# Muennighoff/sgpt

Measured on AMD Instinct MI355X. Metric: encoded sentences/sec (SGPT-125M, seq_len 128, encode + weighted-mean pool + cosine top-10 chunk loop), higher is better.
Workload: dtype f16

## Files before the change

include/sgpt_hip.h:

```cpp
#ifndef SGPT_HIP_H
#define SGPT_HIP_H

#include <stddef.h>
#include <stdint.h>

#ifdef __cplusplus
extern "C" {
#endif

#define SGPT_ABI_VERSION 18

typedef int sgpt_status;
#define SGPT_OK 0
#define SGPT_ERR_INVALID (-1)
#define SGPT_ERR_HIP (-2)
#define SGPT_ERR_MISSING (-3)
#define SGPT_ERR_OOM (-4)
#define SGPT_ERR_COMM (-6)
#define SGPT_ERR_RANGE (-5)

typedef struct sgpt_ctx sgpt_ctx;
typedef struct sgpt_model sgpt_model;

enum { SGPT_F32 = 0, SGPT_BF16 = 1, SGPT_FP8W = 2, SGPT_F16 = 3, SGPT_FP8M = 4 };
enum { SGPT_ARCH_GPTNEO = 0, SGPT_ARCH_GPTJ = 1, SGPT_ARCH_BLOOM = 2, SGPT_ARCH_BERT = 3, SGPT_ARCH_LLAMA = 4 };
enum { SGPT_POOL_WEIGHTEDMEAN = 0, SGPT_POOL_MEAN = 1, SGPT_POOL_LASTTOKEN = 2, SGPT_POOL_LEARNTMEAN = 3,
       SGPT_POOL_CLS = 4 };
enum { SGPT_COS = 0, SGPT_DOT = 1, SGPT_NEG_L2 = 2 };

typedef struct {
    int32_t arch;
    int32_t n_layers;
    int32_t d_model;
    int32_t n_heads;
    int32_t d_ffn;
    int32_t vocab;
    int32_t max_pos;
    int32_t window;
    float ln_eps;
    float attn_scale;
    int32_t compute_dtype;
    const uint8_t* layer_is_local;
    int32_t rotary_dim;
    int32_t qk_split;
    int32_t split_weights;
    int32_t n_kv_heads;
} sgpt_model_desc;

typedef struct {
    const char* name;
    const float* ptr;
    int64_t numel;
} sgpt_tensor_view;

int sgpt_abi_version(void);
sgpt_status sgpt_ctx_create(int hip_device, sgpt_ctx** out);
void sgpt_ctx_destroy(sgpt_ctx* ctx);
const char* sgpt_last_error(const sgpt_ctx* ctx);

sgpt_status sgpt_model_load(sgpt_ctx* ctx, const sgpt_model_desc* desc,
                            const sgpt_tensor_view* tensors, size_t n_tensors, sgpt_model** out);
void sgpt_model_free(sgpt_model* model);

sgpt_status sgpt_model_calibrate_begin(sgpt_model* model);
sgpt_status sgpt_model_calibrate_end(sgpt_model* model, float margin, float* scales_out);
sgpt_status sgpt_model_set_act_scales(sgpt_model* model, const float* scales, int32_t n_scales);

sgpt_status sgpt_encode(sgpt_model* model, const int32_t* ids, const int32_t* pos,
                        const int32_t* seq_off, const int32_t* seq_len, const int32_t* pad_left,
                        int32_t B, int32_t T_pad, int32_t max_alloc_len,
                        int32_t pool_mode, int32_t n_layers_run, int32_t apply_final_ln,
                        int32_t normalize, float* out, float* hidden_out, void* stream);

sgpt_status sgpt_encode_layers(sgpt_model* model, const int32_t* ids, const int32_t* pos,
                               const int32_t* seq_off, const int32_t* seq_len, const int32_t* pad_left,
                               int32_t B, int32_t T_pad, int32_t max_alloc_len, int32_t pool_mode,
                               int32_t normalize, float* out_layers, float* out_mean, void* stream);

sgpt_status sgpt_model_set_pool_weights(sgpt_model* model, const float* weights, int32_t n);

sgpt_status sgpt_lm_logprobs(sgpt_model* model, const float* hidden, const int32_t* row_idx, const int32_t* targets,
                             int32_t n, float* out_logprob, int32_t* out_greedy, void* stream);

sgpt_status sgpt_pool(sgpt_ctx* ctx, const void* hidden, int32_t hidden_dtype, const int32_t* mask,
                      int32_t B, int32_t S, int32_t d, int32_t pool_mode, float* out, void* stream);
sgpt_status sgpt_pool_learnt(sgpt_ctx* ctx, const void* hidden, int32_t hidden_dtype, const int32_t* mask,
                             int32_t B, int32_t S, int32_t d, const float* pos_weights, float* out, void* stream);

sgpt_status sgpt_l2_normalize(sgpt_ctx* ctx, const float* in, int64_t n, int32_t d,
                              void* out, int32_t out_dtype, void* stream);

sgpt_status sgpt_pairwise_scores(sgpt_ctx* ctx, const float* a, const float* b, int64_t n, int32_t d, int32_t cosine,
                                 float* out, void* stream);

sgpt_status sgpt_f32_to_16(sgpt_ctx* ctx, const float* in, int64_t numel, void* out, int32_t out_dtype, void* stream);
sgpt_status sgpt_f32_to_bf16(sgpt_ctx* ctx, const float* in, int64_t numel, void* out, void* stream);

sgpt_status sgpt_model_range_check(sgpt_model* model, int32_t* flagged, int32_t reset, void* stream);
sgpt_status sgpt_model_range_adapt(sgpt_model* model, int32_t* n_raised, void* stream);
sgpt_status sgpt_model_get_range_shifts(sgpt_model* model, int32_t* shifts, int32_t n);
sgpt_status sgpt_model_set_range_shifts(sgpt_model* model, const int32_t* shifts, int32_t n);
sgpt_status sgpt_range_check(sgpt_ctx* ctx, int32_t* flagged, int32_t reset, void* stream);

#define SGPT_PREC_CLASSES 5
enum { SGPT_PC_LN1 = 0, SGPT_PC_ATT = 1, SGPT_PC_CTX = 2, SGPT_PC_LN2 = 3, SGPT_PC_H = 4 };
sgpt_status sgpt_model_set_precision(sgpt_model* model, const int32_t* plan, int32_t n);
sgpt_status sgpt_model_get_precision(sgpt_model* model, int32_t* plan, int32_t n);
sgpt_status sgpt_model_release_split_weights(sgpt_model* model, int64_t* bytes_freed);
sgpt_status sgpt_model_precision_probe_begin(sgpt_model* model);
sgpt_status sgpt_model_precision_probe_end(sgpt_model* model, float* crest_out );
sgpt_status sgpt_row_crest(sgpt_ctx* ctx, const void* x, int32_t dtype, int64_t n, int32_t d, int64_t ld, float* crest_out,
                           void* stream);
sgpt_status sgpt_split16(sgpt_ctx* ctx, const float* in, int64_t n, int32_t d, int32_t layout, void* out, int32_t out_dtype,
                         void* stream);
sgpt_status sgpt_linear_split(sgpt_ctx* ctx, int32_t dtype, int32_t epi, const void* A, const void* W, const float* bias,
                              void* out, int64_t ldo, int64_t lo_delta, int64_t hi2_delta, int32_t M, int32_t N, int32_t K,
                              void* stream);

uint64_t sgpt_ctx_generation(const sgpt_ctx* ctx);
sgpt_status sgpt_ctx_reserve(sgpt_ctx* ctx, size_t encode_bytes, size_t score_bytes);

sgpt_status sgpt_fp8_quantize_rows(sgpt_ctx* ctx, const float* w, int64_t rows, int64_t cols,
                                   uint8_t* codes, float* scale, void* stream);
sgpt_status sgpt_fp8_dequantize_rows(sgpt_ctx* ctx, const uint8_t* codes, const float* scale, int64_t rows,
                                     int64_t cols, void* out, int32_t out_dtype, void* stream);

sgpt_status sgpt_scores(sgpt_ctx* ctx, const void* a, const void* b, int32_t dtype,
                        int64_t na, int64_t nb, int32_t d, float* out, int64_t ldo, void* stream);

sgpt_status sgpt_score_topk(sgpt_ctx* ctx, const void* q, const void* corpus, int32_t dtype,
                            int32_t nq, int64_t N, int32_t d, int32_t k, int64_t idx_base,
                            float* run_val, int64_t* run_idx, int32_t n_run, int32_t* n_out,
                            void* stream);

sgpt_status sgpt_score_topk_q8(sgpt_ctx* ctx, const void* q, const uint8_t* codes, const float* scale, int32_t nq, int64_t N, int32_t d,
                               int32_t k, int64_t idx_base, float* run_val, int64_t* run_idx, int32_t n_run, int32_t* n_out,
                               void* stream);

sgpt_status sgpt_score_topk_refined(sgpt_ctx* ctx, const float* q, const float* corpus32, const void* corpus16, int32_t dtype16,
                                    int32_t nq, int64_t N, int32_t d, int32_t k, int64_t idx_base, float margin,
                                    float* run_val, int64_t* run_idx, int32_t n_run, int32_t* n_out, int32_t* fallback_flag_out,
                                    void* stream);

sgpt_status sgpt_topk_merge(sgpt_ctx* ctx, const float* val, const int64_t* idx, int32_t nq,
                            int32_t m, int32_t k, const int64_t* exclude_idx,
                            float* out_val, int64_t* out_idx, void* stream);

#define SGPT_COMM_ID_BYTES 128
sgpt_status sgpt_comm_unique_id(uint8_t* id );
sgpt_status sgpt_comm_init(sgpt_ctx* ctx, const uint8_t* id, int32_t rank, int32_t world);
sgpt_status sgpt_comm_destroy(sgpt_ctx* ctx);
int32_t sgpt_comm_world(const sgpt_ctx* ctx);
int32_t sgpt_comm_rank(const sgpt_ctx* ctx);
sgpt_status sgpt_allgather_rows(sgpt_ctx* ctx, const void* local, const int64_t* counts, int64_t row_bytes, void* out,
                                void* stream);
sgpt_status sgpt_allgather_rows_padded(sgpt_ctx* ctx, const void* local, const int64_t* counts, int64_t row_bytes, void* out,
                                       void* stream);
sgpt_status sgpt_exchange_topk(sgpt_ctx* ctx, const float* val, const int64_t* idx, int32_t nq, int32_t k, int32_t k_out,
                               const int64_t* exclude_idx, float* out_val, int64_t* out_idx, void* stream);
sgpt_status sgpt_fold_gathered_topk(sgpt_ctx* ctx, const float* gathered_val, const int64_t* gathered_idx, int32_t world,
                                    int32_t nq, int32_t k, int32_t k_out, const int64_t* exclude_idx, float* out_val,
                                    int64_t* out_idx, void* stream);

sgpt_status sgpt_topk(sgpt_ctx* ctx, const float* scores, int32_t nq, int64_t n, int64_t ld,
                      int32_t k, int64_t idx_base, float* out_val, int64_t* out_idx, void* stream);

#define SGPT_EVAL_MAX_CUTS 16
sgpt_status sgpt_eval_ranked(sgpt_ctx* ctx, const int64_t* idx, const float* val, int32_t nq, int32_t K,
                             const int32_t* qrel_off, const int64_t* qrel_pos, const int32_t* qrel_rel,
                             const int32_t* ideal_rel, const int32_t* k_values, int32_t nk, int32_t check_order,
                             int32_t* out_hits, int32_t* out_first, float* out_dcg, float* out_idcg, float* out_sp,
                             int32_t* out_R, void* stream);

#define SGPT_EVAL_MAX_GROUP 1024
sgpt_status sgpt_eval_groups(sgpt_ctx* ctx, const float* emb, int32_t n_rows, int32_t d, int32_t mode, const float* scores_in,
                             int32_t G, const int32_t* grp_off, int32_t n_cand, int32_t max_group, const int32_t* q_row,
                             const int32_t* cand_row, const int32_t* cand_rel, const int32_t* R_extra,
                             const int32_t* ideal_off, const int32_t* ideal_rel, int32_t n_ideal, float* out_scores,
                             int32_t* out_order, int32_t* out_hits1, int32_t* out_hits5, int32_t* out_first, int32_t* out_R, float* out_sp,
                             float* out_dcg, float* out_idcg, void* stream);

#define SGPT_EVAL_MAX_PAIRS (1 << 24)
sgpt_status sgpt_eval_pairs(sgpt_ctx* ctx, const float* score, const int32_t* label, int32_t n, int32_t check_nan,
                            int32_t* out_rank2, int64_t* out_n_pos, int64_t* out_n_used, double* out_ap_num, void* stream);

sgpt_status sgpt_linear(sgpt_ctx* ctx, int32_t dtype, int32_t epi, int32_t out_dtype, const void* A, const void* W,
                        const float* bias, const float* resid, void* out, int32_t M, int32_t N, int32_t K, void* stream);

sgpt_status sgpt_linear_query(sgpt_ctx* ctx, int32_t dtype, int32_t epi, const void* A, const float* x, const float* ln_gamma,
                              const float* ln_beta, float ln_eps, const void* W, const float* bias, const float* resid, void* out,
                              void* out_vt, int32_t n_split, int32_t M, int32_t N, int32_t K, void* stream);

sgpt_status sgpt_linear_qkv(sgpt_ctx* ctx, int32_t dtype, const void* A, const void* W, void* out, void* out_vt, int32_t n_split,
                            int32_t M, int32_t N, int32_t K, void* stream);

sgpt_status sgpt_attention(sgpt_ctx* ctx, int32_t dtype, const void* q, const void* k, const void* v, int64_t ldq, int64_t ldvt,
                           void* out, int64_t ldo, const int32_t* seq_off, int32_t B, int32_t T, int32_t H, int32_t dh,
                           int32_t window, float scale, const float* alibi, int32_t max_alloc_len, int32_t out_fp8,
                           float out_scale, int32_t* range_flag, int32_t x3, int64_t qk_lo_delta, int64_t v_lo_delta,
                           int64_t ctx_lo_delta, int64_t ctx_hi2_delta, void* stream);

sgpt_status sgpt_attention_ex(sgpt_ctx* ctx, int32_t dtype, const void* q, const void* k, const void* v, int64_t ldq, int64_t ldvt,
                              void* out, int64_t ldo, const int32_t* seq_off, int32_t B, int32_t T, int32_t H, int32_t dh,
                              int32_t window, float scale, const float* alibi, int32_t max_alloc_len, int32_t out_fp8,
                              float out_scale, int32_t* range_flag, int32_t x3, int64_t qk_lo_delta, int64_t v_lo_delta,
                              int64_t ctx_lo_delta, int64_t ctx_hi2_delta, int32_t causal, const int32_t* seq_len, void* stream);

sgpt_status sgpt_attention_gqa(sgpt_ctx* ctx, int32_t dtype, const void* q, const void* k, const void* v, int64_t ldq, int64_t ldvt,
                               void* out, int64_t ldo, const int32_t* seq_off, int32_t B, int32_t T, int32_t H, int32_t n_kv_heads,
                               int32_t dh, int32_t window, float scale, const float* alibi, int32_t max_alloc_len, int32_t out_fp8,
                               float out_scale, int32_t* range_flag, int32_t x3, int64_t qk_lo_delta, int64_t v_lo_delta,
                               int64_t ctx_lo_delta, int64_t ctx_hi2_delta, void* stream);

sgpt_status sgpt_embed(sgpt_ctx* ctx, const int32_t* ids, const int32_t* pos, const float* wte, const float* wpe, int32_t T,
                       int32_t d, int32_t vocab, int32_t max_pos, float* out, void* stream);
sgpt_status sgpt_layernorm(sgpt_ctx* ctx, const float* x, const float* gamma, const float* beta, int32_t T, int32_t d, float eps,
                           void* out, int32_t out_dtype, float out_mul, int32_t split, void* stream);
sgpt_status sgpt_layernorm_writeback(sgpt_ctx* ctx, float* x, const float* gamma, const float* beta, int32_t T, int32_t d, float eps,
                                     void* out16, int32_t out_dtype, void* stream);
sgpt_status sgpt_rmsnorm(sgpt_ctx* ctx, const float* x, const float* gamma, int32_t T, int32_t d, float eps, void* out, int32_t out_dtype,
                         void* stream);
sgpt_status sgpt_swiglu(sgpt_ctx* ctx, const void* gu, int32_t dtype, int32_t T, int32_t ffn, void* out, void* stream);
sgpt_status sgpt_rope_half(sgpt_ctx* ctx, void* buf, int32_t dtype, int64_t ld, int64_t k_off, const int32_t* pos, const float* sin_t,
                           const float* cos_t, int32_t T, int32_t H, int32_t H_kv, int32_t head_dim, int32_t max_pos, void* stream);
sgpt_status sgpt_qknorm_rope_half(sgpt_ctx* ctx, void* buf, int32_t dtype, int64_t ld, int64_t k_off, const int32_t* pos,
                                  const float* sin_t, const float* cos_t, int32_t T, int32_t H, int32_t H_kv, int32_t head_dim,
                                  int32_t max_pos, const float* q_gamma, const float* k_gamma, float eps, void* stream);
sgpt_status sgpt_lnf_pool_ex(sgpt_ctx* ctx, const float* x, const float* gamma, const float* beta, const int32_t* seq_off,
                             const int32_t* seq_len, const int32_t* pad_left, int32_t B, int32_t d, float eps, int32_t apply_ln,
                             int32_t mode, int32_t normalize, const float* pos_weights, int32_t n_weights, float* out,
                             int32_t* nonfinite_flag, int32_t norm_kind, void* stream);
sgpt_status sgpt_lnf_pool(sgpt_ctx* ctx, const float* x, const float* gamma, const float* beta, const int32_t* seq_off,
                          const int32_t* seq_len, const int32_t* pad_left, int32_t B, int32_t d, float eps, int32_t apply_ln,
                          int32_t mode, int32_t normalize, const float* pos_weights, int32_t n_weights, float* out,
                          int32_t* nonfinite_flag, void* stream);
sgpt_status sgpt_rope(sgpt_ctx* ctx, void* buf, int32_t dtype, int64_t ld, int64_t k_off, const int32_t* pos, const float* sin,
                      const float* cos, int32_t T, int32_t H, int32_t head_dim, int32_t rotary_dim, int32_t max_pos, void* stream);
sgpt_status sgpt_logprob_rows(sgpt_ctx* ctx, const float* logits, int64_t ld, int32_t V, const int32_t* targets, int32_t n,
                              float* out_logprob, int32_t* out_greedy, void* stream);

sgpt_status sgpt_layernorm_fp8(sgpt_ctx* ctx, const float* x, const float* gamma, const float* beta, int32_t T, int32_t d,
                               float eps, uint8_t* codes, float* row_scale, void* stream);
sgpt_status sgpt_linear_fp8(sgpt_ctx* ctx, int32_t epi, int32_t out_dtype, const uint8_t* A, const float* a_scale,
                            float a_scalar, const uint8_t* W, const float* w_scale, const float* bias, const float* resid,
                            void* out, float out_scale, int32_t M, int32_t N, int32_t K, void* stream);

sgpt_status sgpt_prof_enable(sgpt_ctx* ctx, int32_t on);
sgpt_status sgpt_prof_read(sgpt_ctx* ctx, int64_t* launches, double* ms, double* flops, int32_t reset);

int32_t sgpt_ctx_set_gemm_cu_cap(sgpt_ctx* ctx, int32_t n);
int32_t sgpt_ctx_set_low_latency(sgpt_ctx* ctx, int32_t on);
int32_t sgpt_ctx_set_tile_policy(sgpt_ctx* ctx, int32_t policy);
int32_t sgpt_ctx_set_query_tile(sgpt_ctx* ctx, int32_t k);

sgpt_status sgpt_bench_gemm(sgpt_ctx* ctx, int32_t dtype, int32_t epi, int32_t out_dtype,
                            int32_t M, int32_t N, int32_t K, int32_t iters, float* ms_out);

#ifdef __cplusplus
}
#endif
#endif
```

sgpt_amd/_lib.py:

```python
import ctypes as C
import os

HERE = os.path.dirname(os.path.abspath(__file__))
LIB_PATH = os.environ.get("SGPT_HIP_LIB") or os.path.join(HERE, "lib", "libsgpt_hip.so")

SGPT_F32, SGPT_BF16, SGPT_FP8W, SGPT_F16, SGPT_FP8M = 0, 1, 2, 3, 4
SGPT_ABI_VERSION = 18
SGPT_PREC_CLASSES = 5
PC_LN1, PC_ATT, PC_CTX, PC_LN2, PC_H = 0, 1, 2, 3, 4
SGPT_ERR_RANGE = -5
SGPT_ERR_COMM = -6
SGPT_COMM_ID_BYTES = 128
SGPT_EVAL_MAX_CUTS = 16
SGPT_EVAL_MAX_GROUP = 1024
SGPT_EVAL_MAX_PAIRS = 1 << 24
SGPT_COS, SGPT_DOT, SGPT_NEG_L2 = 0, 1, 2
SGPT_ARCH_GPTNEO, SGPT_ARCH_GPTJ, SGPT_ARCH_BLOOM, SGPT_ARCH_BERT, SGPT_ARCH_LLAMA = 0, 1, 2, 3, 4
POOL_MODES = {"weightedmean": 0, "mean": 1, "lasttoken": 2, "learntmean": 3, "cls": 4}
EPI_BIAS_GELU_ERF = 9


class ModelDesc(C.Structure):
    _fields_ = [("arch", C.c_int32), ("n_layers", C.c_int32), ("d_model", C.c_int32), ("n_heads", C.c_int32),
                ("d_ffn", C.c_int32), ("vocab", C.c_int32), ("max_pos", C.c_int32), ("window", C.c_int32),
                ("ln_eps", C.c_float), ("attn_scale", C.c_float), ("compute_dtype", C.c_int32),
                ("layer_is_local", C.POINTER(C.c_uint8)), ("rotary_dim", C.c_int32), ("qk_split", C.c_int32),
                ("split_weights", C.c_int32), ("n_kv_heads", C.c_int32)]


class TensorView(C.Structure):
    _fields_ = [("name", C.c_char_p), ("ptr", C.c_void_p), ("numel", C.c_int64)]


SIGNATURES = {
    "sgpt_abi_version": (C.c_int, []),
    "sgpt_ctx_create": (C.c_int, [C.c_int, C.POINTER(C.c_void_p)]),
    "sgpt_ctx_destroy": (None, [C.c_void_p]),
    "sgpt_last_error": (C.c_char_p, [C.c_void_p]),
    "sgpt_model_load": (C.c_int, [C.c_void_p, C.POINTER(ModelDesc), C.POINTER(TensorView), C.c_size_t,
                                  C.POINTER(C.c_void_p)]),
    "sgpt_model_free": (None, [C.c_void_p]),
    "sgpt_encode": (C.c_int, [C.c_void_p, C.c_void_p, C.c_void_p, C.c_void_p, C.c_void_p, C.c_void_p,
                              C.c_int32, C.c_int32, C.c_int32, C.c_int32, C.c_int32, C.c_int32, C.c_int32,
                              C.c_void_p, C.c_void_p, C.c_void_p]),
    "sgpt_encode_layers": (C.c_int, [C.c_void_p, C.c_void_p, C.c_void_p, C.c_void_p, C.c_void_p, C.c_void_p,
                                     C.c_int32, C.c_int32, C.c_int32, C.c_int32, C.c_int32, C.c_void_p, C.c_void_p,
                                     C.c_void_p]),
    "sgpt_model_set_pool_weights": (C.c_int, [C.c_void_p, C.c_void_p, C.c_int32]),
    "sgpt_pool_learnt": (C.c_int, [C.c_void_p, C.c_void_p, C.c_int32, C.c_void_p, C.c_int32, C.c_int32, C.c_int32,
                                   C.c_void_p, C.c_void_p, C.c_void_p]),
    "sgpt_fp8_quantize_rows": (C.c_int, [C.c_void_p, C.c_void_p, C.c_int64, C.c_int64, C.c_void_p, C.c_void_p,
                                         C.c_void_p]),
    "sgpt_fp8_dequantize_rows": (C.c_int, [C.c_void_p, C.c_void_p, C.c_void_p, C.c_int64, C.c_int64, C.c_void_p,
                                           C.c_int32, C.c_void_p]),
    "sgpt_lm_logprobs": (C.c_int, [C.c_void_p, C.c_void_p, C.c_void_p, C.c_void_p, C.c_int32, C.c_void_p, C.c_void_p,
                                   C.c_void_p]),
    "sgpt_pool": (C.c_int, [C.c_void_p, C.c_void_p, C.c_int32, C.c_void_p, C.c_int32, C.c_int32, C.c_int32,
                            C.c_int32, C.c_void_p, C.c_void_p]),
    "sgpt_l2_normalize": (C.c_int, [C.c_void_p, C.c_void_p, C.c_int64, C.c_int32, C.c_void_p, C.c_int32, C.c_void_p]),
    "sgpt_pairwise_scores": (C.c_int, [C.c_void_p, C.c_void_p, C.c_void_p, C.c_int64, C.c_int32, C.c_int32, C.c_void_p, C.c_void_p]),
    "sgpt_f32_to_bf16": (C.c_int, [C.c_void_p, C.c_void_p, C.c_int64, C.c_void_p, C.c_void_p]),
    "sgpt_f32_to_16": (C.c_int, [C.c_void_p, C.c_void_p, C.c_int64, C.c_void_p, C.c_int32, C.c_void_p]),
    "sgpt_range_check": (C.c_int, [C.c_void_p, C.POINTER(C.c_int32), C.c_int32, C.c_void_p]),
    "sgpt_ctx_generation": (C.c_uint64, [C.c_void_p]),
    "sgpt_ctx_reserve": (C.c_int, [C.c_void_p, C.c_size_t, C.c_size_t]),
    "sgpt_scores": (C.c_int, [C.c_void_p, C.c_void_p, C.c_void_p, C.c_int32, C.c_int64, C.c_int64, C.c_int32,
                              C.c_void_p, C.c_int64, C.c_void_p]),
    "sgpt_score_topk": (C.c_int, [C.c_void_p, C.c_void_p, C.c_void_p, C.c_int32, C.c_int32, C.c_int64, C.c_int32,
                                  C.c_int32, C.c_int64, C.c_void_p, C.c_void_p, C.c_int32, C.POINTER(C.c_int32),
                                  C.c_void_p]),
    "sgpt_score_topk_q8": (C.c_int, [C.c_void_p, C.c_void_p, C.c_void_p, C.c_void_p, C.c_int32, C.c_int64, C.c_int32,
                                     C.c_int32, C.c_int64, C.c_void_p, C.c_void_p, C.c_int32, C.POINTER(C.c_int32),
                                     C.c_void_p]),
    "sgpt_score_topk_refined": (C.c_int, [C.c_void_p, C.c_void_p, C.c_void_p, C.c_void_p, C.c_int32, C.c_int32, C.c_int64, C.c_int32,
                                           C.c_int32, C.c_int64, C.c_float, C.c_void_p, C.c_void_p, C.c_int32, C.c_void_p, C.c_void_p,
                                           C.c_void_p]),
    "sgpt_topk_merge": (C.c_int, [C.c_void_p, C.c_void_p, C.c_void_p, C.c_int32, C.c_int32, C.c_int32, C.c_void_p,
                                  C.c_void_p, C.c_void_p, C.c_void_p]),
    "sgpt_topk": (C.c_int, [C.c_void_p, C.c_void_p, C.c_int32, C.c_int64, C.c_int64, C.c_int32, C.c_int64,
                            C.c_void_p, C.c_void_p, C.c_void_p]),
    "sgpt_eval_ranked": (C.c_int, [C.c_void_p, C.c_void_p, C.c_void_p, C.c_int32, C.c_int32, C.c_void_p, C.c_void_p, C.c_void_p,
                                   C.c_void_p, C.POINTER(C.c_int32), C.c_int32, C.c_int32, C.c_void_p, C.c_void_p, C.c_void_p,
                                   C.c_void_p, C.c_void_p, C.c_void_p, C.c_void_p]),
    "sgpt_eval_groups": (C.c_int, [C.c_void_p, C.c_void_p, C.c_int32, C.c_int32, C.c_int32, C.c_void_p, C.c_int32, C.c_void_p, C.c_int32,
                                   C.c_int32, C.c_void_p, C.c_void_p, C.c_void_p, C.c_void_p, C.c_void_p, C.c_void_p, C.c_int32,
                                   C.c_void_p, C.c_void_p, C.c_void_p, C.c_void_p, C.c_void_p, C.c_void_p, C.c_void_p, C.c_void_p,
                                   C.c_void_p, C.c_void_p]),
    "sgpt_eval_pairs": (C.c_int, [C.c_void_p, C.c_void_p, C.c_void_p, C.c_int32, C.c_int32, C.c_void_p, C.c_void_p, C.c_void_p,
                                  C.c_void_p, C.c_void_p]),
    "sgpt_linear": (C.c_int, [C.c_void_p, C.c_int32, C.c_int32, C.c_int32, C.c_void_p, C.c_void_p, C.c_void_p, C.c_void_p,
                              C.c_void_p, C.c_int32, C.c_int32, C.c_int32, C.c_void_p]),
    "sgpt_linear_query": (C.c_int, [C.c_void_p, C.c_int32, C.c_int32, C.c_void_p, C.c_void_p, C.c_void_p, C.c_void_p, C.c_float, C.c_void_p,
                                    C.c_void_p, C.c_void_p, C.c_void_p, C.c_void_p, C.c_int32, C.c_int32, C.c_int32, C.c_int32, C.c_void_p]),
    "sgpt_linear_qkv": (C.c_int, [C.c_void_p, C.c_int32, C.c_void_p, C.c_void_p, C.c_void_p, C.c_void_p, C.c_int32, C.c_int32, C.c_int32,
                                  C.c_int32, C.c_void_p]),
    "sgpt_model_calibrate_begin": (C.c_int, [C.c_void_p]),
    "sgpt_model_calibrate_end": (C.c_int, [C.c_void_p, C.c_float, C.c_void_p]),
    "sgpt_model_set_act_scales": (C.c_int, [C.c_void_p, C.c_void_p, C.c_int32]),
    "sgpt_layernorm_fp8": (C.c_int, [C.c_void_p, C.c_void_p, C.c_void_p, C.c_void_p, C.c_int32, C.c_int32, C.c_float, C.c_void_p,
                                     C.c_void_p, C.c_void_p]),
    "sgpt_linear_fp8": (C.c_int, [C.c_void_p, C.c_int32, C.c_int32, C.c_void_p, C.c_void_p, C.c_float, C.c_void_p, C.c_void_p,
                                  C.c_void_p, C.c_void_p, C.c_void_p, C.c_float, C.c_int32, C.c_int32, C.c_int32, C.c_void_p]),
    "sgpt_comm_unique_id": (C.c_int, [C.c_void_p]),
    "sgpt_comm_init": (C.c_int, [C.c_void_p, C.c_void_p, C.c_int32, C.c_int32]),
    "sgpt_comm_destroy": (C.c_int, [C.c_void_p]),
    "sgpt_comm_world": (C.c_int32, [C.c_void_p]),
    "sgpt_comm_rank": (C.c_int32, [C.c_void_p]),
    "sgpt_allgather_rows": (C.c_int, [C.c_void_p, C.c_void_p, C.c_void_p, C.c_int64, C.c_void_p, C.c_void_p]),
    "sgpt_allgather_rows_padded": (C.c_int, [C.c_void_p, C.c_void_p, C.c_void_p, C.c_int64, C.c_void_p, C.c_void_p]),
    "sgpt_exchange_topk": (C.c_int, [C.c_void_p, C.c_void_p, C.c_void_p, C.c_int32, C.c_int32, C.c_int32, C.c_void_p,
                                     C.c_void_p, C.c_void_p, C.c_void_p]),
    "sgpt_fold_gathered_topk": (C.c_int, [C.c_void_p, C.c_void_p, C.c_void_p, C.c_int32, C.c_int32, C.c_int32, C.c_int32,
                                          C.c_void_p, C.c_void_p, C.c_void_p, C.c_void_p]),
    "sgpt_ctx_set_low_latency": (C.c_int32, [C.c_void_p, C.c_int32]),
    "sgpt_ctx_set_tile_policy": (C.c_int32, [C.c_void_p, C.c_int32]),
    "sgpt_ctx_set_gemm_cu_cap": (C.c_int32, [C.c_void_p, C.c_int32]),
    "sgpt_ctx_set_query_tile": (C.c_int32, [C.c_void_p, C.c_int32]),
    "sgpt_model_range_check": (C.c_int, [C.c_void_p, C.POINTER(C.c_int32), C.c_int32, C.c_void_p]),
    "sgpt_model_range_adapt": (C.c_int, [C.c_void_p, C.POINTER(C.c_int32), C.c_void_p]),
    "sgpt_model_get_range_shifts": (C.c_int, [C.c_void_p, C.c_void_p, C.c_int32]),
    "sgpt_model_set_range_shifts": (C.c_int, [C.c_void_p, C.c_void_p, C.c_int32]),
    "sgpt_model_set_precision": (C.c_int, [C.c_void_p, C.c_void_p, C.c_int32]),
    "sgpt_model_get_precision": (C.c_int, [C.c_void_p, C.c_void_p, C.c_int32]),
    "sgpt_model_release_split_weights": (C.c_int, [C.c_void_p, C.c_void_p]),
    "sgpt_model_precision_probe_begin": (C.c_int, [C.c_void_p]),
    "sgpt_model_precision_probe_end": (C.c_int, [C.c_void_p, C.c_void_p]),
    "sgpt_row_crest": (C.c_int, [C.c_void_p, C.c_void_p, C.c_int32, C.c_int64, C.c_int32, C.c_int64, C.POINTER(C.c_float), C.c_void_p]),
    "sgpt_split16": (C.c_int, [C.c_void_p, C.c_void_p, C.c_int64, C.c_int32, C.c_int32, C.c_void_p, C.c_int32, C.c_void_p]),
    "sgpt_linear_split": (C.c_int, [C.c_void_p, C.c_int32, C.c_int32, C.c_void_p, C.c_void_p, C.c_void_p, C.c_void_p,
                                    C.c_int64, C.c_int64, C.c_int64, C.c_int32, C.c_int32, C.c_int32, C.c_void_p]),
    "sgpt_attention": (C.c_int, [C.c_void_p, C.c_int32, C.c_void_p, C.c_void_p, C.c_void_p, C.c_int64, C.c_int64,
                                 C.c_void_p, C.c_int64, C.c_void_p, C.c_int32, C.c_int32, C.c_int32, C.c_int32,
                                 C.c_int32, C.c_float, C.c_void_p, C.c_int32, C.c_int32,
                                 C.c_float, C.c_void_p, C.c_int32, C.c_int64, C.c_int64,
                                 C.c_int64, C.c_int64, C.c_void_p]),
    "sgpt_attention_ex": (C.c_int, [C.c_void_p, C.c_int32, C.c_void_p, C.c_void_p, C.c_void_p, C.c_int64, C.c_int64,
                                    C.c_void_p, C.c_int64, C.c_void_p, C.c_int32, C.c_int32, C.c_int32, C.c_int32,
                                    C.c_int32, C.c_float, C.c_void_p, C.c_int32, C.c_int32,
                                    C.c_float, C.c_void_p, C.c_int32, C.c_int64, C.c_int64,
                                    C.c_int64, C.c_int64, C.c_int32, C.c_void_p, C.c_void_p]),
    "sgpt_attention_gqa": (C.c_int, [C.c_void_p, C.c_int32, C.c_void_p, C.c_void_p, C.c_void_p, C.c_int64, C.c_int64,
                                     C.c_void_p, C.c_int64, C.c_void_p, C.c_int32, C.c_int32, C.c_int32, C.c_int32, C.c_int32,
                                     C.c_int32, C.c_float, C.c_void_p, C.c_int32, C.c_int32,
                                     C.c_float, C.c_void_p, C.c_int32, C.c_int64, C.c_int64,
                                     C.c_int64, C.c_int64, C.c_void_p]),
    "sgpt_rmsnorm": (C.c_int, [C.c_void_p, C.c_void_p, C.c_void_p, C.c_int32, C.c_int32, C.c_float, C.c_void_p, C.c_int32, C.c_void_p]),
    "sgpt_swiglu": (C.c_int, [C.c_void_p, C.c_void_p, C.c_int32, C.c_int32, C.c_int32, C.c_void_p, C.c_void_p]),
    "sgpt_rope_half": (C.c_int, [C.c_void_p, C.c_void_p, C.c_int32, C.c_int64, C.c_int64, C.c_void_p, C.c_void_p, C.c_void_p,
                                 C.c_int32, C.c_int32, C.c_int32, C.c_int32, C.c_int32, C.c_void_p]),
    "sgpt_qknorm_rope_half": (C.c_int, [C.c_void_p, C.c_void_p, C.c_int32, C.c_int64, C.c_int64, C.c_void_p, C.c_void_p, C.c_void_p,
                                        C.c_int32, C.c_int32, C.c_int32, C.c_int32, C.c_int32, C.c_void_p, C.c_void_p, C.c_float,
                                        C.c_void_p]),
    "sgpt_lnf_pool_ex": (C.c_int, [C.c_void_p, C.c_void_p, C.c_void_p, C.c_void_p, C.c_void_p, C.c_void_p, C.c_void_p, C.c_int32,
                                   C.c_int32, C.c_float, C.c_int32, C.c_int32, C.c_int32, C.c_void_p, C.c_int32, C.c_void_p,
                                   C.c_void_p, C.c_int32, C.c_void_p]),
    "sgpt_layernorm_writeback": (C.c_int, [C.c_void_p, C.c_void_p, C.c_void_p, C.c_void_p, C.c_int32, C.c_int32, C.c_float, C.c_void_p,
                                           C.c_int32, C.c_void_p]),
    "sgpt_embed": (C.c_int, [C.c_void_p, C.c_void_p, C.c_void_p, C.c_void_p, C.c_void_p, C.c_int32, C.c_int32, C.c_int32, C.c_int32,
                             C.c_void_p, C.c_void_p]),
    "sgpt_layernorm": (C.c_int, [C.c_void_p, C.c_void_p, C.c_void_p, C.c_void_p, C.c_int32, C.c_int32, C.c_float, C.c_void_p,
                                 C.c_int32, C.c_float, C.c_int32, C.c_void_p]),
    "sgpt_lnf_pool": (C.c_int, [C.c_void_p, C.c_void_p, C.c_void_p, C.c_void_p, C.c_void_p, C.c_void_p, C.c_void_p, C.c_int32,
                                C.c_int32, C.c_float, C.c_int32, C.c_int32, C.c_int32, C.c_void_p, C.c_int32, C.c_void_p,
                                C.c_void_p, C.c_void_p]),
    "sgpt_rope": (C.c_int, [C.c_void_p, C.c_void_p, C.c_int32, C.c_int64, C.c_int64, C.c_void_p, C.c_void_p, C.c_void_p,
                            C.c_int32, C.c_int32, C.c_int32, C.c_int32, C.c_int32, C.c_void_p]),
    "sgpt_logprob_rows": (C.c_int, [C.c_void_p, C.c_void_p, C.c_int64, C.c_int32, C.c_void_p, C.c_int32, C.c_void_p, C.c_void_p,
                                    C.c_void_p]),
    "sgpt_bench_gemm": (C.c_int, [C.c_void_p, C.c_int32, C.c_int32, C.c_int32, C.c_int32, C.c_int32, C.c_int32,
                                  C.c_int32, C.POINTER(C.c_float)]),
    "sgpt_prof_enable": (C.c_int, [C.c_void_p, C.c_int32]),
    "sgpt_prof_read": (C.c_int, [C.c_void_p, C.POINTER(C.c_int64), C.POINTER(C.c_double), C.POINTER(C.c_double),
                                 C.c_int32]),
}

_lib = None


class SgptHipError(RuntimeError):
    pass


class SgptRangeError(SgptHipError):
    """dtype='f16': a weight is outside the IEEE-half range, or an activation class is beyond every power-of-two range
    shift (use dtype='bf16'); dtype='fp8mfma': an e4m3 code saturated (re-calibrate)."""

EXPERIMENT_SIGNATURES = {
    "sgpt_exp_set_gemm_skew": (C.c_int32, [C.c_int32]),
    "sgpt_exp_set_gemm_w": (C.c_int32, [C.c_int32]),
}


def load():
    global _lib
    if _lib is not None:
        return _lib
    if not os.path.exists(LIB_PATH):
        raise SgptHipError(f"{LIB_PATH} is missing: build it with `python -m sgpt_amd.build` "
                           "(hipcc --offload-arch=gfx950); there is no CPU/PyTorch fallback")
    lib = C.CDLL(LIB_PATH)
    for name, (res, args) in SIGNATURES.items():
        fn = getattr(lib, name)
        fn.restype = res
        fn.argtypes = args
    for name, (res, args) in EXPERIMENT_SIGNATURES.items():
        if hasattr(lib, name):
            fn = getattr(lib, name)
            fn.restype = res
            fn.argtypes = args
    if lib.sgpt_abi_version() != SGPT_ABI_VERSION:
        raise SgptHipError("libsgpt_hip.so ABI version mismatch: rebuild with `python -m sgpt_amd.build --force`")
    _lib = lib
    return lib


def check(ctx_handle, status, what=""):
    if status == 0:
        return
    msg = load().sgpt_last_error(ctx_handle)
    msg = msg.decode() if msg else ""
    if status == -1:
        raise ValueError(f"{what}: {msg}")
    if status == SGPT_ERR_RANGE:
        raise SgptRangeError(f"{what}: {msg}")
    raise SgptHipError(f"{what}: status {status}: {msg}")
```

sgpt_amd/csrc/common.h:

```cpp
#pragma once
#include <hip/hip_runtime.h>
#include <stdint.h>

typedef uint16_t bf16_t;
struct f16_t { uint16_t bits; };
typedef __attribute__((ext_vector_type(8))) __bf16 bf16x8;
typedef __attribute__((ext_vector_type(8))) _Float16 f16x8;
typedef __attribute__((ext_vector_type(4))) float f32x4;
typedef __attribute__((ext_vector_type(16))) float f32x16;

constexpr int DT_F32 = 0, DT_BF16 = 1, DT_FP8W = 2, DT_F16 = 3;
__host__ __device__ constexpr bool dt_is16(int dt) { return dt == DT_BF16 || dt == DT_F16; }

#define WAVE 64

typedef uint2 __attribute__((may_alias)) uint2_a;
typedef uint4 __attribute__((may_alias)) uint4_a;
typedef float4 __attribute__((may_alias)) float4_a;

__device__ __forceinline__ float bf16_to_f32(bf16_t v) { return __uint_as_float(((uint32_t)v) << 16); }

typedef __attribute__((ext_vector_type(2))) __bf16 bf16x2_t;
typedef __attribute__((ext_vector_type(2))) float f32x2_t;
__device__ __forceinline__ uint32_t pack_bf16x2(float lo, float hi) {
// ... 80 lines not shown
    u32x4v_t w;
    if constexpr (NT) w = __builtin_nontemporal_load(reinterpret_cast<const u32x4v_t*>(ptr));
    else w = *reinterpret_cast<const u32x4v_t*>(ptr);
    return make_uint4(w[0], w[1], w[2], w[3]);
}

template <bool NT>
__device__ __forceinline__ float4 ldg16(const float* ptr) {
    if constexpr (NT) {
        typedef float f32x4v_t __attribute__((ext_vector_type(4)));
        const f32x4v_t w = __builtin_nontemporal_load(reinterpret_cast<const f32x4v_t*>(ptr));
        return make_float4(w[0], w[1], w[2], w[3]);
    } else {
        return *reinterpret_cast<const float4*>(ptr);
    }
}

__device__ __forceinline__ float wave_sum(float v) {
#pragma unroll
    for (int o = 32; o > 0; o >>= 1) v += __shfl_xor(v, o, 64);
    return v;
}
template <int CTRL> __device__ __forceinline__ float dpp_mov(float v) {
    return __uint_as_float((unsigned)__builtin_amdgcn_update_dpp(0, (int)__float_as_uint(v), CTRL, 0xf, 0xf, false));
}
__device__ __forceinline__ float wave_sum_valu(float v) {
    { const auto r = __builtin_amdgcn_permlane32_swap(__float_as_uint(v), __float_as_uint(v), false, false);
      v = __uint_as_float(r[0]) + __uint_as_float(r[1]); }
    { const auto r = __builtin_amdgcn_permlane16_swap(__float_as_uint(v), __float_as_uint(v), false, false);
      v = __uint_as_float(r[0]) + __uint_as_float(r[1]); }
    v += dpp_mov<0x128>(v);
    v += dpp_mov<0x1B>(dpp_mov<0x141>(v));
    v += dpp_mov<0x4E>(v);
    v += dpp_mov<0xB1>(v);
    return v;
}
template <int R>
__device__ __forceinline__ void wave_sum_valu_multi(float (&v)[R]) {
#pragma unroll
    for (int u = 0; u < R; ++u) {
        const auto r = __builtin_amdgcn_permlane32_swap(__float_as_uint(v[u]), __float_as_uint(v[u]), false, false);
        v[u] = __uint_as_float(r[0]) + __uint_as_float(r[1]);
    }
#pragma unroll
    for (int u = 0; u < R; ++u) {
        const auto r = __builtin_amdgcn_permlane16_swap(__float_as_uint(v[u]), __float_as_uint(v[u]), false, false);
        v[u] = __uint_as_float(r[0]) + __uint_as_float(r[1]);
    }
#pragma unroll
    for (int u = 0; u < R; ++u) v[u] += dpp_mov<0x128>(v[u]);
#pragma unroll
    for (int u = 0; u < R; ++u) v[u] += dpp_mov<0x1B>(dpp_mov<0x141>(v[u]));
#pragma unroll
    for (int u = 0; u < R; ++u) v[u] += dpp_mov<0x4E>(v[u]);
#pragma unroll
    for (int u = 0; u < R; ++u) v[u] += dpp_mov<0xB1>(v[u]);
}
__device__ __forceinline__ float wave_max(float v) {
#pragma unroll
    for (int o = 32; o > 0; o >>= 1) v = fmaxf(v, __shfl_xor(v, o, 64));
    return v;
}

__device__ __forceinline__ float gelu_new(float u) {
    const float c = 0.7978845608028654f;
    float t = c * (u + 0.044715f * u * u * u);
    return 0.5f * u * (1.0f + tanhf(t));
}

__device__ __forceinline__ float gelu_erf(float u) { return 0.5f * u * (1.0f + erff(u * 0.70710678118654752f)); }

__device__ __forceinline__ float gelu_new_fast(float u) {
    const float k0 = -2.0f * 0.7978845608028654f * 1.4426950408889634f;
    const float k1 = k0 * 0.044715f;
    const float z = u * __builtin_fmaf(u * u, k1, k0);
    return u * __builtin_amdgcn_rcpf(1.0f + __builtin_amdgcn_exp2f(z));
}

__device__ __forceinline__ float gelu_new_fast_scaled(float u, float inv) {
    const float k0 = -2.0f * 0.7978845608028654f * 1.4426950408889634f;
    const float k1 = k0 * 0.044715f;
    const float z = u * __builtin_fmaf(u * u, k1, k0);
    return u * __builtin_amdgcn_rcpf(__builtin_fmaf(__builtin_amdgcn_exp2f(z), inv, inv));
}

__device__ __forceinline__ bool cand_room(const int* cnt, int cap) {
    return __hip_atomic_load(cnt, __ATOMIC_RELAXED, __HIP_MEMORY_SCOPE_AGENT) <= cap;
}

enum GemmEpi {
    EPI_STORE = 0,
    EPI_BIAS_GELU = 1,
    EPI_BIAS_RESID = 2,
    EPI_SCORE = 3,
    EPI_VT = 4,
    EPI_NONE = 5,
    EPI_SCORE_FILTER = 6,
    EPI_SCORE_TOP2 = 8,
    EPI_BIAS_GELU_ERF = 9,
    EPI_QKV = 7,
};

__host__ __device__ constexpr bool epi_is_gelu(int epi) { return epi == EPI_BIAS_GELU || epi == EPI_BIAS_GELU_ERF; }

struct GemmArgs {
    const void* A;
    const void* W;
    void* out;
    const float* bias;
    const float* resid;
    int M, N, K;
    long lda, ldw, ldo;
    int m_valid;
    int skew;
    int gm, gn;
    int balanced;
    const int* pred;
    const float* thr;
    long thr_ld;
    float* cand_val;
    long long* cand_idx;
    int* cand_cnt;
    int cand_cap;
    long idx_base;
    long long* dbg;
    int* range_flag;
    unsigned* range_amax;
    float in_mul, out_mul, out_mul2;
    int k_algo;
    int kgroups;
    int force256;
    int cu_cap;
    long lo_delta, hi2_delta, lo_delta2;
    void* out2;
    long ldo2;
    int n_split;
    int n_valid;
    const float* a_scale;
    const float* w_scale;
    float a_scalar;
    float out_scale;
};

void launch_gemm(int dtype, int epi, int out_dtype, const GemmArgs& a, hipStream_t s);
constexpr int QGEMM_MAX_ROWS = 4096;
struct QGemmArgs {
    GemmArgs g;
    const float* x;
    const float* ln_g;
    const float* ln_b;
    float eps, ln_mul;
    int group;
    int tile;
};
bool qgemm_shape_ok(int M, int N, int K, int epi, int n_split);
bool qgemm_ln_ok(int M, int N, int d, int epi, int n_split);
bool launch_qgemm(int dtype, int epi, int out_dtype, const QGemmArgs& a, hipStream_t s);

bool gemm_qkv_one_launch(int M, int n_split, bool force256);
bool gemm_score_tail_foldable(int M, long N, int K);
bool gemm_qkv_bulk(int M, int N, int K, int n_split, bool force256);
#ifdef SGPT_EXPERIMENTS
int set_gemm_skew(int cycles);
int set_gemm_use_w(int on);
#endif
bool gemm_fp8_shape_ok(int M, int N, int K);
void launch_gemm_fp8(int epi, int out_dtype, const GemmArgs& a, hipStream_t s);
struct Score8Args {
    GemmArgs g;
    const float* scale;
    long scale_stride;
};
bool score64q8_shape_ok(int M, long N, int K, const void* codes, long ldw);
void launch_score64q8(int epi, const Score8Args& a, hipStream_t s);
void launch_gemm256w(int dtype, int epi, const GemmArgs& a, hipStream_t s, bool deep_a);

struct AttnArgs {
    const void* q;
    const void* k;
    const void* v;
    void* ctx;
    const int* seq_off;
    int B, H, dh;
    long ldq, ldvt, ldo;
    int window;
    float scale;
    int max_alloc_len;
    const float* alibi;
    int dtype;
    int out_fp8;
    float out_scale;
    int* range_flag;
    int x3;
    long qk_lo_delta, v_lo_delta, ctx_lo_delta, ctx_hi2_delta;
    int noncausal;
    const int* seq_len;
    int kv_group = 1;
};
inline bool attn_x3_supported(int dh) { return dh == 64 || dh == 128; }
void launch_attn_bf16(const AttnArgs& a, hipStream_t s);
void launch_attn_f32(const AttnArgs& a, hipStream_t s);

void launch_embed(const int* ids, const int* pos, const float* wte, const float* wpe, float* x, int T, int d, int vocab,
                  int max_pos, hipStream_t s);
void launch_layernorm(const float* x, const float* g, const float* b, void* out, int out_dtype, int T, int d,
                      float eps, hipStream_t s, float out_mul = 1.0f);
void launch_layernorm_writeback(float* x, const float* g, const float* b, void* out16, int out_dtype, int T, int d, float eps,
                                int* range_flag, hipStream_t s);
void launch_layernorm_split(const float* x, const float* g, const float* b, void* out, int out_dtype, int T, int d,
                            float eps, hipStream_t s, float out_mul);
void launch_rmsnorm(const float* x, const float* g, void* out, int out_dtype, int T, int d, float eps, int* range_flag, hipStream_t s);
void launch_swiglu(const void* gu, void* h, int dtype, int T, int ffn, int* range_flag, hipStream_t s);
void launch_pack_split_rows(const float* src, long rows, long cols, void* dst, int out_dtype, hipStream_t s);
void launch_crest16(const void* in, int T, int cols, long ld, int dtype, unsigned* out_bits, hipStream_t s);
void launch_split16_rows(const float* in, long n, int d, int layout, void* out, int out_dtype, hipStream_t s);
void launch_layernorm_q8(const float* x, const float* g, const float* b, void* q, float* scale, void* out16, int out16_dtype,
                         int T, int d, float eps, hipStream_t s);
void launch_absmax16(const void* in, long numel, int dtype, unsigned* out_bits, hipStream_t s);
void launch_lnf_pool(const float* x, const float* g, const float* b, const int* seq_off, const int* seq_len,
                     const int* pad_left, int B, int d, float eps, int apply_ln, int mode, int normalize,
                     const float* pos_weights, int pos_weights_n, float* out, hipStream_t s,
                     int* nonfinite_flag = nullptr,
                     int norm_kind = 0);
void launch_pool(const void* hidden, int dtype, const int* mask, int B, int S, int d, int mode,
                 const float* pos_weights, float* out, hipStream_t s);
void launch_fp8_quant_rows(const float* w, long rows, long cols, void* q, float* scale, hipStream_t s);
void launch_fp8_dequant_rows(const void* q, const float* scale, long rows, long cols, void* out, int out_dtype,
                             hipStream_t s);
void launch_l2norm(const float* in, long n, int d, void* out, int out_dtype, hipStream_t s);
void launch_pairwise(const float* a, const float* b, long n, int d, bool cosine, float* out, hipStream_t s);
void launch_gather_rows(const float* src, const int* row_idx, int n, int d, float* dst, hipStream_t s);
void launch_logprob_rows(const float* logits, long ld, int V, const int* targets, int n, float* out_lp, int* out_arg,
                         hipStream_t s);
void launch_mean_over_axis0(const float* in, int n0, long n, float* out, hipStream_t s);
void launch_f32_to_bf16(const float* in, long numel, void* out, hipStream_t s);
void launch_f32_to_16(const float* in, long numel, void* out, int out_dtype, hipStream_t s);
void launch_absmax(const float* in, long numel, unsigned* out_bits, hipStream_t s);
void launch_fill_f32(float* p, long n, float v, hipStream_t s);
void launch_rope(void* qk, int dtype, long ld, long k_off, const int* pos, const float* sin_t, const float* cos_t, int T,
                 int H, int dh, int rotary_dim, int max_pos, hipStream_t s);
void launch_rope_half(void* qk, int dtype, long ld, long k_off, const int* pos, const float* sin_t, const float* cos_t, int T,
                      int H, int H_kv, int dh, int max_pos, hipStream_t s);
void launch_qknorm_rope_half(void* qk, int dtype, long ld, long k_off, const int* pos, const float* sin_t, const float* cos_t,
                             const float* q_g, const float* k_g, float eps, int T, int H, int H_kv, int dh, int max_pos, int* range_flag,
                             hipStream_t s);
void launch_qkv_deinterleave(const float* src, float* dst, int H, int dh, long row_len, hipStream_t s);
void launch_fill_rand(void* p, long n, int dtype, unsigned seed, float scale, hipStream_t s);

void launch_topk_select(const float* scores, long ld, long n, long idx_base, const float* prev_val,
                        const int64_t* prev_idx, int n_prev, long prev_ld, int nq, int k, int nan_to_m1,
                        const int64_t* exclude_idx, float* out_val, int64_t* out_idx, hipStream_t s,
                        const int* pred = nullptr, float* thr_out = nullptr,
                        int gather_k = 0);
void launch_rescore(const float* q, const float* corpus, const int64_t* idx, long ld_idx, int nq, int m, int d, long idx_base,
                    long n_docs, float* out_val, int64_t* out_idx, long ld_out, hipStream_t s);
void launch_refine_check(const float* v16, int k, int kp, float margin, int nq, int* flag, hipStream_t s);
void launch_list_append(const float* in_val, const int64_t* in_idx, long ld_in, int n_run, int nq, float* out_val, int64_t* out_idx,
                        long ld_out, int col0, hipStream_t s);
void launch_score_prep(const void* q, void* qpad, long q_bytes, long qpad_bytes, int* counters, long n_counters, long long* idx_list,
                       long n_idx, hipStream_t s);
void launch_thr_below(const float* list, int k, int nq, float* thr, hipStream_t s);
void launch_cand_merge(const float* run_val, const int64_t* run_idx, const float* cand_val, const int64_t* cand_idx,
                       int* cand_cnt, int cap, int nq, int k, float* out_val, int64_t* out_idx, int* overflow,
                       hipStream_t s, float* thr_io = nullptr);
```

sgpt_amd/csrc/ctx.h:

```cpp
#pragma once
#include <hip/hip_runtime.h>

#include <string>
#include <utility>
#include <vector>

struct sgpt_ctx {
    int device = 0;
    std::string err;
    void* ws = nullptr; size_t ws_bytes = 0;
    void* ws2 = nullptr; size_t ws2_bytes = 0;
    void* ws3 = nullptr; size_t ws3_bytes = 0;
    void* ws4 = nullptr; size_t ws4_bytes = 0;
    void* ws5 = nullptr; size_t ws5_bytes = 0;
    void* ws6 = nullptr; size_t ws6_bytes = 0;
    void* comm = nullptr;
    int comm_rank = 0, comm_world = 0;
    uint64_t generation = 0;
    int* range_flag = nullptr;
    int kgroups = 1;
    int force256 = 0;
    int no_qpath = 0;
    int cu_cap = 0;
    int qtile = 0;
    bool prof = false;
    std::vector<std::pair<hipEvent_t, hipEvent_t>> ev_pool;
    size_t ev_used = 0;
    std::vector<double> ev_flops;
    int64_t prof_launches = 0; double prof_ms = 0, prof_flops = 0;
};
```

sgpt_amd/csrc/ctx.hip:

```cpp
#include "host.h"

namespace sgpt_host {

sgpt_status ensure(sgpt_ctx* c, void** p, size_t* have, size_t need) {
    if (*have >= need) return SGPT_OK;
    if (*p) { HIPC(c, hipDeviceSynchronize()); HIPC(c, hipFree(*p)); *p = nullptr; *have = 0; }
    need = align_up(need + (need >> 3), 1 << 20);
    if (hipMalloc(p, need) != hipSuccess) { *p = nullptr; return fail(c, SGPT_ERR_OOM, "hipMalloc workspace failed"); }
    HIPC(c, hipMemset(*p, 0, need));
    *have = need;
    c->generation++;
    return SGPT_OK;
}

void gemm(sgpt_ctx* c, int dtype, int epi, int out_dtype, const GemmArgs& a0, hipStream_t s) {
    Prof p(c, s, 2.0 * (double)a0.m_valid * a0.N * (a0.k_algo > 0 ? a0.k_algo : a0.K));
    GemmArgs a = a0;
    a.kgroups = c->kgroups; a.force256 = c->force256; a.cu_cap = c->cu_cap;
    launch_gemm(dtype, epi, out_dtype, a, s);
}

bool qgemm(sgpt_ctx* c, int dtype, int epi, int out_dtype, const QGemmArgs& a, hipStream_t s) {
    Prof p(c, s, 2.0 * (double)a.g.m_valid * a.g.N * a.g.K);
    return launch_qgemm(dtype, epi, out_dtype, a, s);
}

}

extern "C" {

int sgpt_abi_version(void) { return SGPT_ABI_VERSION; }

sgpt_status sgpt_ctx_create(int hip_device, sgpt_ctx** out) {
    if (!out) return SGPT_ERR_INVALID;
    *out = nullptr;
    int n = 0;
    if (hipGetDeviceCount(&n) != hipSuccess || hip_device < 0 || hip_device >= n) return SGPT_ERR_HIP;
    if (hipSetDevice(hip_device) != hipSuccess) return SGPT_ERR_HIP;
    sgpt_ctx* c = new sgpt_ctx();
    c->device = hip_device;
    if (hipMalloc((void**)&c->range_flag, 256) != hipSuccess || hipMemset(c->range_flag, 0, 256) != hipSuccess) {
        delete c;
        return SGPT_ERR_OOM;
    }
    *out = c;
    return SGPT_OK;
}

void sgpt_ctx_destroy(sgpt_ctx* c) {
    if (!c) return;
    (void)hipSetDevice(c->device);
    (void)hipDeviceSynchronize();
    if (c->ws) (void)hipFree(c->ws);
    if (c->ws2) (void)hipFree(c->ws2);
    (void)sgpt_comm_destroy(c);
    if (c->ws3) (void)hipFree(c->ws3);
    if (c->ws4) (void)hipFree(c->ws4);
    if (c->ws5) (void)hipFree(c->ws5);
    if (c->ws6) (void)hipFree(c->ws6);
    if (c->range_flag) (void)hipFree(c->range_flag);
    for (auto& e : c->ev_pool) { (void)hipEventDestroy(e.first); (void)hipEventDestroy(e.second); }
    delete c;
}

const char* sgpt_last_error(const sgpt_ctx* c) { return c ? c->err.c_str() : "null ctx"; }

uint64_t sgpt_ctx_generation(const sgpt_ctx* c) { return c ? c->generation : 0; }

sgpt_status sgpt_ctx_reserve(sgpt_ctx* c, size_t encode_bytes, size_t score_bytes) {
    if (!c) return SGPT_ERR_INVALID;
    HIPC(c, hipSetDevice(c->device));
    sgpt_status st = ensure(c, &c->ws, &c->ws_bytes, encode_bytes);
    if (st != SGPT_OK) return st;
    return ensure(c, &c->ws2, &c->ws2_bytes, score_bytes);
}

sgpt_status sgpt_range_check(sgpt_ctx* c, int32_t* flagged, int32_t reset, void* stream) {
    if (!c || !flagged) return SGPT_ERR_INVALID;
    HIPC(c, hipSetDevice(c->device));
    hipStream_t s = (hipStream_t)stream;
    int h = 0;
    HIPC(c, hipMemcpyAsync(&h, c->range_flag, sizeof(int), hipMemcpyDeviceToHost, s));
    HIPC(c, hipStreamSynchronize(s));
    if (reset && h) HIPC(c, hipMemsetAsync(c->range_flag, 0, sizeof(int), s));
    *flagged = h;
    return SGPT_OK;
}

sgpt_status sgpt_prof_enable(sgpt_ctx* c, int32_t on) {
    if (!c) return SGPT_ERR_INVALID;
    c->prof = on != 0;
    return SGPT_OK;
}

sgpt_status sgpt_prof_read(sgpt_ctx* c, int64_t* launches, double* ms, double* flops, int32_t reset) {
    if (!c) return SGPT_ERR_INVALID;
    HIPC(c, hipSetDevice(c->device));
    HIPC(c, hipDeviceSynchronize());
    for (size_t i = 0; i < c->ev_used; ++i) {
        float t = 0;
        HIPC(c, hipEventElapsedTime(&t, c->ev_pool[i].first, c->ev_pool[i].second));
        c->prof_ms += t;
        c->prof_flops += c->ev_flops[i];
        c->prof_launches++;
    }
    c->ev_used = 0;
    if (launches) *launches = c->prof_launches;
    if (ms) *ms = c->prof_ms;
    if (flops) *flops = c->prof_flops;
    if (reset) { c->prof_launches = 0; c->prof_ms = 0; c->prof_flops = 0; }
    return SGPT_OK;
}

int32_t sgpt_ctx_set_low_latency(sgpt_ctx* c, int32_t on) {
    if (!c) return 0;
    const int old = c->kgroups > 1 ? 1 : 0;
    c->kgroups = on ? 2 : 1;
    return old;
}
int32_t sgpt_ctx_set_gemm_cu_cap(sgpt_ctx* c, int32_t n) {
    if (!c) return 0;
    const int old = c->cu_cap;
    c->cu_cap = n > 0 ? n : 0;
    return old;
}
int32_t sgpt_ctx_set_tile_policy(sgpt_ctx* c, int32_t policy) {
    if (!c) return 0;
    const int old = c->force256 ? 1 : c->no_qpath ? 2 : 0;
    c->force256 = policy == 1 ? 1 : 0;
    c->no_qpath = policy == 2 ? 1 : 0;
    return old;
}
int32_t sgpt_ctx_set_query_tile(sgpt_ctx* c, int32_t k) {
    if (!c || k < 0 || k > 7) return -1;
    const int old = c->qtile;
    c->qtile = k;
    return old;
}
#ifdef SGPT_EXPERIMENTS
int32_t sgpt_exp_set_gemm_skew(int32_t cycles) { return set_gemm_skew(cycles); }
int32_t sgpt_exp_set_gemm_w(int32_t on) { return set_gemm_use_w(on); }
#endif

}
```

sgpt_amd/csrc/encode.hip:

```cpp
#include "host.h"

namespace {

struct Fwd {
    sgpt_model* m; sgpt_ctx* c; hipStream_t s;
    const Family* F;
    const int32_t *pos, *seq_off, *seq_len;
    int B, T, max_alloc;
    int d_q, d_kv;
    int dt;
    int* range_flag;
    bool can_split, any_ln, any_att, any_ctx, any_h, split, fp8, mlp8, qpath, qln;
    float* x;
    void *a, *ctx, *qkv, *vt, *h;
    void* gu;
    void* a8; float* sa;
    long att_lo;
};

GemmArgs proj(const Fwd& f, const void* A, long lda, const void* W, int N, int K, void* out, long ldo, const float* bias,
              const float* resid = nullptr) {
    GemmArgs g{};
    g.M = f.T; g.m_valid = f.T; g.range_flag = f.range_flag;
    g.A = A; g.lda = lda; g.W = W; g.ldw = K; g.N = N; g.K = K; g.out = out; g.ldo = ldo; g.bias = bias; g.resid = resid;
    return g;
}

void split_w(GemmArgs& g, const void* W3, int k, int nblk = 3) { g.W = W3; g.K = nblk * k; g.ldw = 3 * k; g.k_algo = k; }

void proj_qk_vt(const Fwd& f, const GemmArgs& g, int n_qk, int n_v, const void* W3 = nullptr, int p_ln1 = 0) {
    GemmArgs qk = g, v = g;
    if (p_ln1) split_w(qk, W3, g.K, p_ln1 == 3 ? 2 : 3);
    qk.N = n_qk;
    gemm(f.c, f.dt, EPI_STORE, f.dt, qk, f.s);
    if (p_ln1 == 2) split_w(v, (const bf16_t*)W3 + (size_t)n_qk * 3 * g.K, g.K);
    else v.W = (const bf16_t*)g.W + (size_t)n_qk * g.K;
    v.N = n_v; v.out = f.vt; v.ldo = f.T; v.bias = g.bias ? g.bias + n_qk : nullptr;
    gemm(f.c, f.dt, EPI_VT, f.dt, v, f.s);
}

AttnArgs attn_base(const Fwd& f, const LayerW& l, int k_qkv) {
    const sgpt_model_desc& d = f.m->d;
    const int dq = f.d_q;
    AttnArgs at{};
    at.dtype = f.dt;
    at.seq_off = f.seq_off; at.B = f.B; at.H = d.n_heads; at.dh = dq / d.n_heads; at.window = l.is_local ? d.window : 0;
    at.scale = d.attn_scale * pow2f(2 * k_qkv);
    at.max_alloc_len = f.max_alloc; at.ctx = f.ctx; at.ldo = dq; at.alibi = f.m->alibi;
    at.q = f.qkv; at.kv_group = d.n_heads / d.n_kv_heads;
    if (f.vt) { at.k = (bf16_t*)f.qkv + dq; at.v = f.vt; at.ldq = dq + f.d_kv; at.ldvt = f.T; }
    else { at.k = (float*)f.qkv + dq; at.v = (float*)f.qkv + dq + f.d_kv; at.ldq = dq + 2 * f.d_kv; }
    return at;
}

AttnArgs attn_bidir(const Fwd& f, const LayerW& l) {
    AttnArgs at = attn_base(f, l, 0);
    at.noncausal = 1; at.seq_len = f.seq_len;
    return at;
}

sgpt_status block_bert_f32(const Fwd& f, const LayerW& l, int) {
    const sgpt_model_desc& d = f.m->d;
    const int dm = d.d_model, ffn = d.d_ffn, T = f.T;
    gemm(f.c, SGPT_F32, EPI_STORE, SGPT_F32, proj(f, f.x, dm, l.w_qkv, 3 * dm, dm, f.qkv, 3 * dm, l.b_qkv), f.s);
    launch_attn_f32(attn_bidir(f, l), f.s);
    gemm(f.c, SGPT_F32, EPI_BIAS_RESID, SGPT_F32, proj(f, f.ctx, dm, l.w_o, dm, dm, f.x, dm, l.b_o, f.x), f.s);
    launch_layernorm(f.x, l.ln1_g, l.ln1_b, f.x, SGPT_F32, T, dm, d.ln_eps, f.s);
    gemm(f.c, SGPT_F32, EPI_BIAS_GELU_ERF, SGPT_F32, proj(f, f.x, dm, l.w_fc, ffn, dm, f.h, ffn, l.b_fc), f.s);
    gemm(f.c, SGPT_F32, EPI_BIAS_RESID, SGPT_F32, proj(f, f.h, ffn, l.w_proj, dm, ffn, f.x, dm, l.b_proj, f.x), f.s);
    launch_layernorm(f.x, l.ln2_g, l.ln2_b, f.x, SGPT_F32, T, dm, d.ln_eps, f.s);
    return SGPT_OK;
}

sgpt_status block_bert16(const Fwd& f, const LayerW& l, int) {
    const sgpt_model_desc& d = f.m->d;
    const int dm = d.d_model, ffn = d.d_ffn, T = f.T, dt = f.dt;
    GemmArgs q = proj(f, f.a, dm, l.w_qkv, 3 * dm, dm, f.qkv, 2 * dm, l.b_qkv);
    if (gemm_qkv_one_launch(T, 2 * dm, f.c->force256 != 0)) {
        q.n_split = 2 * dm; q.out2 = f.vt; q.ldo2 = T;
        gemm(f.c, dt, EPI_QKV, dt, q, f.s);
    } else proj_qk_vt(f, q, 2 * dm, dm);
    launch_attn_bf16(attn_bidir(f, l), f.s);
    gemm(f.c, dt, EPI_BIAS_RESID, SGPT_F32, proj(f, f.ctx, dm, l.w_o, dm, dm, f.x, dm, l.b_o, f.x), f.s);
    launch_layernorm_writeback(f.x, l.ln1_g, l.ln1_b, f.a, dt, T, dm, d.ln_eps, f.range_flag, f.s);
    gemm(f.c, dt, EPI_BIAS_GELU_ERF, dt, proj(f, f.a, dm, l.w_fc, ffn, dm, f.h, ffn, l.b_fc), f.s);
    gemm(f.c, dt, EPI_BIAS_RESID, SGPT_F32, proj(f, f.h, ffn, l.w_proj, dm, ffn, f.x, dm, l.b_proj, f.x), f.s);
    launch_layernorm_writeback(f.x, l.ln2_g, l.ln2_b, f.a, dt, T, dm, d.ln_eps, f.range_flag, f.s);
    return SGPT_OK;
}


void rope_llama(const Fwd& f, const LayerW& l, int dt, long ld, int dh) {
    const sgpt_model_desc& d = f.m->d;
    if (l.qn_g)
        launch_qknorm_rope_half(f.qkv, dt, ld, f.d_q, f.pos, f.m->rot_sin, f.m->rot_cos, l.qn_g, l.kn_g, d.ln_eps, f.T, d.n_heads, d.n_kv_heads,
                                dh, d.max_pos, f.range_flag, f.s);
    else launch_rope_half(f.qkv, dt, ld, f.d_q, f.pos, f.m->rot_sin, f.m->rot_cos, f.T, d.n_heads, d.n_kv_heads, dh, d.max_pos, f.s);
}
sgpt_status block_llama_f32(const Fwd& f, const LayerW& l, int) {
    const sgpt_model_desc& d = f.m->d;
    const int dm = d.d_model, ffn = d.d_ffn, T = f.T, dq = f.d_q, dh = dq / d.n_heads, dkv = f.d_kv;
    launch_rmsnorm(f.x, l.ln1_g, f.a, SGPT_F32, T, dm, d.ln_eps, nullptr, f.s);
    gemm(f.c, SGPT_F32, EPI_STORE, SGPT_F32, proj(f, f.a, dm, l.w_qkv, dq + 2 * dkv, dm, f.qkv, dq + 2 * dkv, l.b_qkv), f.s);
    rope_llama(f, l, SGPT_F32, dq + 2 * dkv, dh);
    launch_attn_f32(attn_base(f, l, 0), f.s);
    gemm(f.c, SGPT_F32, EPI_BIAS_RESID, SGPT_F32, proj(f, f.ctx, dq, l.w_o, dm, dq, f.x, dm, l.b_o, f.x), f.s);
    launch_rmsnorm(f.x, l.ln2_g, f.a, SGPT_F32, T, dm, d.ln_eps, nullptr, f.s);
    gemm(f.c, SGPT_F32, EPI_STORE, SGPT_F32, proj(f, f.a, dm, l.w_fc, 2 * ffn, dm, f.gu, 2 * ffn, nullptr), f.s);
    launch_swiglu(f.gu, f.h, SGPT_F32, T, ffn, nullptr, f.s);
    gemm(f.c, SGPT_F32, EPI_BIAS_RESID, SGPT_F32, proj(f, f.h, ffn, l.w_proj, dm, ffn, f.x, dm, l.b_proj, f.x), f.s);
    return SGPT_OK;
}

sgpt_status block_llama16(const Fwd& f, const LayerW& l, int) {
    const sgpt_model_desc& d = f.m->d;
    const int dm = d.d_model, ffn = d.d_ffn, T = f.T, dt = f.dt, dq = f.d_q, dh = dq / d.n_heads, dkv = f.d_kv;
    launch_rmsnorm(f.x, l.ln1_g, f.a, dt, T, dm, d.ln_eps, f.range_flag, f.s);
    proj_qk_vt(f, proj(f, f.a, dm, l.w_qkv, dq + dkv, dm, f.qkv, dq + dkv, l.b_qkv), dq + dkv, dkv);
    rope_llama(f, l, dt, dq + dkv, dh);
    launch_attn_bf16(attn_base(f, l, 0), f.s);
    gemm(f.c, dt, EPI_BIAS_RESID, SGPT_F32, proj(f, f.ctx, dq, l.w_o, dm, dq, f.x, dm, l.b_o, f.x), f.s);
    launch_rmsnorm(f.x, l.ln2_g, f.a, dt, T, dm, d.ln_eps, f.range_flag, f.s);
    gemm(f.c, dt, EPI_STORE, dt, proj(f, f.a, dm, l.w_fc, 2 * ffn, dm, f.gu, 2 * ffn, nullptr), f.s);
    launch_swiglu(f.gu, f.h, dt, T, ffn, f.range_flag, f.s);
    gemm(f.c, dt, EPI_BIAS_RESID, SGPT_F32, proj(f, f.h, ffn, l.w_proj, dm, ffn, f.x, dm, l.b_proj, f.x), f.s);
    return SGPT_OK;
}

sgpt_status block_f32(const Fwd& f, const LayerW& l, int) {
    const sgpt_model_desc& d = f.m->d;
    const int dm = d.d_model, ffn = d.d_ffn, T = f.T;
    const bool gptj = d.arch == SGPT_ARCH_GPTJ;
    launch_layernorm(f.x, l.ln1_g, l.ln1_b, f.a, SGPT_F32, T, dm, d.ln_eps, f.s);
    gemm(f.c, SGPT_F32, EPI_STORE, SGPT_F32, proj(f, f.a, dm, l.w_qkv, 3 * dm, dm, f.qkv, 3 * dm, l.b_qkv), f.s);
    if (gptj) launch_rope(f.qkv, SGPT_F32, 3 * dm, dm, f.pos, f.m->rot_sin, f.m->rot_cos, T, d.n_heads, dm / d.n_heads, d.rotary_dim, d.max_pos, f.s);
    launch_attn_f32(attn_base(f, l, 0), f.s);
    gemm(f.c, SGPT_F32, EPI_BIAS_RESID, SGPT_F32, proj(f, f.ctx, dm, l.w_o, dm, dm, f.x, dm, l.b_o, f.x), f.s);
    if (!gptj) launch_layernorm(f.x, l.ln2_g, l.ln2_b, f.a, SGPT_F32, T, dm, d.ln_eps, f.s);
    gemm(f.c, SGPT_F32, EPI_BIAS_GELU, SGPT_F32, proj(f, f.a, dm, l.w_fc, ffn, dm, f.h, ffn, l.b_fc), f.s);
    gemm(f.c, SGPT_F32, EPI_BIAS_RESID, SGPT_F32, proj(f, f.h, ffn, l.w_proj, dm, ffn, f.x, dm, l.b_proj, f.x), f.s);
    return SGPT_OK;
}

sgpt_status block_fp8(const Fwd& f, const LayerW& l, int li) {
    const sgpt_model_desc& d = f.m->d;
    const int dm = d.d_model, ffn = d.d_ffn, T = f.T;
    const bool gptj = d.arch == SGPT_ARCH_GPTJ;
    const float s_h = f.m->act_scale[li], s_c = f.m->act_scale[d.n_layers + li];
    auto launch = [&](int epi, int out_dtype, const GemmArgs& q) { Prof pr(f.c, f.s, 2.0 * T * (double)q.N * q.K); launch_gemm_fp8(epi, out_dtype, q, f.s); };
    launch_layernorm_q8(f.x, l.ln1_g, l.ln1_b, f.a8, f.sa, nullptr, f.dt, T, dm, d.ln_eps, f.s);
    GemmArgs qk = proj(f, f.a8, dm, l.w_qkv, 2 * dm, dm, f.qkv, 2 * dm, l.b_qkv);
    qk.a_scale = f.sa; qk.a_scalar = 1.0f; qk.w_scale = l.s_qkv;
    launch(EPI_STORE, f.dt, qk);
    GemmArgs v = proj(f, f.a8, dm, (const uint8_t*)l.w_qkv + (size_t)2 * dm * dm, dm, dm, f.vt, T, l.b_qkv ? l.b_qkv + 2 * dm : nullptr);
    v.a_scale = f.sa; v.a_scalar = 1.0f; v.w_scale = l.s_qkv + 2 * dm;
    launch(EPI_VT, f.dt, v);
    if (gptj) launch_rope(f.qkv, f.dt, 2 * dm, dm, f.pos, f.m->rot_sin, f.m->rot_cos, T, d.n_heads, dm / d.n_heads, d.rotary_dim, d.max_pos, f.s);
    AttnArgs at = attn_base(f, l, 0);
    at.out_fp8 = 1; at.out_scale = s_c; at.range_flag = f.range_flag;
    launch_attn_bf16(at, f.s);
    GemmArgs o = proj(f, f.ctx, dm, l.w_o, dm, dm, f.x, dm, l.b_o, f.x);
    o.a_scalar = s_c; o.w_scale = l.s_o;
    launch(EPI_BIAS_RESID, 0, o);
    if (!gptj) launch_layernorm_q8(f.x, l.ln2_g, l.ln2_b, f.a8, f.sa, nullptr, f.dt, T, dm, d.ln_eps, f.s);
    GemmArgs fc = proj(f, f.a8, dm, l.w_fc, ffn, dm, f.h, ffn, l.b_fc);
    fc.a_scale = f.sa; fc.a_scalar = 1.0f; fc.w_scale = l.s_fc; fc.out_scale = s_h;
    launch(EPI_BIAS_GELU, 0, fc);
    GemmArgs p = proj(f, f.h, ffn, l.w_proj, dm, ffn, f.x, dm, l.b_proj, f.x);
    p.a_scalar = s_h; p.w_scale = l.s_proj;
    launch(EPI_BIAS_RESID, 0, p);
    return SGPT_OK;
}

void block_ln(const Fwd& f, QGemmArgs& q, const float* g, const float* b, int k, bool split, unsigned* crest) {
    const int dm = f.m->d.d_model;
    const float eps = f.m->d.ln_eps;
    q.eps = eps;
    if (f.qln) { q.x = f.x; q.ln_g = g; q.ln_b = b; q.ln_mul = pow2f(-k); return; }
    if (split) launch_layernorm_split(f.x, g, b, f.a, f.dt, f.T, dm, eps, f.s, pow2f(-k));
    else launch_layernorm(f.x, g, b, f.a, f.dt, f.T, dm, eps, f.s, pow2f(-k));
    if (crest) launch_crest16(f.a, f.T, dm, q.g.lda, f.dt, crest, f.s);
}

sgpt_status launch16(const Fwd& f, int epi, int out_dtype, const QGemmArgs& q, const char* what) {
    if (!f.qpath) gemm(f.c, f.dt, epi, out_dtype, q.g, f.s);
    else if (!qgemm(f.c, f.dt, epi, out_dtype, q, f.s)) return fail(f.c, SGPT_ERR_INVALID, std::string("query path: ") + what + " not served");
    return SGPT_OK;
}

sgpt_status block_16(const Fwd& f, const LayerW& l, int li) {
    sgpt_model* m = f.m; sgpt_ctx* c = f.c; hipStream_t s = f.s;
    const int dm = m->d.d_model, ffn = m->d.d_ffn, T = f.T, dt = f.dt;
    const bool gptj = m->d.arch == SGPT_ARCH_GPTJ;
    const bool f16m = dt == SGPT_F16;
    const int* sh = &m->shift[(size_t)li * RS_N];
    const int k_ln1 = f16m ? sh[RS_LN1] : 0, k_qkv = f16m ? sh[RS_QKV] : 0, k_h = f16m ? sh[RS_H] : 0;
    const int k_ln2 = f16m ? (gptj ? sh[RS_LN1] : sh[RS_LN2]) : 0;
    unsigned* slots = m->range_dev + 1 + (size_t)li * RS_N;
    const int* pc = &m->prec[(size_t)li * PC_N];
    const int p_ln1 = f.can_split ? pc[PC_LN1] : 0;
    const bool p_att = f.can_split && pc[PC_ATT] != 0, p_ctx = f.can_split && pc[PC_CTX] != 0, p_h = f.can_split && pc[PC_H] != 0;
    const bool p_ln2 = f.can_split && pc[PC_LN2] != 0 && (!gptj || p_ln1 != 0);
    unsigned* crest = (m->probing && m->crest_dev) ? m->crest_dev + (size_t)li * RS_N : nullptr;
    const long lda1 = p_ln1 ? 3 * dm : dm, lda2 = gptj ? lda1 : (p_ln2 ? 3 * dm : dm), ldc = p_ctx ? 3 * dm : dm, ldh = p_h ? 3 * ffn : ffn;
    sgpt_status st;
    {
        QGemmArgs q{};
        q.g = proj(f, f.a, lda1, l.w_qkv, 3 * dm, dm, f.qkv, 2 * dm, l.b_qkv);
        q.g.in_mul = pow2f(k_ln1); q.g.out_mul = q.g.out_mul2 = pow2f(-k_qkv); q.g.range_amax = f16m ? slots + RS_QKV : nullptr;
        q.g.lo_delta = q.g.lo_delta2 = p_att ? f.att_lo : 0;
        block_ln(f, q, l.ln1_g, l.ln1_b, k_ln1, p_ln1 != 0, crest ? crest + RS_LN1 : nullptr);
        if (f.qpath || ((p_ln1 == 0 || p_ln1 == 2) && gemm_qkv_one_launch(T, 2 * dm, c->force256 != 0)) ||
            (p_ln1 == 0 && !p_att && l.b_qkv == nullptr && gemm_qkv_bulk(T, 3 * dm, dm, 2 * dm, c->force256 != 0))) {
            if (p_ln1 == 2) split_w(q.g, l.w_qkv3, dm);
            q.g.n_split = 2 * dm; q.g.out2 = f.vt; q.g.ldo2 = T;
            if ((st = launch16(f, EPI_QKV, dt, q, "QKV projection")) != SGPT_OK) return st;
        } else {
            proj_qk_vt(f, q.g, 2 * dm, dm, l.w_qkv3, p_ln1);
        }
    }
    if (gptj) launch_rope(f.qkv, dt, 2 * dm, dm, f.pos, m->rot_sin, m->rot_cos, T, m->d.n_heads, dm / m->d.n_heads, m->d.rotary_dim, m->d.max_pos, s);
    AttnArgs at = attn_base(f, l, k_qkv);
    at.x3 = p_att ? 1 : 0; at.qk_lo_delta = f.att_lo; at.v_lo_delta = f.att_lo;
    at.ldo = ldc; at.ctx_lo_delta = p_ctx ? dm : 0; at.ctx_hi2_delta = p_ctx ? 2 * dm : 0;
    launch_attn_bf16(at, s);
    if (crest) launch_crest16(f.ctx, T, dm, ldc, dt, crest + RS_QKV, s);
    if (m->calibrating)
        launch_absmax16(f.ctx, (long)T * dm, dt, m->h_amax + m->d.n_layers + li, s);
    {
        QGemmArgs q{};
        q.g = proj(f, f.ctx, ldc, l.w_o, dm, dm, f.x, dm, l.b_o, f.x);
        if (p_ctx) split_w(q.g, l.w_o3, dm);
        q.g.in_mul = pow2f(k_qkv);
        if ((st = launch16(f, EPI_BIAS_RESID, SGPT_F32, q, "out-projection")) != SGPT_OK) return st;
    }
    {
        QGemmArgs q{};
        q.g = proj(f, f.a, lda2, l.w_fc, ffn, dm, f.h, ldh, l.b_fc);
        if (p_ln2) split_w(q.g, l.w_fc3, dm);
        if (p_h) { q.g.lo_delta = ffn; q.g.hi2_delta = 2 * ffn; }
        q.g.in_mul = pow2f(k_ln2); q.g.out_mul = pow2f(-k_h); q.g.range_amax = f16m ? slots + RS_H : nullptr;
        if (!gptj) block_ln(f, q, l.ln2_g, l.ln2_b, k_ln2, p_ln2, crest ? crest + RS_LN2 : nullptr);
        if ((st = launch16(f, EPI_BIAS_GELU, dt, q, "fc1")) != SGPT_OK) return st;
    }
    if (crest) launch_crest16(f.h, T, ffn, ldh, dt, crest + RS_H, s);
    if (m->calibrating) launch_absmax16(f.h, (long)T * ffn, dt, m->h_amax + li, s);
    QGemmArgs q{};
    q.g = proj(f, f.h, ldh, l.w_proj, dm, ffn, f.x, dm, l.b_proj, f.x);
    if (p_h) split_w(q.g, l.w_proj3, ffn);
    q.g.in_mul = pow2f(k_h);
    return launch16(f, EPI_BIAS_RESID, SGPT_F32, q, "fc2");
}

using BlockFn = sgpt_status (*)(const Fwd&, const LayerW&, int);
BlockFn pick_block(const Fwd& f) {
    const bool bf = f.dt != SGPT_F32;
    if (f.m->d.arch == SGPT_ARCH_BERT) return bf ? block_bert16 : block_bert_f32;
    if (f.m->d.arch == SGPT_ARCH_LLAMA) return bf ? block_llama16 : block_llama_f32;
    return f.mlp8 ? block_fp8 : (bf ? block_16 : block_f32);
}

sgpt_status check_call(sgpt_model* m, const int32_t* const (&layout)[4], const int32_t* pad_left, int B, int T, int max_alloc, int pool_mode,
                       int n_layers_run, bool pooled, const float* hidden_out) {
    sgpt_ctx* c = m->ctx;
    const Family& F = family(m->d.arch);
    if (!layout[0] || !layout[1] || !layout[2] || !layout[3] || B <= 0 || T <= 0 || T % 32 != 0 || max_alloc <= 0 || max_alloc % 2 != 0)
        return fail(c, SGPT_ERR_INVALID, "sgpt_encode: bad token layout (T_pad % 32, max_alloc_len % 2)");
    if (n_layers_run < 0 || n_layers_run > m->d.n_layers) return fail(c, SGPT_ERR_INVALID, "sgpt_encode: n_layers_run out of range");
    if (pool_mode < 0 || pool_mode > SGPT_POOL_CLS) return fail(c, SGPT_ERR_INVALID, "sgpt_encode: bad pool_mode");
    if (pool_mode == SGPT_POOL_LEARNTMEAN && !F.learntmean)
        return fail(c, SGPT_ERR_INVALID, std::string("sgpt_encode: learntmean pooling (trained position weights of the SGPT checkpoints) is not available for ") + F.name);
    if (pool_mode == SGPT_POOL_CLS && !F.cls) return fail(c, SGPT_ERR_INVALID, "sgpt_encode: cls pooling belongs to SGPT_ARCH_BERT");
    if (pool_mode == SGPT_POOL_LEARNTMEAN && pooled) {
        if (!m->pool_w) return fail(c, SGPT_ERR_MISSING, "sgpt_encode: learntmean needs sgpt_model_set_pool_weights first");
        if (!pad_left && max_alloc - 7 > m->pool_w_n)
            return fail(c, SGPT_ERR_INVALID, "sgpt_encode: fewer learnt position weights than the longest sequence");
    }
    if (max_alloc > 2048) return fail(c, SGPT_ERR_INVALID, "sgpt_encode: sequence longer than 2048 tokens");
    if (!pooled && !hidden_out) return fail(c, SGPT_ERR_INVALID, "sgpt_encode: no output requested");
    return SGPT_OK;
}

constexpr size_t SLACK = 64;

sgpt_status plan(Fwd& f, int n_layers_run, float** lp) {
    sgpt_model* m = f.m; sgpt_ctx* c = f.c;
    const int T = f.T, dm = m->d.d_model, ffn = m->d.d_ffn;
    const bool gptj = m->d.arch == SGPT_ARCH_GPTJ, fp8m = m->d.compute_dtype == SGPT_FP8M;
    const bool bf = m->d.compute_dtype != SGPT_F32;
    const size_t esz = bf ? 2 : 4;
    f.fp8 = m->d.compute_dtype == SGPT_FP8W || fp8m;
    f.dt = !bf ? SGPT_F32 : (m->d.compute_dtype == SGPT_F16 ? SGPT_F16 : SGPT_BF16);
    f.d_q = m->d.n_heads * head_dim(m->d); f.d_kv = m->d.n_kv_heads * head_dim(m->d);
    const size_t dq = f.d_q, dkv = f.d_kv;
    f.can_split = bf && !f.fp8;
    for (int li = 0; f.can_split && li < n_layers_run; ++li) {
        const int* pc = &m->prec[(size_t)li * PC_N];
        f.any_ln |= pc[PC_LN1] != 0 || pc[PC_LN2] != 0; f.any_att |= pc[PC_ATT] != 0; f.any_ctx |= pc[PC_CTX] != 0; f.any_h |= pc[PC_H] != 0;
    }
    f.split = f.any_ln || f.any_att || f.any_ctx || f.any_h;
    const bool shapes8 = gemm_fp8_shape_ok(T, ffn, dm) && gemm_fp8_shape_ok(T, dm, ffn) && gemm_fp8_shape_ok(T, 2 * dm, dm);
    f.mlp8 = fp8m && !m->calibrating && shapes8;
    if (f.mlp8)
        for (int li = 0; li < n_layers_run; ++li)
            if (!(m->act_scale[li] > 0.f) || !(m->act_scale[m->d.n_layers + li] > 0.f))
                return fail(c, SGPT_ERR_INVALID, "SGPT_FP8M: activation scales are not set (sgpt_model_calibrate_begin / _end, or sgpt_model_set_act_scales)");
    f.qpath = bf && !f.fp8 && !f.split && f.F->qpath && !(m->probing && m->crest_dev) && !m->calibrating && !c->force256 && !c->no_qpath && T <= QGEMM_MAX_ROWS &&
              qgemm_shape_ok(T, 3 * dm, dm, EPI_QKV, 2 * dm) && qgemm_shape_ok(T, dm, dm, EPI_BIAS_RESID, 0) &&
              qgemm_shape_ok(T, ffn, dm, EPI_BIAS_GELU, 0) && qgemm_shape_ok(T, dm, ffn, EPI_BIAS_RESID, 0);
    f.qln = f.qpath && !gptj && qgemm_ln_ok(T, 3 * dm, dm, EPI_QKV, 2 * dm) && qgemm_ln_ok(T, ffn, dm, EPI_BIAS_GELU, 0);
    size_t off = 0;
    auto carve = [&](size_t bytes) { size_t o = off; off = align_up(off + bytes, 256); return o; };
    const size_t o_x = carve((size_t)T * dm * 4);
    const size_t o_a = carve((size_t)T * (dq > (size_t)dm ? dq : (size_t)dm) * esz * (f.any_ln ? 3 : 1));
    const size_t o_c = (gptj || f.split) ? carve((size_t)T * dm * esz * (f.any_ctx ? 3 : 1)) : o_a;
    size_t qkv_elems = ((size_t)T + SLACK) * (dq + 2 * dkv);
    if (bf && ((size_t)T + 256) * (dq + dkv) > qkv_elems) qkv_elems = ((size_t)T + 256) * (dq + dkv);
    const size_t qkv_bytes = qkv_elems * esz;
    const size_t o_qkv = carve(qkv_bytes * (f.any_att ? 2 : 1));
    const size_t o_h = carve((size_t)T * ffn * esz * (f.any_h ? 3 : 1));
    const size_t o_gu = f.F->swiglu ? carve((size_t)T * 2 * ffn * esz) : 0;
    const size_t o_a8 = f.mlp8 ? carve((size_t)T * dm) : 0;
    const size_t o_sa = f.mlp8 ? carve((size_t)T * 4) : 0;
    const size_t o_lp = lp ? carve((size_t)(m->d.n_layers + 1) * f.B * dm * 4) : 0;
    sgpt_status st = ensure(c, &c->ws, &c->ws_bytes, off);
    if (st != SGPT_OK) return st;
    char* base = (char*)c->ws;
    f.range_flag = (f.mlp8 || f.dt == SGPT_F16) ? (int*)m->range_dev : nullptr;
    f.x = (float*)(base + o_x); f.a = base + o_a; f.ctx = base + o_c; f.qkv = base + o_qkv; f.h = base + o_h;
    if (f.F->swiglu) f.gu = base + o_gu;
    f.vt = bf ? (void*)((bf16_t*)f.qkv + ((size_t)T + SLACK) * (dq + dkv)) : nullptr;
    if (f.mlp8) { f.a8 = base + o_a8; f.sa = (float*)(base + o_sa); }
    if (lp) *lp = (float*)(base + o_lp);
    f.att_lo = (long)(qkv_bytes / 2);
    return SGPT_OK;
}

sgpt_status zero_overread(const Fwd& f) {
    sgpt_ctx* c = f.c; const size_t T = f.T, dm = f.m->d.d_model, dq = f.d_q, dkv = f.d_kv, esz = f.vt ? 2 : 4;
    if (f.vt)
        for (long lo = 0; lo <= (f.any_att ? f.att_lo : 0); lo += f.att_lo) {
            HIPC(c, hipMemsetAsync((bf16_t*)f.qkv + lo + T * (dq + dkv), 0, SLACK * (dq + dkv) * esz, f.s));
            HIPC(c, hipMemsetAsync((bf16_t*)f.vt + lo + T * dkv, 0, SLACK * dkv * esz, f.s));
        }
    else if (f.F->slack_f32) HIPC(c, hipMemsetAsync((float*)f.qkv + T * (dq + 2 * dkv), 0, SLACK * (dq + 2 * dkv) * esz, f.s));
    if (f.m->d.arch == SGPT_ARCH_GPTJ || f.mlp8 || f.split || f.qln || (f.F->post_ln && !f.vt))
        HIPC(c, hipMemsetAsync(f.ctx, 0, T * dm * esz * (f.any_ctx ? 3 : 1), f.s));
    else if (dq > dm) HIPC(c, hipMemsetAsync(f.ctx, 0, T * dq * esz, f.s));
    return SGPT_OK;
}

}

static sgpt_status encode_impl(sgpt_model* m, const int32_t* ids, const int32_t* pos, const int32_t* seq_off,
                               const int32_t* seq_len, const int32_t* pad_left, int32_t B, int32_t T, int32_t max_alloc,
                               int32_t pool_mode, int32_t n_layers_run, int32_t apply_final_ln, int32_t normalize,
                               float* out, float* hidden_out, float* layer_out, float* layer_mean, void* stream) {
    if (!m) return SGPT_ERR_INVALID;
    sgpt_ctx* c = m->ctx;
    const Family& F = family(m->d.arch);
    sgpt_status st = check_call(m, {ids, pos, seq_off, seq_len}, pad_left, B, T, max_alloc, pool_mode, n_layers_run, out || layer_out || layer_mean, hidden_out);
    if (st != SGPT_OK) return st;
    if (!F.lnf) apply_final_ln = 0;
    HIPC(c, hipSetDevice(c->device));
    hipStream_t s = (hipStream_t)stream;
    Fwd f{};
    f.m = m; f.c = c; f.s = s; f.F = &F; f.pos = pos; f.seq_off = seq_off; f.seq_len = seq_len; f.B = B; f.T = T; f.max_alloc = max_alloc;
    if ((st = plan(f, n_layers_run, layer_mean && !layer_out ? &layer_out : nullptr)) != SGPT_OK) return st;
    if ((st = zero_overread(f)) != SGPT_OK) return st;
    const int dm = m->d.d_model, ffn = m->d.d_ffn, dt = f.dt; float* x = f.x;
    auto pool = [&](int final_ln, float* dst, int* range_flag) {
        launch_lnf_pool(x, m->lnf_g, m->lnf_b, seq_off, seq_len, pad_left, B, dm, m->d.ln_eps, final_ln, pool_mode, normalize, m->pool_w,
                        m->pool_w_n, dst, s, range_flag, F.norm_kind);
    };
    launch_embed(ids, pos, m->wte, m->wpe, x, T, dm, m->d.vocab, m->d.max_pos, s);
    if (F.post_ln && f.vt) launch_layernorm_writeback(x, m->emb_ln_g, m->emb_ln_b, f.a, dt, T, dm, m->d.ln_eps, f.range_flag, s);
    else if (m->emb_ln_g) launch_layernorm(x, m->emb_ln_g, m->emb_ln_b, x, SGPT_F32, T, dm, m->d.ln_eps, s);
    const BlockFn block = pick_block(f);
    for (int li = 0; li < n_layers_run; ++li) {
        LayerW l = m->L[li];
        if (layer_out) pool(0, layer_out + (size_t)li * B * dm, nullptr);
        if (f.fp8 && !f.mlp8) {
            launch_fp8_dequant_rows(l.w_qkv, l.s_qkv, (long)3 * dm, dm, m->dq[0], SGPT_BF16, s);
            launch_fp8_dequant_rows(l.w_o, l.s_o, dm, dm, m->dq[1], SGPT_BF16, s);
            launch_fp8_dequant_rows(l.w_fc, l.s_fc, ffn, dm, m->dq[2], SGPT_BF16, s);
            launch_fp8_dequant_rows(l.w_proj, l.s_proj, dm, ffn, m->dq[3], SGPT_BF16, s);
            l.w_qkv = m->dq[0]; l.w_o = m->dq[1]; l.w_fc = m->dq[2]; l.w_proj = m->dq[3];
        }
        if ((st = block(f, l, li)) != SGPT_OK) return st;
    }
    if (hidden_out) {
        if (apply_final_ln && F.norm_kind == 1) launch_rmsnorm(x, m->lnf_g, hidden_out, SGPT_F32, T, dm, m->d.ln_eps, nullptr, s);
        else if (apply_final_ln) launch_layernorm(x, m->lnf_g, m->lnf_b, hidden_out, SGPT_F32, T, dm, m->d.ln_eps, s);
        else HIPC(c, hipMemcpyAsync(hidden_out, x, (size_t)T * dm * 4, hipMemcpyDeviceToDevice, s));
    }
    if (out) pool(apply_final_ln, out, m->d.compute_dtype == SGPT_F16 ? (int*)m->range_dev : nullptr);
    if (layer_out) pool(apply_final_ln, layer_out + (size_t)n_layers_run * B * dm, nullptr);
    if (layer_mean) launch_mean_over_axis0(layer_out, n_layers_run + 1, (long)B * dm, layer_mean, s);
    HIPC(c, hipGetLastError());
    return SGPT_OK;
}

extern "C" {

sgpt_status sgpt_encode(sgpt_model* m, const int32_t* ids, const int32_t* pos, const int32_t* seq_off,
                        const int32_t* seq_len, const int32_t* pad_left, int32_t B, int32_t T, int32_t max_alloc,
                        int32_t pool_mode, int32_t n_layers_run, int32_t apply_final_ln, int32_t normalize,
                        float* out, float* hidden_out, void* stream) {
    return encode_impl(m, ids, pos, seq_off, seq_len, pad_left, B, T, max_alloc, pool_mode, n_layers_run,
                       apply_final_ln, normalize, out, hidden_out, nullptr, nullptr, stream);
}

sgpt_status sgpt_encode_layers(sgpt_model* m, const int32_t* ids, const int32_t* pos, const int32_t* seq_off,
                               const int32_t* seq_len, const int32_t* pad_left, int32_t B, int32_t T, int32_t max_alloc,
                               int32_t pool_mode, int32_t normalize, float* out_layers, float* out_mean, void* stream) {
    if (!m) return SGPT_ERR_INVALID;
    if (!out_layers && !out_mean) return fail(m->ctx, SGPT_ERR_INVALID, "sgpt_encode_layers: no output requested");
    return encode_impl(m, ids, pos, seq_off, seq_len, pad_left, B, T, max_alloc, pool_mode, m->d.n_layers, 1, normalize,
                       nullptr, nullptr, out_layers, out_mean, stream);
}

sgpt_status sgpt_lm_logprobs(sgpt_model* m, const float* hidden, const int32_t* row_idx, const int32_t* targets,
                             int32_t n, float* out_logprob, int32_t* out_greedy, void* stream) {
    if (!m) return SGPT_ERR_INVALID;
    sgpt_ctx* c = m->ctx;
    if (!hidden || !row_idx || !targets || !out_logprob || n <= 0) return fail(c, SGPT_ERR_INVALID, "sgpt_lm_logprobs: bad arguments");
    if (family(m->d.arch).no_lm) return fail(c, SGPT_ERR_INVALID, std::string("sgpt_lm_logprobs: ") + family(m->d.arch).no_lm);
    HIPC(c, hipSetDevice(c->device));
    hipStream_t s = (hipStream_t)stream;
    const int dm = m->d.d_model, V = m->d.vocab;
    const long ldv = (V + 3) / 4 * 4;
    const int R = n < 1024 ? n : 1024;
    const size_t rows_bytes = align_up((size_t)R * dm * 4, 256), lg_bytes = align_up((size_t)R * ldv * 4, 256);
    sgpt_status st = ensure(c, &c->ws2, &c->ws2_bytes, rows_bytes + lg_bytes);
    if (st != SGPT_OK) return st;
    float* rows = (float*)c->ws2;
    float* logits = (float*)((char*)c->ws2 + rows_bytes);
    for (int r0 = 0; r0 < n; r0 += R) {
        const int nr = (n - r0) < R ? (n - r0) : R;
        launch_gather_rows(hidden, row_idx + r0, nr, dm, rows, s);
        GemmArgs g{};
        g.A = rows; g.lda = dm; g.W = m->lm_w; g.ldw = dm; g.M = nr; g.m_valid = nr; g.N = V; g.K = dm;
        g.out = logits; g.ldo = ldv; g.bias = m->lm_b;
        gemm(c, SGPT_F32, EPI_STORE, SGPT_F32, g, s);
        launch_logprob_rows(logits, ldv, V, targets + r0, nr, out_logprob + r0, out_greedy ? out_greedy + r0 : nullptr, s);
    }
    HIPC(c, hipGetLastError());
    return SGPT_OK;
}

}
```

sgpt_amd/csrc/ops.hip:

```cpp
#include "host.h"

extern "C" {

sgpt_status sgpt_pool(sgpt_ctx* c, const void* hidden, int32_t dtype, const int32_t* mask, int32_t B, int32_t S,
                      int32_t d, int32_t mode, float* out, void* stream) {
    if (!c || !hidden || !mask || !out || B <= 0 || S <= 0 || d <= 0 || d % 4 || mode < 0 || (mode > 2 && mode != SGPT_POOL_CLS))
        return fail(c, SGPT_ERR_INVALID, "sgpt_pool: bad arguments (d % 4 == 0 required; mode 0 | 1 | 2 | 4)");
    HIPC(c, hipSetDevice(c->device));
    launch_pool(hidden, dtype, mask, B, S, d, mode, nullptr, out, (hipStream_t)stream);
    HIPC(c, hipGetLastError());
    return SGPT_OK;
}

sgpt_status sgpt_pool_learnt(sgpt_ctx* c, const void* hidden, int32_t dtype, const int32_t* mask, int32_t B, int32_t S,
                             int32_t d, const float* pos_weights, float* out, void* stream) {
    if (!c || !hidden || !mask || !out || !pos_weights || B <= 0 || S <= 0 || d <= 0 || d % 4)
        return fail(c, SGPT_ERR_INVALID, "sgpt_pool_learnt: bad arguments (d % 4 == 0 required)");
    HIPC(c, hipSetDevice(c->device));
    launch_pool(hidden, dtype, mask, B, S, d, SGPT_POOL_LEARNTMEAN, pos_weights, out, (hipStream_t)stream);
    HIPC(c, hipGetLastError());
    return SGPT_OK;
}

sgpt_status sgpt_fp8_quantize_rows(sgpt_ctx* c, const float* w, int64_t rows, int64_t cols, uint8_t* codes, float* scale,
                                   void* stream) {
    if (!c || !w || !codes || !scale || rows <= 0 || cols <= 0 || cols % 4)
        return fail(c, SGPT_ERR_INVALID, "sgpt_fp8_quantize_rows: bad arguments (cols % 4 == 0 required)");
    HIPC(c, hipSetDevice(c->device));
    launch_fp8_quant_rows(w, rows, cols, codes, scale, (hipStream_t)stream);
    HIPC(c, hipGetLastError());
    return SGPT_OK;
}

sgpt_status sgpt_fp8_dequantize_rows(sgpt_ctx* c, const uint8_t* codes, const float* scale, int64_t rows, int64_t cols,
                                     void* out, int32_t out_dtype, void* stream) {
    if (!c || !codes || !scale || !out || rows <= 0 || cols <= 0 || cols % 4 || (out_dtype != SGPT_F32 && out_dtype != SGPT_BF16 && out_dtype != SGPT_F16))
        return fail(c, SGPT_ERR_INVALID, "sgpt_fp8_dequantize_rows: bad arguments (cols % 4 == 0 required)");
    HIPC(c, hipSetDevice(c->device));
    launch_fp8_dequant_rows(codes, scale, rows, cols, out, out_dtype, (hipStream_t)stream);
    HIPC(c, hipGetLastError());
    return SGPT_OK;
}

sgpt_status sgpt_f32_to_16(sgpt_ctx* c, const float* in, int64_t numel, void* out, int32_t out_dtype, void* stream) {
    if (!c || !in || !out || numel <= 0 || (out_dtype != SGPT_BF16 && out_dtype != SGPT_F16))
        return fail(c, SGPT_ERR_INVALID, "sgpt_f32_to_16: bad arguments");
    HIPC(c, hipSetDevice(c->device));
    launch_f32_to_16(in, numel, out, out_dtype, (hipStream_t)stream);
    HIPC(c, hipGetLastError());
    return SGPT_OK;
}

sgpt_status sgpt_f32_to_bf16(sgpt_ctx* c, const float* in, int64_t numel, void* out, void* stream) {
    return sgpt_f32_to_16(c, in, numel, out, SGPT_BF16, stream);
}

sgpt_status sgpt_layernorm_fp8(sgpt_ctx* c, const float* x, const float* gamma, const float* beta, int32_t T, int32_t d, float eps,
                               uint8_t* codes, float* row_scale, void* stream) {
    if (!c || !x || !gamma || !beta || !codes || !row_scale || T <= 0 || d <= 0 || d % 4 || d > 4096)
        return fail(c, SGPT_ERR_INVALID, "sgpt_layernorm_fp8: bad arguments (d % 4 == 0, d <= 4096)");
    HIPC(c, hipSetDevice(c->device));
    launch_layernorm_q8(x, gamma, beta, codes, row_scale, nullptr, SGPT_BF16, T, d, eps, (hipStream_t)stream);
    HIPC(c, hipGetLastError());
    return SGPT_OK;
}

sgpt_status sgpt_linear_fp8(sgpt_ctx* c, int32_t epi, int32_t out_dtype, const uint8_t* A, const float* a_scale, float a_scalar,
                            const uint8_t* W, const float* w_scale, const float* bias, const float* resid, void* out,
                            float out_scale, int32_t M, int32_t N, int32_t K, void* stream) {
    if (!c || !A || !W || !w_scale || !out || !(a_scalar > 0.f)) return fail(c, SGPT_ERR_INVALID, "sgpt_linear_fp8: bad arguments");
    if (!gemm_fp8_shape_ok(M, N, K)) return fail(c, SGPT_ERR_INVALID, "sgpt_linear_fp8: M, N, K must be multiples of 256");
    if (epi != EPI_BIAS_GELU && epi != EPI_BIAS_RESID && epi != EPI_STORE && epi != EPI_VT)
        return fail(c, SGPT_ERR_INVALID, "sgpt_linear_fp8: epi 0 (store 16-bit), 1 (bias+gelu -> fp8), 2 (bias+residual -> fp32) or 4 (transposed 16-bit)");
    if ((epi == EPI_STORE || epi == EPI_VT) && out_dtype != SGPT_BF16 && out_dtype != SGPT_F16)
        return fail(c, SGPT_ERR_INVALID, "sgpt_linear_fp8: store epilogues write bf16 or f16");
    if ((epi == EPI_BIAS_GELU || epi == EPI_BIAS_RESID) && !bias) return fail(c, SGPT_ERR_INVALID, "sgpt_linear_fp8: bias required");
    if (epi == EPI_BIAS_RESID && !resid) return fail(c, SGPT_ERR_INVALID, "sgpt_linear_fp8: residual required");
    if (epi == EPI_BIAS_GELU && !(out_scale > 0.f)) return fail(c, SGPT_ERR_INVALID, "sgpt_linear_fp8: out_scale required");
    HIPC(c, hipSetDevice(c->device));
    GemmArgs q{};
    q.A = A; q.lda = K; q.W = W; q.ldw = K; q.M = M; q.m_valid = M; q.N = N; q.K = K; q.out = out; q.ldo = epi == EPI_VT ? M : N;
    q.bias = bias; q.resid = resid; q.a_scale = a_scale; q.a_scalar = a_scalar; q.w_scale = w_scale; q.out_scale = out_scale;
    q.range_flag = c->range_flag;
    { Prof pr(c, (hipStream_t)stream, 2.0 * M * (double)N * K); launch_gemm_fp8(epi, out_dtype, q, (hipStream_t)stream); }
    HIPC(c, hipGetLastError());
    return SGPT_OK;
}

sgpt_status sgpt_row_crest(sgpt_ctx* c, const void* x, int32_t dtype, int64_t n, int32_t d, int64_t ld, float* crest_out, void* stream) {
    if (!c || !x || !crest_out || n <= 0 || n > INT32_MAX || d <= 0 || d % 2 || ld < d || (dtype != SGPT_BF16 && dtype != SGPT_F16))
        return fail(c, SGPT_ERR_INVALID, "sgpt_row_crest: bad arguments (16-bit rows, d % 2 == 0)");
    HIPC(c, hipSetDevice(c->device));
    hipStream_t s = (hipStream_t)stream;
    unsigned* slot = (unsigned*)c->range_flag + 16;
    HIPC(c, hipMemsetAsync(slot, 0, 4, s));
    launch_crest16(x, (int)n, d, ld, dtype, slot, s);
    unsigned h = 0;
    HIPC(c, hipMemcpyAsync(&h, slot, 4, hipMemcpyDeviceToHost, s));
    HIPC(c, hipStreamSynchronize(s));
    memcpy(crest_out, &h, 4);
    return SGPT_OK;
}

sgpt_status sgpt_split16(sgpt_ctx* c, const float* in, int64_t n, int32_t d, int32_t layout, void* out, int32_t out_dtype,
                         void* stream) {
    if (!c || !in || !out || n <= 0 || d <= 0 || d % 4 || (layout != 0 && layout != 1) || (out_dtype != SGPT_BF16 && out_dtype != SGPT_F16))
        return fail(c, SGPT_ERR_INVALID, "sgpt_split16: bad arguments (d % 4 == 0, layout 0 | 1, 16-bit out_dtype)");
    HIPC(c, hipSetDevice(c->device));
    launch_split16_rows(in, n, d, layout, out, out_dtype, (hipStream_t)stream);
    HIPC(c, hipGetLastError());
    return SGPT_OK;
}

sgpt_status sgpt_linear(sgpt_ctx* c, int32_t dtype, int32_t epi, int32_t out_dtype, const void* A, const void* W,
                        const float* bias, const float* resid, void* out, int32_t M, int32_t N, int32_t K, void* stream) {
    if (!c || !A || !W || !out || M <= 0 || N <= 0 || K <= 0) return fail(c, SGPT_ERR_INVALID, "sgpt_linear: bad arguments");
    const bool in16 = dtype == SGPT_BF16 || dtype == SGPT_F16, o16 = out_dtype == SGPT_BF16 || out_dtype == SGPT_F16;
    if (!in16 && dtype != SGPT_F32) return fail(c, SGPT_ERR_INVALID, "sgpt_linear: bad dtype");
    if (epi != EPI_STORE && !epi_is_gelu(epi) && epi != EPI_BIAS_RESID && epi != EPI_VT)
        return fail(c, SGPT_ERR_INVALID, "sgpt_linear: epi must be 0 (store), 1 (bias+gelu), 2 (bias+residual), 4 (transposed store) or 9 (bias+erf gelu)");
    if ((epi_is_gelu(epi) || epi == EPI_BIAS_RESID) && !bias) return fail(c, SGPT_ERR_INVALID, "sgpt_linear: bias required");
    if (epi == EPI_BIAS_RESID && (!resid || out_dtype != SGPT_F32)) return fail(c, SGPT_ERR_INVALID, "sgpt_linear: residual epilogue is fp32");
    if (epi == EPI_VT && (!in16 || out_dtype != dtype || M % 128)) return fail(c, SGPT_ERR_INVALID, "sgpt_linear: transposed store is 16-bit, M % 128 == 0");
    if (epi_is_gelu(epi) && out_dtype != dtype) return fail(c, SGPT_ERR_INVALID, "sgpt_linear: gelu output has the operand dtype");
    if (in16 && (o16 ? out_dtype != dtype : false)) return fail(c, SGPT_ERR_INVALID, "sgpt_linear: 16-bit output must match the operand format");
    if (!in16 && o16) return fail(c, SGPT_ERR_INVALID, "sgpt_linear: fp32 operands give fp32 output");
    if (K % (in16 ? 8 : 4) || (epi != EPI_STORE && N % 4)) return fail(c, SGPT_ERR_INVALID, "sgpt_linear: K % 8 (16-bit) / 4 (fp32), N % 4");
    HIPC(c, hipSetDevice(c->device));
    GemmArgs g{};
    g.A = A; g.lda = K; g.W = W; g.ldw = K; g.M = M; g.m_valid = M; g.N = N; g.K = K; g.out = out;
    g.ldo = epi == EPI_VT ? M : N; g.bias = bias; g.resid = resid;
    g.range_flag = out_dtype == SGPT_F16 ? c->range_flag : nullptr;
    gemm(c, dtype, epi, out_dtype, g, (hipStream_t)stream);
    HIPC(c, hipGetLastError());
    return SGPT_OK;
}

sgpt_status sgpt_linear_query(sgpt_ctx* c, int32_t dtype, int32_t epi, const void* A, const float* x, const float* ln_gamma,
                              const float* ln_beta, float ln_eps, const void* W, const float* bias, const float* resid, void* out,
                              void* out_vt, int32_t n_split, int32_t M, int32_t N, int32_t K, void* stream) {
    if (!c || !W || !out || M <= 0 || N <= 0 || K <= 0 || (!A && !x)) return fail(c, SGPT_ERR_INVALID, "sgpt_linear_query: bad arguments");
    if (dtype != SGPT_BF16 && dtype != SGPT_F16) return fail(c, SGPT_ERR_INVALID, "sgpt_linear_query: 16-bit operands (SGPT_BF16 | SGPT_F16)");
    if (epi != EPI_STORE && epi != EPI_BIAS_GELU && epi != EPI_BIAS_RESID && epi != EPI_QKV)
        return fail(c, SGPT_ERR_INVALID, "sgpt_linear_query: epi must be 0 (store), 1 (bias+gelu), 2 (bias+residual) or 7 (q | k | V^T)");
    if (x && (!ln_gamma || !ln_beta || (epi != EPI_QKV && epi != EPI_BIAS_GELU)))
        return fail(c, SGPT_ERR_INVALID, "sgpt_linear_query: the LayerNorm prologue feeds epi 7 (QKV) and 1 (fc1 + GELU) and needs gamma / beta");
    if ((epi == EPI_BIAS_GELU || epi == EPI_BIAS_RESID) && !bias) return fail(c, SGPT_ERR_INVALID, "sgpt_linear_query: bias required");
    if (epi == EPI_BIAS_RESID && !resid) return fail(c, SGPT_ERR_INVALID, "sgpt_linear_query: residual required");
    if (epi == EPI_QKV && (!out_vt || n_split <= 0 || n_split >= N)) return fail(c, SGPT_ERR_INVALID, "sgpt_linear_query: epi 7 needs out_vt and 0 < n_split < N");
    HIPC(c, hipSetDevice(c->device));
    QGemmArgs q{};
    q.g.A = A; q.g.lda = K; q.g.W = W; q.g.ldw = K; q.g.M = M; q.g.m_valid = M; q.g.N = N; q.g.K = K; q.g.out = out;
    q.g.ldo = epi == EPI_QKV ? n_split : N; q.g.out2 = out_vt; q.g.ldo2 = M; q.g.n_split = epi == EPI_QKV ? n_split : 0;
    q.g.bias = bias; q.g.resid = resid;
    const int out_dtype = epi == EPI_BIAS_RESID ? SGPT_F32 : dtype;
    q.g.range_flag = out_dtype == SGPT_F16 ? c->range_flag : nullptr;
    if (x) { q.x = x; q.ln_g = ln_gamma; q.ln_b = ln_beta; q.eps = ln_eps; q.g.A = nullptr; }
    q.tile = c->qtile;
    if (!qgemm(c, dtype, epi, out_dtype, q, (hipStream_t)stream))
        return fail(c, SGPT_ERR_INVALID, "sgpt_linear_query: shape not served by the query-sized kernels (M % 32, M <= 4096; K / 128 a multiple of 4 or 6; "
                                         "N % 16; LayerNorm prologue: K = 512 | 768 | 1024, N % 32)");
    HIPC(c, hipGetLastError());
    return SGPT_OK;
}

sgpt_status sgpt_linear_split(sgpt_ctx* c, int32_t dtype, int32_t epi, const void* A, const void* W, const float* bias, void* out,
                              int64_t ldo, int64_t lo_delta, int64_t hi2_delta, int32_t M, int32_t N, int32_t K, void* stream) {
    if (!c || !A || !W || !out || M <= 0 || N <= 0 || K <= 0 || lo_delta == 0) return fail(c, SGPT_ERR_INVALID, "sgpt_linear_split: bad arguments");
    if (dtype != SGPT_BF16 && dtype != SGPT_F16) return fail(c, SGPT_ERR_INVALID, "sgpt_linear_split: 16-bit operands");
    if (epi != EPI_STORE && epi != EPI_BIAS_GELU && epi != EPI_VT) return fail(c, SGPT_ERR_INVALID, "sgpt_linear_split: epi 0 (store), 1 (bias+gelu) or 4 (transposed store)");
    if (epi == EPI_BIAS_GELU && !bias) return fail(c, SGPT_ERR_INVALID, "sgpt_linear_split: bias required");
    if (epi == EPI_VT && (M % 128 || hi2_delta != 0)) return fail(c, SGPT_ERR_INVALID, "sgpt_linear_split: transposed store needs M % 128 == 0 and writes hi + lo only");
    if (K % 8 || N % 4 || ldo < (epi == EPI_VT ? M : N)) return fail(c, SGPT_ERR_INVALID, "sgpt_linear_split: K % 8, N % 4, ldo >= row length");
    HIPC(c, hipSetDevice(c->device));
    GemmArgs g{};
    g.A = A; g.lda = K; g.W = W; g.ldw = K; g.M = M; g.m_valid = M; g.N = N; g.K = K; g.out = out; g.ldo = ldo; g.bias = bias;
    g.lo_delta = lo_delta; g.hi2_delta = hi2_delta;
    g.range_flag = dtype == SGPT_F16 ? c->range_flag : nullptr;
    gemm(c, dtype, epi, dtype, g, (hipStream_t)stream);
    HIPC(c, hipGetLastError());
    return SGPT_OK;
}

sgpt_status sgpt_linear_qkv(sgpt_ctx* c, int32_t dtype, const void* A, const void* W, void* out, void* out_vt, int32_t n_split,
                            int32_t M, int32_t N, int32_t K, void* stream) {
    if (!c || !A || !W || !out || !out_vt || M <= 0 || N <= 0 || K <= 0 || n_split <= 0) return fail(c, SGPT_ERR_INVALID, "sgpt_linear_qkv: bad arguments");
    if (dtype != SGPT_BF16 && dtype != SGPT_F16) return fail(c, SGPT_ERR_INVALID, "sgpt_linear_qkv: 16-bit operands (SGPT_BF16 | SGPT_F16)");
    if (!gemm_qkv_bulk(M, N, K, n_split, c->force256 != 0))
        return fail(c, SGPT_ERR_INVALID, "sgpt_linear_qkv: not a bulk shape (M, N, n_split % 256; K % 64, K >= 128; 0 < n_split < N; more than "
                                         "half a wave of q | k tiles)");
    HIPC(c, hipSetDevice(c->device));
    GemmArgs g{};
    g.A = A; g.lda = K; g.W = W; g.ldw = K; g.M = M; g.m_valid = M; g.N = N; g.K = K;
    g.out = out; g.ldo = n_split; g.out2 = out_vt; g.ldo2 = M; g.n_split = n_split;
    g.range_flag = dtype == SGPT_F16 ? c->range_flag : nullptr;
    gemm(c, dtype, EPI_QKV, dtype, g, (hipStream_t)stream);
    HIPC(c, hipGetLastError());
    return SGPT_OK;
}

}

static sgpt_status attention_impl(sgpt_ctx* c, int32_t dtype, const void* q, const void* k, const void* v, int64_t ldq, int64_t ldvt,
                              void* out, int64_t ldo, const int32_t* seq_off, int32_t B, int32_t T, int32_t H, int32_t dh,
                              int32_t window, float scale, const float* alibi, int32_t max_alloc_len, int32_t out_fp8,
                              float out_scale, int32_t* range_flag, int32_t x3, int64_t qk_lo_delta, int64_t v_lo_delta,
                              int64_t ctx_lo_delta, int64_t ctx_hi2_delta, int32_t causal, const int32_t* seq_len, int32_t kv_group, const char* who, void* stream) {
    const std::string w = std::string(who) + ": ";
    if (causal != 0 && causal != 1) return fail(c, SGPT_ERR_INVALID, w + "causal 0 | 1");
    if (causal && seq_len) return fail(c, SGPT_ERR_INVALID, w + "seq_len belongs to the bidirectional mode (causal = 0)");
    if (!causal) {
        if (window != 0 || alibi != nullptr) return fail(c, SGPT_ERR_INVALID, w + "bidirectional attention takes no window and no ALiBi");
        if (out_fp8 || x3 || ctx_lo_delta != 0 || ctx_hi2_delta != 0)
            return fail(c, SGPT_ERR_INVALID, w + "out_fp8 and the split-precision modes are causal only");
        if (dtype != SGPT_F32 && dh != 64 && dh != 128) return fail(c, SGPT_ERR_INVALID, w + "16-bit bidirectional attention serves head_dim 64 | 128");
    }
    auto mis = [](const void* p, unsigned a) { return ((uintptr_t)p & (a - 1)) != 0; };
    if (!c || !q || !k || !v || !out || !seq_off || B <= 0 || T <= 0 || H <= 0 || window < 0 || !std::isfinite(scale))
        return fail(c, SGPT_ERR_INVALID, w + "bad arguments");
    const bool in16 = dtype == SGPT_BF16 || dtype == SGPT_F16;
    if (!in16 && dtype != SGPT_F32) return fail(c, SGPT_ERR_INVALID, w + "dtype SGPT_F32 | SGPT_BF16 | SGPT_F16");
    if (dh != 64 && dh != 128 && dh != 256) return fail(c, SGPT_ERR_INVALID, w + "head_dim 64, 128 or 256");
    if (T % 32) return fail(c, SGPT_ERR_INVALID, w + "T % 32 == 0");
    if (max_alloc_len <= 0 || max_alloc_len > 2048 || max_alloc_len % 2)
        return fail(c, SGPT_ERR_INVALID, w + "max_alloc_len even, in [2, 2048]");
    const long d = (long)H * dh;
    if (ldq < d || ldo < d) return fail(c, SGPT_ERR_INVALID, w + "ldq, ldo >= H * head_dim");
    const bool split_ctx = ctx_lo_delta != 0;
    if (!in16 && (out_fp8 || x3 || split_ctx || ctx_hi2_delta))
        return fail(c, SGPT_ERR_INVALID, w + "out_fp8 / x3 / split context are 16-bit modes");
    if (ctx_hi2_delta != 0 && !split_ctx) return fail(c, SGPT_ERR_INVALID, w + "ctx_hi2_delta needs ctx_lo_delta");
    if (out_fp8) {
        if (dtype != SGPT_BF16) return fail(c, SGPT_ERR_INVALID, w + "out_fp8 takes bf16 operands");
        if (x3 || split_ctx) return fail(c, SGPT_ERR_INVALID, w + "out_fp8 with a split-precision mode");
        if (!(out_scale > 0.f) || !std::isfinite(out_scale)) return fail(c, SGPT_ERR_INVALID, w + "out_scale > 0");
    }
    if (x3 && !attn_x3_supported(dh)) return fail(c, SGPT_ERR_INVALID, w + "x3 needs head_dim 64 | 128");
    if (x3 && (qk_lo_delta == 0 || v_lo_delta == 0)) return fail(c, SGPT_ERR_INVALID, w + "x3 needs non-zero lo deltas");
    if (in16) {
        if (mis(q, 16) || mis(k, 16) || mis(v, 4) || mis(out, 16))
            return fail(c, SGPT_ERR_INVALID, w + "16-byte aligned q / k / out, 4-byte aligned V^T");
        if (ldq % 8 || ldo % (out_fp8 ? 16 : 8) || qk_lo_delta % 8 || ctx_lo_delta % 8 || ctx_hi2_delta % 8 || ldvt % 2 || v_lo_delta % 2)
            return fail(c, SGPT_ERR_INVALID, w + "ldq, ldo, qk / ctx deltas % 8 (out_fp8: ldo % 16); ldvt, v_lo_delta even");
        if (ldvt < T) return fail(c, SGPT_ERR_INVALID, w + "ldvt >= T");
    } else if (mis(q, 16) || mis(k, 16) || mis(v, 16) || mis(out, 4) || ldq % 4) {
        return fail(c, SGPT_ERR_INVALID, w + "fp32 q / k / v 16-byte aligned, ldq % 4");
    }
    HIPC(c, hipSetDevice(c->device));
    AttnArgs at{};
    at.q = q; at.k = k; at.v = v; at.ctx = out; at.seq_off = seq_off;
    at.B = B; at.H = H; at.dh = dh; at.ldq = ldq; at.ldvt = ldvt; at.ldo = ldo;
    at.window = window; at.scale = scale; at.max_alloc_len = max_alloc_len; at.alibi = alibi;
    at.dtype = in16 ? dtype : SGPT_F32;
    at.out_fp8 = out_fp8 ? 1 : 0; at.out_scale = out_scale; at.range_flag = range_flag;
    at.x3 = x3 ? 1 : 0; at.qk_lo_delta = qk_lo_delta; at.v_lo_delta = v_lo_delta;
    at.ctx_lo_delta = ctx_lo_delta; at.ctx_hi2_delta = ctx_hi2_delta;
    at.noncausal = causal ? 0 : 1; at.seq_len = seq_len; at.kv_group = kv_group;
    if (in16) launch_attn_bf16(at, (hipStream_t)stream);
    else launch_attn_f32(at, (hipStream_t)stream);
    HIPC(c, hipGetLastError());
    return SGPT_OK;
}

extern "C" {

sgpt_status sgpt_attention_ex(sgpt_ctx* c, int32_t dtype, const void* q, const void* k, const void* v, int64_t ldq, int64_t ldvt,
                              void* out, int64_t ldo, const int32_t* seq_off, int32_t B, int32_t T, int32_t H, int32_t dh,
                              int32_t window, float scale, const float* alibi, int32_t max_alloc_len, int32_t out_fp8,
                              float out_scale, int32_t* range_flag, int32_t x3, int64_t qk_lo_delta, int64_t v_lo_delta,
                              int64_t ctx_lo_delta, int64_t ctx_hi2_delta, int32_t causal, const int32_t* seq_len, void* stream) {
    return attention_impl(c, dtype, q, k, v, ldq, ldvt, out, ldo, seq_off, B, T, H, dh, window, scale, alibi, max_alloc_len, out_fp8,
                          out_scale, range_flag, x3, qk_lo_delta, v_lo_delta, ctx_lo_delta, ctx_hi2_delta, causal, seq_len, 1, "sgpt_attention_ex", stream);
}

sgpt_status sgpt_attention_gqa(sgpt_ctx* c, int32_t dtype, const void* q, const void* k, const void* v, int64_t ldq, int64_t ldvt,
                               void* out, int64_t ldo, const int32_t* seq_off, int32_t B, int32_t T, int32_t H, int32_t n_kv_heads,
                               int32_t dh, int32_t window, float scale, const float* alibi, int32_t max_alloc_len, int32_t out_fp8,
                               float out_scale, int32_t* range_flag, int32_t x3, int64_t qk_lo_delta, int64_t v_lo_delta,
                               int64_t ctx_lo_delta, int64_t ctx_hi2_delta, void* stream) {
    if (H <= 0 || n_kv_heads <= 0 || H % n_kv_heads) return fail(c, SGPT_ERR_INVALID, "sgpt_attention_gqa: n_heads % n_kv_heads == 0, both > 0");
    if (alibi != nullptr) return fail(c, SGPT_ERR_INVALID, "sgpt_attention_gqa: no ALiBi with grouped K / V");
    if (out_fp8 || x3 || ctx_lo_delta != 0 || ctx_hi2_delta != 0)
        return fail(c, SGPT_ERR_INVALID, "sgpt_attention_gqa: out_fp8 and the split-precision modes are not available with grouped K / V");
    if (dtype != SGPT_F32 && dh != 64 && dh != 128) return fail(c, SGPT_ERR_INVALID, "sgpt_attention_gqa: 16-bit grouped attention serves head_dim 64 | 128");
    return attention_impl(c, dtype, q, k, v, ldq, ldvt, out, ldo, seq_off, B, T, H, dh, window, scale, nullptr, max_alloc_len, 0,
                          out_scale, range_flag, 0, qk_lo_delta, v_lo_delta, 0, 0, 1, nullptr, H / n_kv_heads, "sgpt_attention_gqa", stream);
}

sgpt_status sgpt_attention(sgpt_ctx* c, int32_t dtype, const void* q, const void* k, const void* v, int64_t ldq, int64_t ldvt,
                           void* out, int64_t ldo, const int32_t* seq_off, int32_t B, int32_t T, int32_t H, int32_t dh,
                           int32_t window, float scale, const float* alibi, int32_t max_alloc_len, int32_t out_fp8,
                           float out_scale, int32_t* range_flag, int32_t x3, int64_t qk_lo_delta, int64_t v_lo_delta,
                           int64_t ctx_lo_delta, int64_t ctx_hi2_delta, void* stream) {
    return attention_impl(c, dtype, q, k, v, ldq, ldvt, out, ldo, seq_off, B, T, H, dh, window, scale, alibi, max_alloc_len, out_fp8,
                          out_scale, range_flag, x3, qk_lo_delta, v_lo_delta, ctx_lo_delta, ctx_hi2_delta, 1, nullptr, 1, "sgpt_attention", stream);
}

static bool row_width_ok(int32_t d) { return d > 0 && d % 4 == 0 && d <= 4096; }
static bool mis(const void* p, unsigned a) { return ((uintptr_t)p & (a - 1)) != 0; }

sgpt_status sgpt_embed(sgpt_ctx* c, const int32_t* ids, const int32_t* pos, const float* wte, const float* wpe, int32_t T,
                       int32_t d, int32_t vocab, int32_t max_pos, float* out, void* stream) {
    if (!c || !ids || !wte || !out || T <= 0 || d <= 0 || d % 4 || vocab <= 0)
        return fail(c, SGPT_ERR_INVALID, "sgpt_embed: bad arguments (d % 4 == 0 required)");
    if (wpe && (!pos || max_pos <= 0)) return fail(c, SGPT_ERR_INVALID, "sgpt_embed: a position table needs pos and max_pos > 0");
    if (mis(wte, 16) || mis(wpe, 16) || mis(out, 16)) return fail(c, SGPT_ERR_INVALID, "sgpt_embed: 16-byte aligned tables and output");
    HIPC(c, hipSetDevice(c->device));
    launch_embed(ids, pos, wte, wpe, out, T, d, vocab, max_pos, (hipStream_t)stream);
    HIPC(c, hipGetLastError());
    return SGPT_OK;
}
// ... 246 lines not shown
```

sgpt_amd/csrc/qgemm.hip:

```cpp
#include <atomic>
#include <type_traits>

#include "common.h"
#include "rowln.h"

namespace {

constexpr int QNW = 8;
constexpr int QNT = 64 * QNW;
typedef unsigned int qv4 __attribute__((ext_vector_type(4)));

template <typename OutT> __device__ __forceinline__ void q_store4(OutT* p, float a, float b, float c, float d) {
    if constexpr (sizeof(OutT) == 4) *reinterpret_cast<float4*>(p) = make_float4(a, b, c, d);
    else *reinterpret_cast<uint2*>(p) = make_uint2(Half<OutT>::pack2(a, b), Half<OutT>::pack2(c, d));
}
template <typename OutT> struct QRange { typedef RangeTrack<bf16_t> type; };
template <> struct QRange<f16_t> { typedef RangeTrack<f16_t> type; };

template <typename T, int EPI, typename OutT, int BM, int BN, bool LN_A, int NV, int KD, int D>
__global__ __launch_bounds__(QNT) void qgemm_kernel(const QGemmArgs q) {
    const GemmArgs& p = q.g;
    constexpr int ROWB = KD * 2, CPR = KD / 8;
    constexpr int NFM = BM / 16, NFN = BN / 16;
    constexpr int WGN = NFN >= 4 ? 4 : NFN, WGM = QNW / WGN;
    constexpr int FN = NFN / WGN, FM = (NFM + WGM - 1) / WGM;
    static_assert(NFN % WGN == 0 && (NFM % WGM == 0 || NFM < WGM), "tile / wave grid");
    constexpr int A_ROWS = LN_A ? 0 : BM;
    constexpr int STAGE = (A_ROWS + BN) * ROWB;
    constexpr int CH = STAGE / (QNT * 16);
    constexpr int RPJ = QNT / CPR;
    static_assert(STAGE % (QNT * 16) == 0 && CH >= 1 && A_ROWS % RPJ == 0, "a stage is whole slabs; a slab is all A or all W");
    constexpr bool HAS_BIAS = EPI == EPI_BIAS_GELU || EPI == EPI_BIAS_RESID;
    extern __shared__ __attribute__((aligned(16))) char smem[];

    const int K = p.K, nk = K / KD;
    const int G = LN_A ? q.group : 1;
    const int MT = (p.M + BM - 1) / BM, NT = p.N / BN, NG = (NT + G - 1) / G;
    const int R = MT * NG, c0 = R >> 3, rem = R & 7;
    const int xcd = blockIdx.x & 7, local = blockIdx.x >> 3;
    if (local >= c0 + (xcd < rem ? 1 : 0)) return;
    const int gi = xcd * c0 + (xcd < rem ? xcd : rem) + local;
    const int ng = gi / MT, mt = gi - ng * MT;
    const int m0 = mt * BM, nt0 = ng * G;
    const int ntiles = NT - nt0 < G ? NT - nt0 : G;

    const int t = threadIdx.x, lane = t & 63;
    const int wave = __builtin_amdgcn_readfirstlane(t >> 6);
    const int fr = lane & 15, g = lane >> 4;
    const int wn = wave % WGN, wm = wave / WGN;

    const int panel_bytes = LN_A ? nk * BM * ROWB : 0;
    char* const ring = smem + panel_bytes;
    const int bias_off = panel_bytes + 2 * STAGE;

    const char* srcp[CH];
#pragma unroll
    for (int j = 0; j < CH; ++j) {
        const int ci = j * QNT + t;
        const int r = ci / CPR, pos = ci % CPR;
        const int chunk = pos ^ (r & 15);
        if (j * RPJ < A_ROWS) {
            const int row = m0 + r < p.M ? m0 + r : p.M - 1;
            srcp[j] = reinterpret_cast<const char*>(static_cast<const T*>(p.A) + (long)row * p.lda) + chunk * 16;
        } else {
            srcp[j] = reinterpret_cast<const char*>(static_cast<const T*>(p.W) + (long)(nt0 * BN + r - A_ROWS) * p.ldw) + chunk * 16;
        }
    }
    const long wtile = (long)BN * p.ldw * 2;
    qv4 stg[D][CH];
    auto load_into = [&](qv4 (&dst)[CH], int ti, int kt) __attribute__((always_inline)) {
        const long aoff = (long)kt * ROWB, woff = (long)ti * wtile + aoff;
#pragma unroll
        for (int j = 0; j < CH; ++j) dst[j] = *reinterpret_cast<const qv4*>(srcp[j] + (j * RPJ < A_ROWS ? aoff : woff));
    };

    constexpr int RPW = BM / QNW;
    constexpr int RB = RPW > 4 ? 4 : RPW;
    float4 gg[LN_A ? NV : 1], bb[LN_A ? NV : 1];
    RowLN<NV, false> rl[LN_A ? RB : 1];
    auto ln_rows_load = [&](int batch) __attribute__((always_inline)) {
#pragma unroll
        for (int u = 0; u < RB; ++u) {
            const int row = m0 + wave * RPW + batch * RB + u;
            rl[u].load(q.x + (long)(row < p.M ? row : p.M - 1) * K, K, lane);
        }
    };
    float bias_r[2] = {0.f, 0.f};
    if constexpr (LN_A) {
        if (p.bias != nullptr) {
#pragma unroll
            for (int u = 0; u < 2; ++u)
                if (u * QNT + t < ntiles * BN) bias_r[u] = p.bias[nt0 * BN + u * QNT + t];
        }
        ln_rows_load(0);
#pragma unroll
        for (int i = 0; i < NV; ++i) {
            const int c = (i * 64 + lane) * 4;
            gg[i] = c < K ? *reinterpret_cast<const float4*>(q.ln_g + c) : make_float4(0.f, 0.f, 0.f, 0.f);
            bb[i] = c < K ? *reinterpret_cast<const float4*>(q.ln_b + c) : make_float4(0.f, 0.f, 0.f, 0.f);
        }
    }
#pragma unroll
    for (int j = 0; j < D; ++j) {
        load_into(stg[j], 0, j);
        __builtin_amdgcn_sched_barrier(0);
    }

    float4 bpre[FN], rpre[EPI == EPI_BIAS_RESID ? FM : 1][FN];
    if constexpr (!LN_A) {
#pragma unroll
        for (int j = 0; j < FN; ++j) {
            const int n = nt0 * BN + (wn + WGN * j) * 16 + 4 * g;
            bpre[j] = (HAS_BIAS || p.bias != nullptr) ? *reinterpret_cast<const float4*>(p.bias + n) : make_float4(0.f, 0.f, 0.f, 0.f);
            if constexpr (EPI == EPI_BIAS_RESID) {
#pragma unroll
                for (int i = 0; i < FM; ++i) {
                    const int fm = wm + WGM * i;
                    const int m = m0 + (fm < NFM ? fm : 0) * 16 + fr;
                    rpre[i][j] = *reinterpret_cast<const float4*>(p.resid + (long)(m < p.M ? m : p.M - 1) * p.ldo + n);
                }
            }
        }
    }

    if constexpr (LN_A) {
        if (p.bias != nullptr) {
#pragma unroll
            for (int u = 0; u < 2; ++u)
                if (u * QNT + t < ntiles * BN) reinterpret_cast<float*>(smem + bias_off)[u * QNT + t] = bias_r[u];
            for (int i = 2 * QNT + t; i < ntiles * BN; i += QNT) reinterpret_cast<float*>(smem + bias_off)[i] = p.bias[nt0 * BN + i];
        }
#pragma unroll
        for (int batch = 0; batch < RPW / RB; ++batch) {
            if (batch > 0) ln_rows_load(batch);
            rowln_normalize_rows<NV, RB, false>(rl, gg, bb, K, q.eps, lane);
#pragma unroll
            for (int u = 0; u < RB; ++u) {
                const int row = wave * RPW + batch * RB + u;
#pragma unroll
                for (int i = 0; i < NV; ++i) {
                    const int c = (i * 64 + lane) * 4;
                    if (c < K) {
                        const int kt = c / KD, cc = c % KD;
                        const int ch = cc >> 3;
                        const unsigned off = (unsigned)(kt * BM * ROWB + row * ROWB + ((ch ^ (row & 15)) << 4) + ((cc >> 2) & 1) * 8);
                        const uint2 v = make_uint2(Half<T>::pack2(rl[u].v[i].x * q.ln_mul, rl[u].v[i].y * q.ln_mul),
                                                   Half<T>::pack2(rl[u].v[i].z * q.ln_mul, rl[u].v[i].w * q.ln_mul));
                        *reinterpret_cast<uint2_a*>(smem + off) = v;
                    }
                }
            }
        }
    }

    f32x4 acc[FM][FN];
    int par = 0;
    auto stage = [&](qv4 (&reg)[CH], int kt, auto load_tag, int lti, int lkt, auto swap_tag) __attribute__((always_inline)) {
        constexpr bool SW = decltype(swap_tag)::value;
        char* const st = ring + par * STAGE;
#pragma unroll
        for (int j = 0; j < CH; ++j) *reinterpret_cast<qv4*>(st + (j * QNT + t) * 16) = reg[j];
        if constexpr (decltype(load_tag)::value) load_into(reg, lti, lkt);
        __syncthreads();
        const char* ab = LN_A ? smem + kt * BM * ROWB : st;
        const char* wb = st + A_ROWS * ROWB;
#pragma unroll
        for (int ks = 0; ks < KD / 32; ++ks) {
            uint4 af[FM], wf[FN];
            const int co = ((4 * ks + g) ^ fr) << 4;
#pragma unroll
            for (int i = 0; i < FM; ++i) {
                const int fm = wm + WGM * i;
                af[i] = *reinterpret_cast<const uint4_a*>(ab + ((fm < NFM ? fm : 0) * 16 + fr) * ROWB + co);
            }
#pragma unroll
            for (int j = 0; j < FN; ++j) wf[j] = *reinterpret_cast<const uint4_a*>(wb + ((wn + WGN * j) * 16 + fr) * ROWB + co);
#pragma unroll
            for (int i = 0; i < FM; ++i)
#pragma unroll
                for (int j = 0; j < FN; ++j) {
                    if constexpr (SW) acc[i][j] = Half<T>::mfma16(wf[j], af[i], acc[i][j]);
                    else acc[i][j] = Half<T>::mfma16(af[i], wf[j], acc[i][j]);
                }
        }
        par ^= 1;
    };
    auto group = [&](int kt0, auto load_tag, int lti, int lkt0, auto swap_tag) __attribute__((always_inline)) {
#pragma unroll
        for (int j = 0; j < D; ++j) stage(stg[j], kt0 + j, load_tag, lti, lkt0 + j, swap_tag);
    };
    auto ktile = [&](int ti, auto swap_tag) __attribute__((always_inline)) {
#pragma unroll
        for (int i = 0; i < FM; ++i)
#pragma unroll
            for (int j = 0; j < FN; ++j) acc[i][j] = f32x4{0.f, 0.f, 0.f, 0.f};
        int kt0 = 0;
        for (; kt0 + D < nk; kt0 += D) group(kt0, std::true_type{}, ti, kt0 + D, swap_tag);
        if (ti + 1 < ntiles) group(kt0, std::true_type{}, ti + 1, 0, swap_tag);
        else group(kt0, std::false_type{}, 0, 0, swap_tag);
    };

    typename QRange<OutT>::type range;
    for (int ti = 0; ti < ntiles; ++ti) {
        const int n0 = (nt0 + ti) * BN;
        const bool vt_tile = EPI == EPI_QKV && n0 >= p.n_split;
        if (vt_tile) ktile(ti, std::false_type{}); else ktile(ti, std::true_type{});
        if (vt_tile) {
            if constexpr (EPI == EPI_QKV) {
                OutT* __restrict__ vt = static_cast<OutT*>(p.out2);
                const float csv = p.in_mul * p.out_mul2;
#pragma unroll
                for (int j = 0; j < FN; ++j) {
                    const int nl = (wn + WGN * j) * 16 + fr, n = n0 + nl;
                    float bn = 0.f;
                    if (p.bias != nullptr) bn = (LN_A ? reinterpret_cast<const float*>(smem + bias_off)[ti * BN + nl] : p.bias[n]) * p.out_mul2;
#pragma unroll
                    for (int i = 0; i < FM; ++i) {
                        const int fm = wm + WGM * i;
                        if (fm >= NFM) continue;
                        const int m = m0 + fm * 16 + 4 * g;
                        if (m >= p.M) continue;
                        const float v0 = __builtin_fmaf(acc[i][j][0], csv, bn), v1 = __builtin_fmaf(acc[i][j][1], csv, bn);
                        const float v2 = __builtin_fmaf(acc[i][j][2], csv, bn), v3 = __builtin_fmaf(acc[i][j][3], csv, bn);
                        range.note(v0, v1); range.note(v2, v3);
                        q_store4<OutT>(vt + (long)(n - p.n_split) * p.ldo2 + m, v0, v1, v2, v3);
                    }
                }
            }
        } else {
            OutT* __restrict__ out = static_cast<OutT*>(p.out);
            const float om = p.out_mul;
            const float cs = HAS_BIAS ? p.in_mul : p.in_mul * om;
            const float bsc = EPI == EPI_BIAS_GELU ? 1.0f : om;
#pragma unroll
            for (int i = 0; i < FM; ++i) {
                const int fm = wm + WGM * i;
                if (fm >= NFM) continue;
                const int m = m0 + fm * 16 + fr;
                if (m >= p.M) continue;
#pragma unroll
                for (int j = 0; j < FN; ++j) {
                    const int nl = (wn + WGN * j) * 16 + 4 * g, n = n0 + nl;
                    float v[4] = {acc[i][j][0], acc[i][j][1], acc[i][j][2], acc[i][j][3]};
                    float4 bb4 = make_float4(0.f, 0.f, 0.f, 0.f);
                    if constexpr (LN_A) {
                        if (HAS_BIAS || p.bias != nullptr) bb4 = *reinterpret_cast<const float4_a*>(smem + bias_off + (ti * BN + nl) * 4);
                    } else {
                        bb4 = bpre[j];
                    }
                    if constexpr (EPI == EPI_BIAS_RESID) {
                        const float4 rr = rpre[i][j];
                        v[0] = __builtin_fmaf(v[0], cs, bb4.x + rr.x); v[1] = __builtin_fmaf(v[1], cs, bb4.y + rr.y);
                        v[2] = __builtin_fmaf(v[2], cs, bb4.z + rr.z); v[3] = __builtin_fmaf(v[3], cs, bb4.w + rr.w);
                    } else if (EPI == EPI_BIAS_GELU || p.bias != nullptr) {
                        v[0] = __builtin_fmaf(v[0], cs, bb4.x * bsc); v[1] = __builtin_fmaf(v[1], cs, bb4.y * bsc);
                        v[2] = __builtin_fmaf(v[2], cs, bb4.z * bsc); v[3] = __builtin_fmaf(v[3], cs, bb4.w * bsc);
                    } else if constexpr (sizeof(OutT) == 2) {
#pragma unroll
                        for (int r = 0; r < 4; ++r) v[r] = __builtin_fmaf(v[r], cs, 0.f);
                    }
                    if constexpr (EPI == EPI_BIAS_GELU) {
                        const float ginv = 1.0f / om;
#pragma unroll
                        for (int r = 0; r < 4; ++r) v[r] = gelu_new_fast_scaled(v[r], ginv);
                    }
                    range.note(v[0], v[1]); range.note(v[2], v[3]);
                    q_store4<OutT>(out + (long)m * p.ldo + n, v[0], v[1], v[2], v[3]);
                }
            }
        }
    }
    range.finish(p.range_flag, p.range_amax);
}

constexpr int q_chunks(int bm, int bn, bool ln_a, int kd) { return ((ln_a ? 0 : bm) + bn) * kd * 2 / (QNT * 16); }
constexpr int q_depth_rule(int ch, bool six) { return ch >= 8 ? 2 : six ? (ch * 6 <= 24 ? 6 : 3) : (ch * 4 <= 16 ? 4 : 2); }
template <int BM, int BN, bool LN_A, int KD, bool SIX>
constexpr int q_depth() { return q_depth_rule(q_chunks(BM, BN, LN_A, KD), SIX); }

template <typename T, int EPI, typename OutT, int BM, int BN, bool LN_A, int NV, int KD, int D>
void qlaunch(const QGemmArgs& a, int group, hipStream_t s) {
    auto* kern = qgemm_kernel<T, EPI, OutT, BM, BN, LN_A, NV, KD, D>;
    static std::atomic<unsigned> attr_done{0u};
    int dev = 0;
    (void)hipGetDevice(&dev);
    const unsigned bit = 1u << (dev & 31);
    if (!(attr_done.load(std::memory_order_relaxed) & bit)) {
        (void)hipFuncSetAttribute(reinterpret_cast<const void*>(kern), hipFuncAttributeMaxDynamicSharedMemorySize, 160 * 1024);
        attr_done.fetch_or(bit, std::memory_order_relaxed);
    }
    QGemmArgs b = a;
    b.group = group;
    const int nk = a.g.K / KD;
    const size_t lds = (size_t)(LN_A ? nk * BM * KD * 2 + group * BN * 4 : 0) + (size_t)2 * ((LN_A ? 0 : BM) + BN) * KD * 2;
    const int NT = a.g.N / BN, R = ((a.g.M + BM - 1) / BM) * ((NT + group - 1) / group);
    hipLaunchKernelGGL(kern, dim3(8 * ((R + 7) / 8)), dim3(QNT), lds, s, b);
}

inline int q_ncu() {
    static const int ncu = [] {
        int dev = 0, n = 256;
        (void)hipGetDevice(&dev);
        (void)hipDeviceGetAttribute(&n, hipDeviceAttributeMultiprocessorCount, dev);
        return n;
    }();
    return ncu;
}

struct QTile { int bm, bn, kd; };
constexpr QTile Q_TILES[] = {{32, 16, 256}, {32, 32, 128}, {32, 64, 128}, {64, 32, 128}, {64, 64, 128}, {128, 64, 128}, {128, 128, 128}};
constexpr int Q_NTILES = sizeof(Q_TILES) / sizeof(Q_TILES[0]);

inline int q_class(const QTile& tl, bool ln_a, int K) {
    if (K % tl.kd) return 0;
    const int nk = K / tl.kd;
    const int ch = q_chunks(tl.bm, tl.bn, ln_a, tl.kd);
    const int d6 = q_depth_rule(ch, true), d4 = q_depth_rule(ch, false);
    const bool ok6 = nk % d6 == 0, ok4 = nk % d4 == 0;
    if (ok6 && (!ok4 || d6 >= d4)) return 6;
    return ok4 ? 4 : 0;
}

inline int q_pick_plain(int M, int N, int K, int epi, int n_split, int force = 0) {
    const int ncu = q_ncu();
    int best = -1; long best_cost = 0;
    for (int i = 0; i < Q_NTILES; ++i) {
        const QTile& tl = Q_TILES[i];
        if (force > 0 && i != force - 1) continue;
        if (N % tl.bn || !q_class(tl, false, K)) continue;
        if (epi == EPI_QKV && (n_split % tl.bn || tl.bn < 16)) continue;
        if (tl.bm > 32 && M <= 32) continue;
        const long tiles = (long)((M + tl.bm - 1) / tl.bm) * (N / tl.bn);
        const long rounds = (tiles + ncu - 1) / ncu;
        const long cost = rounds * (tl.bm + tl.bn);
        if (best < 0 || cost < best_cost || (cost == best_cost && tl.bm * tl.bn > Q_TILES[best].bm * Q_TILES[best].bn)) { best = i; best_cost = cost; }
    }
    return best;
}

template <typename T, int EPI, typename OutT, int BM, int BN, int KD>
bool qrun_plain(const QGemmArgs& a, int cls, hipStream_t s) {
    if (cls == 6) qlaunch<T, EPI, OutT, BM, BN, false, 1, KD, q_depth<BM, BN, false, KD, true>()>(a, 1, s);
    else qlaunch<T, EPI, OutT, BM, BN, false, 1, KD, q_depth<BM, BN, false, KD, false>()>(a, 1, s);
    return true;
}

template <typename T, int EPI, typename OutT>
bool qdispatch_plain(const QGemmArgs& a, int epi, hipStream_t s) {
    const int i = q_pick_plain(a.g.M, a.g.N, a.g.K, epi, a.g.n_split, a.tile);
    if (i < 0) return false;
    const int cls = q_class(Q_TILES[i], false, a.g.K);
    switch (i) {
        case 0: return qrun_plain<T, EPI, OutT, 32, 16, 256>(a, cls, s);
        case 1: return qrun_plain<T, EPI, OutT, 32, 32, 128>(a, cls, s);
        case 2: return qrun_plain<T, EPI, OutT, 32, 64, 128>(a, cls, s);
        case 3: return qrun_plain<T, EPI, OutT, 64, 32, 128>(a, cls, s);
        case 4: return qrun_plain<T, EPI, OutT, 64, 64, 128>(a, cls, s);
        case 5: return qrun_plain<T, EPI, OutT, 128, 64, 128>(a, cls, s);
        case 6: return qrun_plain<T, EPI, OutT, 128, 128, 128>(a, cls, s);
    }
    return false;
}

struct QLnPlan { int bm, bn, group; };
inline bool q_plan_ln(int M, int N, int d, int epi, int n_split, QLnPlan* out, int force = 0) {
    if (d % 128 || N % 32) return false;
    const int nk = d / 128;
    if (nk % 6 != 0 && nk % 4 != 0) return false;
    const int ncu = q_ncu();
    QLnPlan best{0, 0, 0}; long best_cost = 0;
    const int cands[3][2] = {{32, 32}, {32, 64}, {64, 64}};
    for (int ci = 0; ci < 3; ++ci) {
        const int* c = cands[ci];
        if (force > 0 && ci != force - 1) continue;
        const int bm = c[0], bn = c[1];
        if (N % bn || (epi == EPI_QKV && n_split % bn)) continue;
        if (bm > 32 && M <= 32) continue;
        const int mt = (M + bm - 1) / bm, nt = N / bn;
        int gq = (int)(((long)mt * nt + ncu - 1) / ncu);
        gq = gq < 1 ? 1 : gq;
        while ((long)mt * ((nt + gq - 1) / gq) > ncu) ++gq;
        const long lds = (long)nk * bm * 256 + 2l * bn * 256 + (long)gq * bn * 4;
        if (lds > 160 * 1024) continue;
        const long cost = (bm == 32 ? 6200 : 9400) + (long)gq * nk * (bn == 32 ? 250 : bm == 32 ? 350 : 440);
        if (best.bm == 0 || cost < best_cost) { best = QLnPlan{bm, bn, gq}; best_cost = cost; }
    }
    if (best.bm == 0) return false;
    *out = best;
    return true;
}

template <typename T, int EPI, typename OutT, int NV, bool SIX>
bool qdispatch_ln(const QGemmArgs& a, const QLnPlan& pl, hipStream_t s) {
    if (pl.bm == 32 && pl.bn == 32) qlaunch<T, EPI, OutT, 32, 32, true, NV, 128, q_depth<32, 32, true, 128, SIX>()>(a, pl.group, s);
    else if (pl.bm == 32 && pl.bn == 64) qlaunch<T, EPI, OutT, 32, 64, true, NV, 128, q_depth<32, 64, true, 128, SIX>()>(a, pl.group, s);
    else if (pl.bm == 64 && pl.bn == 64) qlaunch<T, EPI, OutT, 64, 64, true, NV, 128, q_depth<64, 64, true, 128, SIX>()>(a, pl.group, s);
    else return false;
    return true;
}

template <typename T>
bool qgemm16(int epi, int out_dtype, const QGemmArgs& a, hipStream_t s) {
    const bool o16 = dt_is16(out_dtype);
    if (a.x != nullptr) {
        const int d = a.g.K;
        QLnPlan pl;
        if (!o16 || !q_plan_ln(a.g.M, a.g.N, d, epi, a.g.n_split, &pl, a.tile)) return false;
        const bool six = (d / 128) % 6 == 0;
#define QLN(NVV)                                                                                                          \
        do {                                                                                                               \
            if (epi == EPI_QKV) return six ? qdispatch_ln<T, EPI_QKV, T, NVV, true>(a, pl, s) : qdispatch_ln<T, EPI_QKV, T, NVV, false>(a, pl, s);   \
            if (epi == EPI_BIAS_GELU) return six ? qdispatch_ln<T, EPI_BIAS_GELU, T, NVV, true>(a, pl, s) : qdispatch_ln<T, EPI_BIAS_GELU, T, NVV, false>(a, pl, s); \
            return false;                                                                                                  \
        } while (0)
        if (d == 768) QLN(3);
        if (d == 1024 || d == 512) QLN(4);
        return false;
#undef QLN
    }
    if (epi == EPI_STORE && o16) return qdispatch_plain<T, EPI_STORE, T>(a, epi, s);
    if (epi == EPI_STORE && !o16) return qdispatch_plain<T, EPI_STORE, float>(a, epi, s);
    if (epi == EPI_QKV && o16) return qdispatch_plain<T, EPI_QKV, T>(a, epi, s);
    if (epi == EPI_BIAS_GELU && o16) return qdispatch_plain<T, EPI_BIAS_GELU, T>(a, epi, s);
    if (epi == EPI_BIAS_RESID && !o16) return qdispatch_plain<T, EPI_BIAS_RESID, float>(a, epi, s);
    return false;
}

}

bool qgemm_shape_ok(int M, int N, int K, int epi, int n_split) {
    if (M <= 0 || M > QGEMM_MAX_ROWS || M % 32 || K < 128 || N % 16) return false;
    if (epi == EPI_QKV && (n_split % 32 || n_split <= 0 || n_split >= N || N % 32)) return false;
    if (!(epi == EPI_STORE || epi == EPI_QKV || epi == EPI_BIAS_GELU || epi == EPI_BIAS_RESID)) return false;
    return q_pick_plain(M, N, K, epi, n_split) >= 0;
}

bool qgemm_ln_ok(int M, int N, int d, int epi, int n_split) {
    if (M <= 0 || M > QGEMM_MAX_ROWS || M % 32 || (epi != EPI_QKV && epi != EPI_BIAS_GELU)) return false;
    if (epi == EPI_QKV && (n_split % 32 || n_split <= 0 || n_split >= N)) return false;
    if (d != 768 && d != 1024 && d != 512) return false;
    QLnPlan pl;
    return q_plan_ln(M, N, d, epi, n_split, &pl);
}

bool launch_qgemm(int dtype, int epi, int out_dtype, const QGemmArgs& a0, hipStream_t s) {
    QGemmArgs a = a0;
    if (a.g.in_mul == 0.f) a.g.in_mul = 1.f;
    if (a.g.out_mul == 0.f) a.g.out_mul = 1.f;
    if (a.g.out_mul2 == 0.f) a.g.out_mul2 = 1.f;
    if (a.ln_mul == 0.f) a.ln_mul = 1.f;
    if (a.g.lo_delta != 0 || a.g.lo_delta2 != 0 || a.g.hi2_delta != 0 || a.g.m_valid != a.g.M || a.g.pred != nullptr) return false;
    if (a.x != nullptr ? !qgemm_ln_ok(a.g.M, a.g.N, a.g.K, epi, a.g.n_split) : !qgemm_shape_ok(a.g.M, a.g.N, a.g.K, epi, a.g.n_split)) return false;
    if (dtype == DT_BF16) return qgemm16<bf16_t>(epi, out_dtype, a, s);
    if (dtype == DT_F16) return qgemm16<f16_t>(epi, out_dtype, a, s);
    return false;
}
```

sgpt_amd/runtime.py:

```python
import ctypes as C
from dataclasses import dataclass
from typing import Optional, Tuple

import numpy as np
import torch

from . import _lib
from ._lib import SGPT_BF16, SGPT_F16, SGPT_F32, POOL_MODES

DT_CODE = {torch.float32: SGPT_F32, torch.bfloat16: SGPT_BF16, torch.float16: SGPT_F16}


def _stream_ptr(device) -> C.c_void_p:
    return C.c_void_p(torch.cuda.current_stream(device).cuda_stream)


def _p(t: Optional[torch.Tensor]) -> C.c_void_p:
    return C.c_void_p(0 if t is None else t.data_ptr())


@dataclass
class QuantizedCorpus:
    codes: torch.Tensor
    scale: torch.Tensor
    normalized: bool = True
    dim: Optional[int] = None

    def __len__(self) -> int:
        return int(self.codes.shape[0])

    @property
    def nbytes(self) -> int:
        return self.codes.numel() * self.codes.element_size() + self.scale.numel() * self.scale.element_size()

    def dequantize(self, dtype=torch.float32) -> torch.Tensor:
        return get_context(self.codes.device).fp8_dequantize_rows(self.codes, self.scale, out_dtype=dtype)


_contexts = {}


def get_context(device=None) -> "Context":
    if not torch.cuda.is_available():
        raise _lib.SgptHipError("no HIP device visible: sgpt_amd runs its hot path only as gfx950 kernels "
                                "(there is no CPU path)")
    dev = torch.device("cuda", torch.cuda.current_device()) if device is None else torch.device(device)
    if dev.type != "cuda":
        raise _lib.SgptHipError(f"sgpt_amd needs a HIP device, got {dev}")
    idx = dev.index if dev.index is not None else torch.cuda.current_device()
    if idx not in _contexts:
        _contexts[idx] = Context(idx)
    return _contexts[idx]


class Context:
    def __init__(self, device_index: int):
        self.lib = _lib.load()
        self.device = torch.device("cuda", device_index)
        h = C.c_void_p()
        st = self.lib.sgpt_ctx_create(device_index, C.byref(h))
        if st != 0:
            raise _lib.SgptHipError(f"sgpt_ctx_create(device={device_index}) failed with status {st}")
        self.handle = h

    def close(self):
        if getattr(self, "handle", None):
            self.lib.sgpt_ctx_destroy(self.handle)
            self.handle = None

    def _chk(self, st, what):
        _lib.check(self.handle, st, what)

    def _dev_f32(self, a) -> torch.Tensor:
        if not isinstance(a, torch.Tensor):
            a = torch.as_tensor(np.asarray(a))
        if a.dim() == 1:
            a = a.unsqueeze(0)
        return a.to(device=self.device, dtype=torch.float32).contiguous()

    def pool(self, hidden: torch.Tensor, mask: torch.Tensor, mode: str = "weightedmean",
             position_weights: Optional[torch.Tensor] = None) -> torch.Tensor:
        if mode not in POOL_MODES:
            raise ValueError(f"unknown pooling mode {mode}")
        hidden = hidden.to(self.device)
        if hidden.dtype not in DT_CODE:
            hidden = hidden.float()
        hidden = hidden.contiguous()
        B, S, d = hidden.shape
        m = mask.to(device=self.device, dtype=torch.int32).contiguous()
        out = torch.empty((B, d), dtype=torch.float32, device=self.device)
        dt = DT_CODE[hidden.dtype]
        if mode == "learntmean":
            if position_weights is None or position_weights.numel() < S:
                raise ValueError("learntmean needs position_weights covering the sequence length")
            pw = position_weights.to(device=self.device, dtype=torch.float32).contiguous()
            self._chk(self.lib.sgpt_pool_learnt(self.handle, _p(hidden), dt, _p(m), B, S, d, _p(pw), _p(out),
                                                _stream_ptr(self.device)), "sgpt_pool_learnt")
            return out
        self._chk(self.lib.sgpt_pool(self.handle, _p(hidden), dt, _p(m), B, S, d, POOL_MODES[mode], _p(out),
                                     _stream_ptr(self.device)), "sgpt_pool")
        return out

    def l2_normalize(self, x: torch.Tensor, out_dtype=torch.float32) -> torch.Tensor:
        x = self._dev_f32(x)
        n, d = x.shape
        out = torch.empty((n, d), dtype=out_dtype, device=self.device)
        self._chk(self.lib.sgpt_l2_normalize(self.handle, _p(x), n, d, _p(out), DT_CODE[out_dtype],
                                             _stream_ptr(self.device)), "sgpt_l2_normalize")
        return out

    def pairwise_scores(self, a: torch.Tensor, b: torch.Tensor, cosine: bool) -> torch.Tensor:
        a, b = self._dev_f32(a), self._dev_f32(b)
        if a.shape != b.shape or a.dim() != 2:
            raise ValueError(f"pairwise scores need two [n, d] matrices of one shape, got {tuple(a.shape)} and {tuple(b.shape)}")
        n, d = a.shape
        out = torch.empty((n,), dtype=torch.float32, device=self.device)
        if n:
            self._chk(self.lib.sgpt_pairwise_scores(self.handle, _p(a), _p(b), n, d, 1 if cosine else 0, _p(out),
                                                    _stream_ptr(self.device)), "sgpt_pairwise_scores")
        return out

    def to_16(self, x: torch.Tensor, dtype=torch.float16, out: Optional[torch.Tensor] = None) -> torch.Tensor:
        x = x.to(device=self.device, dtype=torch.float32).contiguous()
        if out is None:
            out = torch.empty(x.shape, dtype=dtype, device=self.device)
        self._chk(self.lib.sgpt_f32_to_16(self.handle, _p(x), x.numel(), _p(out), DT_CODE[dtype],
                                          _stream_ptr(self.device)), "sgpt_f32_to_16")
        return out

    def row_crest(self, x: torch.Tensor) -> float:
        if x.dtype not in (torch.float16, torch.bfloat16):
            x = self.to_16(self._dev_f32(x), torch.float16)
        x = x.to(self.device).contiguous()
        n, d = x.shape
        out = C.c_float(0)
        self._chk(self.lib.sgpt_row_crest(self.handle, _p(x), DT_CODE[x.dtype], n, d, d, C.byref(out),
                                          _stream_ptr(self.device)), "sgpt_row_crest")
        return float(out.value)

    def split16(self, x: torch.Tensor, role: str, dtype=torch.float16) -> torch.Tensor:
        if role not in ("doc", "query"):
            raise ValueError("role must be 'doc' or 'query'")
        x = self._dev_f32(x)
        n, d = x.shape
        out = torch.empty((n, 3 * d), dtype=dtype, device=self.device)
        self._chk(self.lib.sgpt_split16(self.handle, _p(x), n, d, 0 if role == "doc" else 1, _p(out), DT_CODE[dtype],
                                        _stream_ptr(self.device)), "sgpt_split16")
        return out

    def to_bf16(self, x: torch.Tensor) -> torch.Tensor:
        return self.to_16(x, torch.bfloat16)

    def range_check(self, reset: bool = True) -> int:
        flagged = C.c_int32(0)
        self._chk(self.lib.sgpt_range_check(self.handle, C.byref(flagged), 1 if reset else 0, _stream_ptr(self.device)),
                  "sgpt_range_check")
        return int(flagged.value)

    def generation(self) -> int:
        return int(self.lib.sgpt_ctx_generation(self.handle))

    def set_low_latency(self, on: bool) -> bool:
        return bool(self.lib.sgpt_ctx_set_low_latency(self.handle, 1 if on else 0))

    def set_gemm_cu_cap(self, n: int) -> int:
        return int(self.lib.sgpt_ctx_set_gemm_cu_cap(self.handle, int(n)))

    def set_tile_policy(self, force_256) -> int:
        return int(self.lib.sgpt_ctx_set_tile_policy(self.handle, int(force_256)))

    def set_query_tile(self, k: int) -> int:
        return int(self.lib.sgpt_ctx_set_query_tile(self.handle, int(k)))

    def reserve(self, encode_bytes: int = 0, score_bytes: int = 0) -> None:
        self._chk(self.lib.sgpt_ctx_reserve(self.handle, encode_bytes, score_bytes), "sgpt_ctx_reserve")

    def fp8_quantize_rows(self, w: torch.Tensor) -> Tuple[torch.Tensor, torch.Tensor]:
        w = w.to(device=self.device, dtype=torch.float32).contiguous()
        rows, cols = w.shape
        codes = torch.empty((rows, cols), dtype=torch.uint8, device=self.device)
        scale = torch.empty((rows,), dtype=torch.float32, device=self.device)
        self._chk(self.lib.sgpt_fp8_quantize_rows(self.handle, _p(w), rows, cols, _p(codes), _p(scale),
                                                  _stream_ptr(self.device)), "sgpt_fp8_quantize_rows")
        return codes, scale

    def fp8_dequantize_rows(self, codes: torch.Tensor, scale: torch.Tensor, out_dtype=torch.float32) -> torch.Tensor:
        codes = codes.to(device=self.device, dtype=torch.uint8).contiguous()
        scale = scale.to(device=self.device, dtype=torch.float32).contiguous()
        rows, cols = codes.shape
        out = torch.empty((rows, cols), dtype=out_dtype, device=self.device)
        self._chk(self.lib.sgpt_fp8_dequantize_rows(self.handle, _p(codes), _p(scale), rows, cols, _p(out),
                                                    DT_CODE[out_dtype],
                                                    _stream_ptr(self.device)), "sgpt_fp8_dequantize_rows")
        return out

    def quantize_corpus(self, emb, normalize: bool = True, block_rows: int = 65536) -> QuantizedCorpus:
        if not isinstance(emb, torch.Tensor):
            emb = torch.as_tensor(np.asarray(emb))
        if emb.dim() != 2 or emb.shape[0] == 0 or emb.shape[1] == 0:
            raise ValueError(f"quantize_corpus needs a non-empty [N, d] matrix, got {tuple(emb.shape)}")
        N, d0 = emb.shape
        d = (d0 + 7) // 8 * 8
        codes = torch.empty((N, d), dtype=torch.uint8, device=self.device)
        scale = torch.empty((N,), dtype=torch.float32, device=self.device)
        for r0 in range(0, N, block_rows):
            n = min(block_rows, N - r0)
            blk = self._dev_f32(emb[r0:r0 + n])
            if normalize:
                blk = self.l2_normalize(blk)
            if d != d0:
                blk = torch.nn.functional.pad(blk, (0, d - d0))
            self._chk(self.lib.sgpt_fp8_quantize_rows(self.handle, _p(blk), n, d, _p(codes[r0:r0 + n]), _p(scale[r0:r0 + n]),
                                                      _stream_ptr(self.device)), "sgpt_fp8_quantize_rows")
        return QuantizedCorpus(codes, scale, bool(normalize), d0)

    def _operand(self, x: torch.Tensor, dtype) -> torch.Tensor:
        if x.dtype == dtype and x.device == self.device and x.is_contiguous():
            return x
        if dtype in (torch.bfloat16, torch.float16):
            return self.to_16(x, dtype)
        return x.to(device=self.device, dtype=torch.float32).contiguous()

    def linear(self, a: torch.Tensor, w: torch.Tensor, bias: Optional[torch.Tensor] = None, epi: str = "store",
               resid: Optional[torch.Tensor] = None, out_dtype=None) -> torch.Tensor:
        code = {"store": 0, "gelu": 1, "resid": 2, "vt": 4, "gelu_erf": 9}[epi]
        M, K = a.shape
        N = w.shape[0]
        if out_dtype is None:
            out_dtype = torch.float32 if epi == "resid" else a.dtype
        out = torch.empty((N, M) if epi == "vt" else (M, N), dtype=out_dtype, device=self.device)
        b = None if bias is None else bias.to(device=self.device, dtype=torch.float32).contiguous()
        r = None if resid is None else resid.to(device=self.device, dtype=torch.float32).contiguous()
        self._chk(self.lib.sgpt_linear(self.handle, DT_CODE[a.dtype], code, DT_CODE[out_dtype], _p(a.contiguous()),
                                       _p(w.contiguous()), _p(b), _p(r), _p(out), M, N, K, _stream_ptr(self.device)),
                  "sgpt_linear")
        return out

    def linear_query(self, w: torch.Tensor, a: Optional[torch.Tensor] = None, x: Optional[torch.Tensor] = None, ln=None,
                     bias: Optional[torch.Tensor] = None, epi: str = "store", resid: Optional[torch.Tensor] = None, n_split: int = 0):
        code = {"store": 0, "gelu": 1, "resid": 2, "qkv": 7}[epi]
        N, K = w.shape
        src = a if a is not None else x
        M = src.shape[0]
        odt = torch.float32 if epi == "resid" else w.dtype
        out = torch.empty((M, n_split if epi == "qkv" else N), dtype=odt, device=self.device)
        vt = torch.empty((N - n_split, M), dtype=odt, device=self.device) if epi == "qkv" else None
        f32 = lambda t_: None if t_ is None else t_.to(device=self.device, dtype=torch.float32).contiguous()
        g, b, eps = (f32(ln[0]), f32(ln[1]), float(ln[2])) if ln is not None else (None, None, 0.0)
        b32, r32, x32 = f32(bias), f32(resid), f32(x)
        self._chk(self.lib.sgpt_linear_query(self.handle, DT_CODE[w.dtype], code, _p(None if a is None else a.contiguous()), _p(x32), _p(g), _p(b), eps,
                                             _p(w.contiguous()), _p(b32), _p(r32), _p(out), _p(vt), int(n_split), M, N, K,
                                             _stream_ptr(self.device)), "sgpt_linear_query")
        return (out, vt) if epi == "qkv" else out

    def linear_qkv(self, a: torch.Tensor, w: torch.Tensor, n_split: int):
        M, K = a.shape
        N = w.shape[0]
        out = torch.empty((M, n_split), dtype=a.dtype, device=self.device)
        vt = torch.empty((N - n_split, M), dtype=a.dtype, device=self.device)
        self._chk(self.lib.sgpt_linear_qkv(self.handle, DT_CODE[a.dtype], _p(a.contiguous()), _p(w.contiguous()), _p(out), _p(vt),
                                           int(n_split), M, N, K, _stream_ptr(self.device)), "sgpt_linear_qkv")
        return out, vt

    def linear_split(self, a: torch.Tensor, w: torch.Tensor, bias: Optional[torch.Tensor] = None, epi: str = "store",
                     triple: bool = False) -> torch.Tensor:
        code = {"store": 0, "gelu": 1, "vt": 4}[epi]
        M, K = a.shape
        N = w.shape[0]
        b = None if bias is None else bias.to(device=self.device, dtype=torch.float32).contiguous()
        if epi == "vt":
            out = torch.zeros((2, N, M), dtype=a.dtype, device=self.device)
            ldo, lo, hi2 = M, N * M, 0
        else:
            out = torch.zeros((M, (3 if triple else 2) * N), dtype=a.dtype, device=self.device)
            ldo, lo, hi2 = out.shape[1], N, (2 * N if triple else 0)
        self._chk(self.lib.sgpt_linear_split(self.handle, DT_CODE[a.dtype], code, _p(a.contiguous()), _p(w.contiguous()), _p(b),
                                             _p(out), ldo, lo, hi2, M, N, K, _stream_ptr(self.device)), "sgpt_linear_split")
        return out

    def attention(self, q: torch.Tensor, k: torch.Tensor, v: torch.Tensor, out: torch.Tensor, seq_off: torch.Tensor,
                  H: int, dh: int, max_alloc_len: int, window: int = 0, scale: float = 1.0, alibi: Optional[torch.Tensor] = None,
                  out_scale: float = 0.0, range_flag: Optional[torch.Tensor] = None, x3: bool = False, qk_lo_delta: int = 0,
                  v_lo_delta: int = 0, ctx_lo_delta: int = 0, ctx_hi2_delta: int = 0, causal: Optional[bool] = None,
                  seq_len: Optional[torch.Tensor] = None, n_kv_heads: Optional[int] = None) -> torch.Tensor:
        T = q.shape[0]
        out_fp8 = out.dtype == torch.uint8
        if q.dtype not in DT_CODE:
            raise ValueError(f"attention: operands are fp32, bf16 or f16, got {q.dtype}")
        if k.stride(0) != q.stride(0) or q.stride(1) != 1 or k.stride(1) != 1 or v.stride(1) != 1 or out.stride(1) != 1:
            raise ValueError("attention: q and k share one leading dimension; unit column strides")
        if k.dtype != q.dtype or v.dtype != q.dtype:
            raise ValueError("attention: q, k and v have one dtype")
        if out.dtype != q.dtype and not (out_fp8 and q.dtype == torch.bfloat16):
            raise ValueError("attention: out has q's dtype (or uint8 e4m3 codes for bf16 operands)")
        if q.dtype == torch.float32 and v.stride(0) != q.stride(0):
            raise ValueError("attention: fp32 v rows share q's leading dimension (the fp32 kernel reads v with ldq)")
        so = seq_off.to(device=self.device, dtype=torch.int32).contiguous()
        al = None if alibi is None else alibi.to(device=self.device, dtype=torch.float32).contiguous()
        if n_kv_heads is not None:
            if causal is False or seq_len is not None:
                raise ValueError("attention: grouped K / V is causal")
            self._chk(self.lib.sgpt_attention_gqa(self.handle, DT_CODE[q.dtype], _p(q), _p(k), _p(v), q.stride(0), v.stride(0), _p(out),
                                                  out.stride(0), _p(so), so.numel() - 1, T, H, int(n_kv_heads), dh, window, scale, _p(al),
                                                  max_alloc_len, 1 if out_fp8 else 0, out_scale, _p(range_flag), 1 if x3 else 0,
                                                  qk_lo_delta, v_lo_delta, ctx_lo_delta, ctx_hi2_delta, _stream_ptr(self.device)),
                      "sgpt_attention_gqa")
            return out
        if causal is not None:
            sl = None if seq_len is None else seq_len.to(device=self.device, dtype=torch.int32).contiguous()
            self._chk(self.lib.sgpt_attention_ex(self.handle, DT_CODE[q.dtype], _p(q), _p(k), _p(v), q.stride(0), v.stride(0), _p(out),
                                                 out.stride(0), _p(so), so.numel() - 1, T, H, dh, window, scale, _p(al), max_alloc_len,
                                                 1 if out_fp8 else 0, out_scale, _p(range_flag), 1 if x3 else 0, qk_lo_delta,
                                                 v_lo_delta, ctx_lo_delta, ctx_hi2_delta, 1 if causal else 0, _p(sl),
                                                 _stream_ptr(self.device)), "sgpt_attention_ex")
            return out
        self._chk(self.lib.sgpt_attention(self.handle, DT_CODE[q.dtype], _p(q), _p(k), _p(v), q.stride(0), v.stride(0), _p(out),
                                          out.stride(0), _p(so), so.numel() - 1, T, H, dh, window, scale, _p(al), max_alloc_len,
                                          1 if out_fp8 else 0, out_scale, _p(range_flag), 1 if x3 else 0, qk_lo_delta,
                                          v_lo_delta, ctx_lo_delta, ctx_hi2_delta, _stream_ptr(self.device)), "sgpt_attention")
        return out

    def _f32c(self, t: Optional[torch.Tensor]) -> Optional[torch.Tensor]:
        return None if t is None else t.to(device=self.device, dtype=torch.float32).contiguous()

    def embed(self, ids: torch.Tensor, pos: Optional[torch.Tensor], wte: torch.Tensor, wpe: Optional[torch.Tensor] = None,
# ... 382 lines not shown
```

Before: 37460.

## Add cost-model tile planner with larger query-GEMM tiles and per-GEMM LN fusion choice

Moves the query-GEMM tile selection into a shared planner that scores candidates with a nanosecond cost model (fixed overhead plus bytes per round). It adds larger tiles (96, 160 and 192 rows) and an XCD-aware block remap for the QKV kernel that specialises the V-transpose path at compile time. LayerNorm fusion into the GEMM prologue is now decided separately for QKV and FC1 by comparing fused against unfused cost, so a standalone LayerNorm launch may be used where the model predicts it is cheaper. Risks include mis-calibrated cost constants, more template instantiations, and larger tiles lowering occupancy.

```diff
diff --git a/include/sgpt_hip.h b/include/sgpt_hip.h
--- a/include/sgpt_hip.h
+++ b/include/sgpt_hip.h
@@ -8,7 +8,7 @@
 extern "C" {
 #endif
 
-#define SGPT_ABI_VERSION 18
+#define SGPT_ABI_VERSION 19
 
 typedef int sgpt_status;
 #define SGPT_OK 0
@@ -252,6 +252,7 @@
 int32_t sgpt_ctx_set_low_latency(sgpt_ctx* ctx, int32_t on);
 int32_t sgpt_ctx_set_tile_policy(sgpt_ctx* ctx, int32_t policy);
 int32_t sgpt_ctx_set_query_tile(sgpt_ctx* ctx, int32_t k);
+int32_t sgpt_ctx_set_query_tile_shape(sgpt_ctx* ctx, int32_t bm, int32_t bn);
 
 sgpt_status sgpt_bench_gemm(sgpt_ctx* ctx, int32_t dtype, int32_t epi, int32_t out_dtype,
                             int32_t M, int32_t N, int32_t K, int32_t iters, float* ms_out);
diff --git a/sgpt_amd/_lib.py b/sgpt_amd/_lib.py
--- a/sgpt_amd/_lib.py
+++ b/sgpt_amd/_lib.py
@@ -5,7 +5,7 @@
 LIB_PATH = os.environ.get("SGPT_HIP_LIB") or os.path.join(HERE, "lib", "libsgpt_hip.so")
 
 SGPT_F32, SGPT_BF16, SGPT_FP8W, SGPT_F16, SGPT_FP8M = 0, 1, 2, 3, 4
-SGPT_ABI_VERSION = 18
+SGPT_ABI_VERSION = 19
 SGPT_PREC_CLASSES = 5
 PC_LN1, PC_ATT, PC_CTX, PC_LN2, PC_H = 0, 1, 2, 3, 4
 SGPT_ERR_RANGE = -5
@@ -116,6 +116,7 @@
     "sgpt_ctx_set_tile_policy": (C.c_int32, [C.c_void_p, C.c_int32]),
     "sgpt_ctx_set_gemm_cu_cap": (C.c_int32, [C.c_void_p, C.c_int32]),
     "sgpt_ctx_set_query_tile": (C.c_int32, [C.c_void_p, C.c_int32]),
+    "sgpt_ctx_set_query_tile_shape": (C.c_int32, [C.c_void_p, C.c_int32, C.c_int32]),
     "sgpt_model_range_check": (C.c_int, [C.c_void_p, C.POINTER(C.c_int32), C.c_int32, C.c_void_p]),
     "sgpt_model_range_adapt": (C.c_int, [C.c_void_p, C.POINTER(C.c_int32), C.c_void_p]),
     "sgpt_model_get_range_shifts": (C.c_int, [C.c_void_p, C.c_void_p, C.c_int32]),
diff --git a/sgpt_amd/csrc/common.h b/sgpt_amd/csrc/common.h
--- a/sgpt_amd/csrc/common.h
+++ b/sgpt_amd/csrc/common.h
@@ -256,9 +256,11 @@
     float eps, ln_mul;
     int group;
     int tile;
+    int tile_bm, tile_bn;
 };
 bool qgemm_shape_ok(int M, int N, int K, int epi, int n_split);
 bool qgemm_ln_ok(int M, int N, int d, int epi, int n_split);
+bool qgemm_ln_fused(int M, int N, int d, int epi, int n_split);
 bool launch_qgemm(int dtype, int epi, int out_dtype, const QGemmArgs& a, hipStream_t s);
 
 bool gemm_qkv_one_launch(int M, int n_split, bool force256);
diff --git a/sgpt_amd/csrc/ctx.h b/sgpt_amd/csrc/ctx.h
--- a/sgpt_amd/csrc/ctx.h
+++ b/sgpt_amd/csrc/ctx.h
@@ -22,6 +22,7 @@
     int force256 = 0;
     int no_qpath = 0;
     int cu_cap = 0;
+    int qtile_bm = 0, qtile_bn = 0;
     int qtile = 0;
     bool prof = false;
     std::vector<std::pair<hipEvent_t, hipEvent_t>> ev_pool;
diff --git a/sgpt_amd/csrc/ctx.hip b/sgpt_amd/csrc/ctx.hip
--- a/sgpt_amd/csrc/ctx.hip
+++ b/sgpt_amd/csrc/ctx.hip
@@ -135,6 +135,14 @@
     if (!c || k < 0 || k > 7) return -1;
     const int old = c->qtile;
     c->qtile = k;
+    if (k > 0) c->qtile_bm = c->qtile_bn = 0;
+    return old;
+}
+int32_t sgpt_ctx_set_query_tile_shape(sgpt_ctx* c, int32_t bm, int32_t bn) {
+    if (!c || bm < 0 || bn < 0 || bm > 0xffff || bn > 0xffff || (bm == 0) != (bn == 0)) return -1;
+    const int old = (c->qtile_bm << 16) | c->qtile_bn;
+    c->qtile_bm = bm; c->qtile_bn = bn;
+    if (bm > 0) c->qtile = 0;
     return old;
 }
 #ifdef SGPT_EXPERIMENTS
diff --git a/sgpt_amd/csrc/encode.hip b/sgpt_amd/csrc/encode.hip
--- a/sgpt_amd/csrc/encode.hip
+++ b/sgpt_amd/csrc/encode.hip
@@ -10,7 +10,7 @@
     int d_q, d_kv;
     int dt;
     int* range_flag;
-    bool can_split, any_ln, any_att, any_ctx, any_h, split, fp8, mlp8, qpath, qln;
+    bool can_split, any_ln, any_att, any_ctx, any_h, split, fp8, mlp8, qpath, qln_qkv, qln_fc1;
     float* x;
     void *a, *ctx, *qkv, *vt, *h;
     void* gu;
@@ -172,11 +172,11 @@
     return SGPT_OK;
 }
 
-void block_ln(const Fwd& f, QGemmArgs& q, const float* g, const float* b, int k, bool split, unsigned* crest) {
+void block_ln(const Fwd& f, QGemmArgs& q, bool fused, const float* g, const float* b, int k, bool split, unsigned* crest) {
     const int dm = f.m->d.d_model;
     const float eps = f.m->d.ln_eps;
     q.eps = eps;
-    if (f.qln) { q.x = f.x; q.ln_g = g; q.ln_b = b; q.ln_mul = pow2f(-k); return; }
+    if (fused) { q.x = f.x; q.ln_g = g; q.ln_b = b; q.ln_mul = pow2f(-k); return; }
     if (split) launch_layernorm_split(f.x, g, b, f.a, f.dt, f.T, dm, eps, f.s, pow2f(-k));
     else launch_layernorm(f.x, g, b, f.a, f.dt, f.T, dm, eps, f.s, pow2f(-k));
     if (crest) launch_crest16(f.a, f.T, dm, q.g.lda, f.dt, crest, f.s);
@@ -209,7 +209,7 @@
         q.g = proj(f, f.a, lda1, l.w_qkv, 3 * dm, dm, f.qkv, 2 * dm, l.b_qkv);
         q.g.in_mul = pow2f(k_ln1); q.g.out_mul = q.g.out_mul2 = pow2f(-k_qkv); q.g.range_amax = f16m ? slots + RS_QKV : nullptr;
         q.g.lo_delta = q.g.lo_delta2 = p_att ? f.att_lo : 0;
-        block_ln(f, q, l.ln1_g, l.ln1_b, k_ln1, p_ln1 != 0, crest ? crest + RS_LN1 : nullptr);
+        block_ln(f, q, f.qln_qkv, l.ln1_g, l.ln1_b, k_ln1, p_ln1 != 0, crest ? crest + RS_LN1 : nullptr);
         if (f.qpath || ((p_ln1 == 0 || p_ln1 == 2) && gemm_qkv_one_launch(T, 2 * dm, c->force256 != 0)) ||
             (p_ln1 == 0 && !p_att && l.b_qkv == nullptr && gemm_qkv_bulk(T, 3 * dm, dm, 2 * dm, c->force256 != 0))) {
             if (p_ln1 == 2) split_w(q.g, l.w_qkv3, dm);
@@ -240,7 +240,7 @@
         if (p_ln2) split_w(q.g, l.w_fc3, dm);
         if (p_h) { q.g.lo_delta = ffn; q.g.hi2_delta = 2 * ffn; }
         q.g.in_mul = pow2f(k_ln2); q.g.out_mul = pow2f(-k_h); q.g.range_amax = f16m ? slots + RS_H : nullptr;
-        if (!gptj) block_ln(f, q, l.ln2_g, l.ln2_b, k_ln2, p_ln2, crest ? crest + RS_LN2 : nullptr);
+        if (!gptj) block_ln(f, q, f.qln_fc1, l.ln2_g, l.ln2_b, k_ln2, p_ln2, crest ? crest + RS_LN2 : nullptr);
         if ((st = launch16(f, EPI_BIAS_GELU, dt, q, "fc1")) != SGPT_OK) return st;
     }
     if (crest) launch_crest16(f.h, T, ffn, ldh, dt, crest + RS_H, s);
@@ -308,7 +308,8 @@
     f.qpath = bf && !f.fp8 && !f.split && f.F->qpath && !(m->probing && m->crest_dev) && !m->calibrating && !c->force256 && !c->no_qpath && T <= QGEMM_MAX_ROWS &&
               qgemm_shape_ok(T, 3 * dm, dm, EPI_QKV, 2 * dm) && qgemm_shape_ok(T, dm, dm, EPI_BIAS_RESID, 0) &&
               qgemm_shape_ok(T, ffn, dm, EPI_BIAS_GELU, 0) && qgemm_shape_ok(T, dm, ffn, EPI_BIAS_RESID, 0);
-    f.qln = f.qpath && !gptj && qgemm_ln_ok(T, 3 * dm, dm, EPI_QKV, 2 * dm) && qgemm_ln_ok(T, ffn, dm, EPI_BIAS_GELU, 0);
+    f.qln_qkv = f.qpath && !gptj && qgemm_ln_fused(T, 3 * dm, dm, EPI_QKV, 2 * dm);
+    f.qln_fc1 = f.qpath && !gptj && qgemm_ln_fused(T, ffn, dm, EPI_BIAS_GELU, 0);
     size_t off = 0;
     auto carve = [&](size_t bytes) { size_t o = off; off = align_up(off + bytes, 256); return o; };
     const size_t o_x = carve((size_t)T * dm * 4);
@@ -344,7 +345,7 @@
             HIPC(c, hipMemsetAsync((bf16_t*)f.vt + lo + T * dkv, 0, SLACK * dkv * esz, f.s));
         }
     else if (f.F->slack_f32) HIPC(c, hipMemsetAsync((float*)f.qkv + T * (dq + 2 * dkv), 0, SLACK * (dq + 2 * dkv) * esz, f.s));
-    if (f.m->d.arch == SGPT_ARCH_GPTJ || f.mlp8 || f.split || f.qln || (f.F->post_ln && !f.vt))
+    if (f.m->d.arch == SGPT_ARCH_GPTJ || f.mlp8 || f.split || f.qln_qkv || (f.F->post_ln && !f.vt))
         HIPC(c, hipMemsetAsync(f.ctx, 0, T * dm * esz * (f.any_ctx ? 3 : 1), f.s));
     else if (dq > dm) HIPC(c, hipMemsetAsync(f.ctx, 0, T * dq * esz, f.s));
     return SGPT_OK;
diff --git a/sgpt_amd/csrc/ops.hip b/sgpt_amd/csrc/ops.hip
--- a/sgpt_amd/csrc/ops.hip
+++ b/sgpt_amd/csrc/ops.hip
@@ -157,6 +157,7 @@
     q.g.range_flag = out_dtype == SGPT_F16 ? c->range_flag : nullptr;
     if (x) { q.x = x; q.ln_g = ln_gamma; q.ln_b = ln_beta; q.eps = ln_eps; q.g.A = nullptr; }
     q.tile = c->qtile;
+    q.tile_bm = c->qtile_bm; q.tile_bn = c->qtile_bn;
     if (!qgemm(c, dtype, epi, out_dtype, q, (hipStream_t)stream))
         return fail(c, SGPT_ERR_INVALID, "sgpt_linear_query: shape not served by the query-sized kernels (M % 32, M <= 4096; K / 128 a multiple of 4 or 6; "
                                          "N % 16; LayerNorm prologue: K = 512 | 768 | 1024, N % 32)");
diff --git a/sgpt_amd/csrc/qgemm.hip b/sgpt_amd/csrc/qgemm.hip
--- a/sgpt_amd/csrc/qgemm.hip
+++ b/sgpt_amd/csrc/qgemm.hip
@@ -2,12 +2,16 @@
 #include <type_traits>
 
 #include "common.h"
+#include "qplan.h"
 #include "rowln.h"
 
 namespace {
+
+using namespace qplan;
 
 constexpr int QNW = 8;
 constexpr int QNT = 64 * QNW;
+static_assert(QNT == Q_THREADS, "qplan.h counts chunks per thread");
 typedef unsigned int qv4 __attribute__((ext_vector_type(4)));
 
 template <typename OutT> __device__ __forceinline__ void q_store4(OutT* p, float a, float b, float c, float d) {
@@ -17,8 +21,8 @@
 template <typename OutT> struct QRange { typedef RangeTrack<bf16_t> type; };
 template <> struct QRange<f16_t> { typedef RangeTrack<f16_t> type; };
 
-template <typename T, int EPI, typename OutT, int BM, int BN, bool LN_A, int NV, int KD, int D>
-__global__ __launch_bounds__(QNT) void qgemm_kernel(const QGemmArgs q) {
+template <typename T, int EPI, typename OutT, int BM, int BN, bool LN_A, int NV, int KD, int D, int VT>
+__device__ __forceinline__ void qgemm_body(const QGemmArgs& q) {
     const GemmArgs& p = q.g;
     constexpr int ROWB = KD * 2, CPR = KD / 8;
     constexpr int NFM = BM / 16, NFN = BN / 16;
@@ -203,7 +207,7 @@
     typename QRange<OutT>::type range;
     for (int ti = 0; ti < ntiles; ++ti) {
         const int n0 = (nt0 + ti) * BN;
-        const bool vt_tile = EPI == EPI_QKV && n0 >= p.n_split;
+        const bool vt_tile = VT >= 0 ? VT == 1 : EPI == EPI_QKV && n0 >= p.n_split;
         if (vt_tile) ktile(ti, std::false_type{}); else ktile(ti, std::true_type{});
         if (vt_tile) {
             if constexpr (EPI == EPI_QKV) {
@@ -273,20 +277,35 @@
     range.finish(p.range_flag, p.range_amax);
 }
 
-constexpr int q_chunks(int bm, int bn, bool ln_a, int kd) { return ((ln_a ? 0 : bm) + bn) * kd * 2 / (QNT * 16); }
-constexpr int q_depth_rule(int ch, bool six) { return ch >= 8 ? 2 : six ? (ch * 6 <= 24 ? 6 : 3) : (ch * 4 <= 16 ? 4 : 2); }
+template <typename T, int EPI, typename OutT, int BM, int BN, bool LN_A, int NV, int KD, int D>
+__global__ __launch_bounds__(QNT) void qgemm_kernel(const QGemmArgs q) {
+    if constexpr (EPI == EPI_QKV && !LN_A && (BM == 96 || BM > 128)) {
+        const int MT = (q.g.M + BM - 1) / BM, R = MT * (q.g.N / BN), c0 = R >> 3, rem = R & 7;
+        const int xcd = blockIdx.x & 7, local = blockIdx.x >> 3;
+        if (local >= c0 + (xcd < rem ? 1 : 0)) return;
+        const int gi = xcd * c0 + (xcd < rem ? xcd : rem) + local;
+        if ((gi / MT) * BN >= q.g.n_split) qgemm_body<T, EPI, OutT, BM, BN, LN_A, NV, KD, D, 1>(q);
+        else qgemm_body<T, EPI, OutT, BM, BN, LN_A, NV, KD, D, 0>(q);
+    } else {
+        qgemm_body<T, EPI, OutT, BM, BN, LN_A, NV, KD, D, -1>(q);
+    }
+}
+
 template <int BM, int BN, bool LN_A, int KD, bool SIX>
 constexpr int q_depth() { return q_depth_rule(q_chunks(BM, BN, LN_A, KD), SIX); }
 
 template <typename T, int EPI, typename OutT, int BM, int BN, bool LN_A, int NV, int KD, int D>
-void qlaunch(const QGemmArgs& a, int group, hipStream_t s) {
+bool qlaunch(const QGemmArgs& a, int group, hipStream_t s) {
     auto* kern = qgemm_kernel<T, EPI, OutT, BM, BN, LN_A, NV, KD, D>;
     static std::atomic<unsigned> attr_done{0u};
     int dev = 0;
     (void)hipGetDevice(&dev);
     const unsigned bit = 1u << (dev & 31);
     if (!(attr_done.load(std::memory_order_relaxed) & bit)) {
-        (void)hipFuncSetAttribute(reinterpret_cast<const void*>(kern), hipFuncAttributeMaxDynamicSharedMemorySize, 160 * 1024);
+        if (hipFuncSetAttribute(reinterpret_cast<const void*>(kern), hipFuncAttributeMaxDynamicSharedMemorySize, (int)Q_LDS_LIMIT) != hipSuccess) {
+            (void)hipGetLastError();
+            return false;
+        }
         attr_done.fetch_or(bit, std::memory_order_relaxed);
     }
     QGemmArgs b = a;
@@ -295,108 +314,61 @@
     const size_t lds = (size_t)(LN_A ? nk * BM * KD * 2 + group * BN * 4 : 0) + (size_t)2 * ((LN_A ? 0 : BM) + BN) * KD * 2;
     const int NT = a.g.N / BN, R = ((a.g.M + BM - 1) / BM) * ((NT + group - 1) / group);
     hipLaunchKernelGGL(kern, dim3(8 * ((R + 7) / 8)), dim3(QNT), lds, s, b);
+    return true;
 }
 
 inline int q_ncu() {
     static const int ncu = [] {
         int dev = 0, n = 256;
         (void)hipGetDevice(&dev);
-        (void)hipDeviceGetAttribute(&n, hipDeviceAttributeMultiprocessorCount, dev);
-        return n;
+        if (hipDeviceGetAttribute(&n, hipDeviceAttributeMultiprocessorCount, dev) != hipSuccess) n = 256;
+        return n < 1 ? 1 : n;
     }();
     return ncu;
 }
-
-struct QTile { int bm, bn, kd; };
-constexpr QTile Q_TILES[] = {{32, 16, 256}, {32, 32, 128}, {32, 64, 128}, {64, 32, 128}, {64, 64, 128}, {128, 64, 128}, {128, 128, 128}};
-constexpr int Q_NTILES = sizeof(Q_TILES) / sizeof(Q_TILES[0]);
-
-inline int q_class(const QTile& tl, bool ln_a, int K) {
-    if (K % tl.kd) return 0;
-    const int nk = K / tl.kd;
-    const int ch = q_chunks(tl.bm, tl.bn, ln_a, tl.kd);
-    const int d6 = q_depth_rule(ch, true), d4 = q_depth_rule(ch, false);
-    const bool ok6 = nk % d6 == 0, ok4 = nk % d4 == 0;
-    if (ok6 && (!ok4 || d6 >= d4)) return 6;
-    return ok4 ? 4 : 0;
-}
-
-inline int q_pick_plain(int M, int N, int K, int epi, int n_split, int force = 0) {
-    const int ncu = q_ncu();
-    int best = -1; long best_cost = 0;
-    for (int i = 0; i < Q_NTILES; ++i) {
-        const QTile& tl = Q_TILES[i];
-        if (force > 0 && i != force - 1) continue;
-        if (N % tl.bn || !q_class(tl, false, K)) continue;
-        if (epi == EPI_QKV && (n_split % tl.bn || tl.bn < 16)) continue;
-        if (tl.bm > 32 && M <= 32) continue;
-        const long tiles = (long)((M + tl.bm - 1) / tl.bm) * (N / tl.bn);
-        const long rounds = (tiles + ncu - 1) / ncu;
-        const long cost = rounds * (tl.bm + tl.bn);
-        if (best < 0 || cost < best_cost || (cost == best_cost && tl.bm * tl.bn > Q_TILES[best].bm * Q_TILES[best].bn)) { best = i; best_cost = cost; }
-    }
-    return best;
-}
+inline QForce q_force(const QGemmArgs& a) { return QForce{a.tile, a.tile_bm, a.tile_bn}; }
+inline int q_kind(int epi) { return epi == EPI_QKV ? Q_KIND_QKV : epi == EPI_BIAS_RESID ? Q_KIND_RESID : Q_KIND_OTHER; }
 
 template <typename T, int EPI, typename OutT, int BM, int BN, int KD>
 bool qrun_plain(const QGemmArgs& a, int cls, hipStream_t s) {
-    if (cls == 6) qlaunch<T, EPI, OutT, BM, BN, false, 1, KD, q_depth<BM, BN, false, KD, true>()>(a, 1, s);
-    else qlaunch<T, EPI, OutT, BM, BN, false, 1, KD, q_depth<BM, BN, false, KD, false>()>(a, 1, s);
-    return true;
+    constexpr int D6 = q_depth<BM, BN, false, KD, true>(), D4 = q_depth<BM, BN, false, KD, false>();
+    if constexpr (D6 == D4) return qlaunch<T, EPI, OutT, BM, BN, false, 1, KD, D6>(a, 1, s);
+    else return cls == 6 ? qlaunch<T, EPI, OutT, BM, BN, false, 1, KD, D6>(a, 1, s) : qlaunch<T, EPI, OutT, BM, BN, false, 1, KD, D4>(a, 1, s);
 }
 
 template <typename T, int EPI, typename OutT>
 bool qdispatch_plain(const QGemmArgs& a, int epi, hipStream_t s) {
-    const int i = q_pick_plain(a.g.M, a.g.N, a.g.K, epi, a.g.n_split, a.tile);
-    if (i < 0) return false;
-    const int cls = q_class(Q_TILES[i], false, a.g.K);
-    switch (i) {
-        case 0: return qrun_plain<T, EPI, OutT, 32, 16, 256>(a, cls, s);
-        case 1: return qrun_plain<T, EPI, OutT, 32, 32, 128>(a, cls, s);
-        case 2: return qrun_plain<T, EPI, OutT, 32, 64, 128>(a, cls, s);
-        case 3: return qrun_plain<T, EPI, OutT, 64, 32, 128>(a, cls, s);
-        case 4: return qrun_plain<T, EPI, OutT, 64, 64, 128>(a, cls, s);
-        case 5: return qrun_plain<T, EPI, OutT, 128, 64, 128>(a, cls, s);
-        case 6: return qrun_plain<T, EPI, OutT, 128, 128, 128>(a, cls, s);
-    }
+    QPlainPlan pl;
+    if (!q_pick_plain(a.g.M, a.g.N, a.g.K, q_kind(epi), a.g.n_split, q_ncu(), &pl, q_force(a))) return false;
+    const int cls = q_class(Q_TILES[pl.tile], false, a.g.K);
+#define QPLAIN(I, BM, BN, KD)                                                                                             \
+        case I: static_assert(Q_TILES[I].bm == BM && Q_TILES[I].bn == BN && Q_TILES[I].kd == KD, "the planner's candidate list"); \
+                if constexpr (EPI == EPI_BIAS_RESID && Q_TILES[I].no_resid) return false;                              \
+                else return qrun_plain<T, EPI, OutT, BM, BN, KD>(a, cls, s)
+    switch (pl.tile) {
+        QPLAIN(0, 32, 16, 256);
+        QPLAIN(1, 32, 32, 128);
+        QPLAIN(2, 32, 64, 128);
+        QPLAIN(3, 64, 32, 128);
+        QPLAIN(4, 64, 64, 128);
+        QPLAIN(5, 128, 64, 128);
+        QPLAIN(6, 128, 128, 128);
+        QPLAIN(7, 96, 64, 128);
+        QPLAIN(8, 96, 128, 128);
+        QPLAIN(9, 160, 128, 128);
+        QPLAIN(10, 192, 128, 128);
+    }
+#undef QPLAIN
+    static_assert(Q_NTILES == 11, "one case per candidate");
     return false;
-}
-
-struct QLnPlan { int bm, bn, group; };
-inline bool q_plan_ln(int M, int N, int d, int epi, int n_split, QLnPlan* out, int force = 0) {
-    if (d % 128 || N % 32) return false;
-    const int nk = d / 128;
-    if (nk % 6 != 0 && nk % 4 != 0) return false;
-    const int ncu = q_ncu();
-    QLnPlan best{0, 0, 0}; long best_cost = 0;
-    const int cands[3][2] = {{32, 32}, {32, 64}, {64, 64}};
-    for (int ci = 0; ci < 3; ++ci) {
-        const int* c = cands[ci];
-        if (force > 0 && ci != force - 1) continue;
-        const int bm = c[0], bn = c[1];
-        if (N % bn || (epi == EPI_QKV && n_split % bn)) continue;
-        if (bm > 32 && M <= 32) continue;
-        const int mt = (M + bm - 1) / bm, nt = N / bn;
-        int gq = (int)(((long)mt * nt + ncu - 1) / ncu);
-        gq = gq < 1 ? 1 : gq;
-        while ((long)mt * ((nt + gq - 1) / gq) > ncu) ++gq;
-        const long lds = (long)nk * bm * 256 + 2l * bn * 256 + (long)gq * bn * 4;
-        if (lds > 160 * 1024) continue;
-        const long cost = (bm == 32 ? 6200 : 9400) + (long)gq * nk * (bn == 32 ? 250 : bm == 32 ? 350 : 440);
-        if (best.bm == 0 || cost < best_cost) { best = QLnPlan{bm, bn, gq}; best_cost = cost; }
-    }
-    if (best.bm == 0) return false;
-    *out = best;
-    return true;
 }
 
 template <typename T, int EPI, typename OutT, int NV, bool SIX>
 bool qdispatch_ln(const QGemmArgs& a, const QLnPlan& pl, hipStream_t s) {
-    if (pl.bm == 32 && pl.bn == 32) qlaunch<T, EPI, OutT, 32, 32, true, NV, 128, q_depth<32, 32, true, 128, SIX>()>(a, pl.group, s);
-    else if (pl.bm == 32 && pl.bn == 64) qlaunch<T, EPI, OutT, 32, 64, true, NV, 128, q_depth<32, 64, true, 128, SIX>()>(a, pl.group, s);
-    else if (pl.bm == 64 && pl.bn == 64) qlaunch<T, EPI, OutT, 64, 64, true, NV, 128, q_depth<64, 64, true, 128, SIX>()>(a, pl.group, s);
-    else return false;
-    return true;
+    if (pl.bm == 32 && pl.bn == 32) return qlaunch<T, EPI, OutT, 32, 32, true, NV, 128, q_depth<32, 32, true, 128, SIX>()>(a, pl.group, s);
+    if (pl.bm == 32 && pl.bn == 64) return qlaunch<T, EPI, OutT, 32, 64, true, NV, 128, q_depth<32, 64, true, 128, SIX>()>(a, pl.group, s);
+    if (pl.bm == 64 && pl.bn == 64) return qlaunch<T, EPI, OutT, 64, 64, true, NV, 128, q_depth<64, 64, true, 128, SIX>()>(a, pl.group, s);
+    return false;
 }
 
 template <typename T>
@@ -405,7 +377,7 @@
     if (a.x != nullptr) {
         const int d = a.g.K;
         QLnPlan pl;
-        if (!o16 || !q_plan_ln(a.g.M, a.g.N, d, epi, a.g.n_split, &pl, a.tile)) return false;
+        if (!o16 || !q_plan_ln(a.g.M, a.g.N, d, q_kind(epi), a.g.n_split, q_ncu(), &pl, q_force(a))) return false;
         const bool six = (d / 128) % 6 == 0;
 #define QLN(NVV)                                                                                                          \
         do {                                                                                                               \
@@ -432,7 +404,8 @@
     if (M <= 0 || M > QGEMM_MAX_ROWS || M % 32 || K < 128 || N % 16) return false;
     if (epi == EPI_QKV && (n_split % 32 || n_split <= 0 || n_split >= N || N % 32)) return false;
     if (!(epi == EPI_STORE || epi == EPI_QKV || epi == EPI_BIAS_GELU || epi == EPI_BIAS_RESID)) return false;
-    return q_pick_plain(M, N, K, epi, n_split) >= 0;
+    QPlainPlan pl;
+    return q_pick_plain(M, N, K, q_kind(epi), n_split, q_ncu(), &pl);
 }
 
 bool qgemm_ln_ok(int M, int N, int d, int epi, int n_split) {
@@ -440,7 +413,12 @@
     if (epi == EPI_QKV && (n_split % 32 || n_split <= 0 || n_split >= N)) return false;
     if (d != 768 && d != 1024 && d != 512) return false;
     QLnPlan pl;
-    return q_plan_ln(M, N, d, epi, n_split, &pl);
+    return q_plan_ln(M, N, d, q_kind(epi), n_split, q_ncu(), &pl);
+}
+
+bool qgemm_ln_fused(int M, int N, int d, int epi, int n_split) {
+    if (!qgemm_ln_ok(M, N, d, epi, n_split)) return false;
+    return q_plan_fused(M, N, d, q_kind(epi), n_split, q_ncu()) == 1;
 }
 
 bool launch_qgemm(int dtype, int epi, int out_dtype, const QGemmArgs& a0, hipStream_t s) {
diff --git a/sgpt_amd/csrc/qplan.h b/sgpt_amd/csrc/qplan.h
--- /dev/null
+++ b/sgpt_amd/csrc/qplan.h
@@ -0,0 +1,106 @@
+#pragma once
+
+namespace qplan {
+
+constexpr int Q_THREADS = 512;
+constexpr long Q_LDS_LIMIT = 160 * 1024;
+
+struct QTile { int bm, bn, kd; bool no_resid; };
+enum QKind { Q_KIND_OTHER = 0, Q_KIND_QKV = 1, Q_KIND_RESID = 2 };
+constexpr QTile Q_TILES[] = {{32, 16, 256, false}, {32, 32, 128, false}, {32, 64, 128, false}, {64, 32, 128, false}, {64, 64, 128, false}, {128, 64, 128, false},
+                             {128, 128, 128, false}, {96, 64, 128, false}, {96, 128, 128, false}, {160, 128, 128, false}, {192, 128, 128, true}};
+constexpr int Q_NTILES = sizeof(Q_TILES) / sizeof(Q_TILES[0]);
+constexpr int Q_NKNOB = 7;
+
+struct QForce { int k, bm, bn; };
+constexpr QForce Q_NO_FORCE = {0, 0, 0};
+inline bool q_forced_out(const QForce& f, int i, int bm, int bn) {
+    if (f.k > 0) return i != f.k - 1;
+    if (f.bm > 0) return bm != f.bm || bn != f.bn;
+    return false;
+}
+
+constexpr int q_chunks(int bm, int bn, bool ln_a, int kd) { return ((ln_a ? 0 : bm) + bn) * kd * 2 / (Q_THREADS * 16); }
+constexpr int q_depth_rule(int ch, bool six) { return ch >= 8 ? 2 : six ? (ch * 6 <= 24 ? 6 : 3) : (ch * 4 <= 16 ? 4 : 2); }
+
+inline int q_class(const QTile& tl, bool ln_a, int K) {
+    if (K % tl.kd) return 0;
+    const int nk = K / tl.kd;
+    const int ch = q_chunks(tl.bm, tl.bn, ln_a, tl.kd);
+    const int d6 = q_depth_rule(ch, true), d4 = q_depth_rule(ch, false);
+    const bool ok6 = nk % d6 == 0, ok4 = nk % d4 == 0;
+    if (ok6 && (!ok4 || d6 >= d4)) return 6;
+    return ok4 ? 4 : 0;
+}
+
+inline long q_cost_ns(long fixed_ns, long rounds, long wg_bytes, long ns_per_16k, long before_ns) {
+    return fixed_ns + rounds * wg_bytes * ns_per_16k / 16384 + before_ns;
+}
+constexpr long Q_PLAIN_FIXED_NS = 1600, Q_PLAIN_NS_PER_16K = 431;
+inline long q_ln_launch_ns(int M, int d) { return 3800 + (long)M * d * 2 / 1024; }
+constexpr long Q_UNFUSE_MARGIN_NS = 1500;
+
+struct QPlainPlan { int tile, rounds; long lds, cost; };
+inline bool q_pick_plain(int M, int N, int K, int kind, int n_split, int ncu, QPlainPlan* out, QForce force = Q_NO_FORCE) {
+    if (ncu < 1) ncu = 1;
+    if (force.k > Q_NKNOB) return false;
+    int best = -1; QPlainPlan bp{-1, 0, 0, 0};
+    for (int i = 0; i < Q_NTILES; ++i) {
+        const QTile& tl = Q_TILES[i];
+        if (q_forced_out(force, i, tl.bm, tl.bn)) continue;
+        if (N % tl.bn || !q_class(tl, false, K)) continue;
+        if (kind == Q_KIND_QKV && (n_split % tl.bn || tl.bn < 16)) continue;
+        if (kind == Q_KIND_RESID && tl.no_resid) continue;
+        if (tl.bm > 32 && M <= 32) continue;
+        const long lds = 2l * (tl.bm + tl.bn) * tl.kd * 2;
+        if (lds > Q_LDS_LIMIT) continue;
+        const long tiles = (long)((M + tl.bm - 1) / tl.bm) * (N / tl.bn);
+        const long rounds = (tiles + ncu - 1) / ncu;
+        const long cost = q_cost_ns(Q_PLAIN_FIXED_NS, rounds, (long)(tl.bm + tl.bn) * K * 2, Q_PLAIN_NS_PER_16K, 0);
+        if (best < 0 || cost < bp.cost || (cost == bp.cost && tl.bm * tl.bn > Q_TILES[best].bm * Q_TILES[best].bn)) {
+            best = i; bp = QPlainPlan{i, (int)rounds, lds, cost};
+        }
+    }
+    if (best < 0) return false;
+    *out = bp;
+    return true;
+}
+
+struct QLnPlan { int bm, bn, group; long lds, cost; };
+constexpr int Q_LN_TILES[3][2] = {{32, 32}, {32, 64}, {64, 64}};
+inline bool q_plan_ln(int M, int N, int d, int kind, int n_split, int ncu, QLnPlan* out, QForce force = Q_NO_FORCE) {
+    if (d % 128 || N % 32) return false;
+    if (ncu < 1) ncu = 1;
+    const int nk = d / 128;
+    if (nk % 6 != 0 && nk % 4 != 0) return false;
+    QLnPlan best{0, 0, 0, 0, 0};
+    for (int ci = 0; ci < 3; ++ci) {
+        const int bm = Q_LN_TILES[ci][0], bn = Q_LN_TILES[ci][1];
+        if (q_forced_out(force, ci, bm, bn)) continue;
+        if (N % bn || (kind == Q_KIND_QKV && n_split % bn)) continue;
+        if (bm > 32 && M <= 32) continue;
+        const int mt = (M + bm - 1) / bm, nt = N / bn;
+        if (mt > ncu) continue;
+        int gq = (int)(((long)mt * nt + ncu - 1) / ncu);
+        gq = gq < 1 ? 1 : gq;
+        while ((long)mt * ((nt + gq - 1) / gq) > ncu && gq < nt) ++gq;
+        const long lds = (long)nk * bm * 256 + 2l * bn * 256 + (long)gq * bn * 4;
+        if (lds > Q_LDS_LIMIT) continue;
+        const long cost = q_cost_ns(bm == 32 ? 6200 : 9400, 1, (long)gq * nk * bn * 256, bn == 32 ? 500 : bm == 32 ? 350 : 440, 0) +
+                          (kind == Q_KIND_QKV ? (long)M * 3 / 2 : 0);
+        if (best.bm == 0 || cost < best.cost) best = QLnPlan{bm, bn, gq, lds, cost};
+    }
+    if (best.bm == 0) return false;
+    *out = best;
+    return true;
+}
+
+inline int q_plan_fused(int M, int N, int d, int kind, int n_split, int ncu) {
+    QLnPlan ln; QPlainPlan pp;
+    const bool has_ln = q_plan_ln(M, N, d, kind, n_split, ncu, &ln), has_plain = q_pick_plain(M, N, d, kind, n_split, ncu, &pp);
+    if (!has_ln) return has_plain ? 0 : -1;
+    if (!has_plain) return 1;
+    return ln.cost <= pp.cost + q_ln_launch_ns(M, d) + Q_UNFUSE_MARGIN_NS ? 1 : 0;
+}
+
+}
diff --git a/sgpt_amd/runtime.py b/sgpt_amd/runtime.py
--- a/sgpt_amd/runtime.py
+++ b/sgpt_amd/runtime.py
@@ -171,6 +171,12 @@
 
     def set_query_tile(self, k: int) -> int:
         return int(self.lib.sgpt_ctx_set_query_tile(self.handle, int(k)))
+
+    def set_query_tile_shape(self, bm: int, bn: int) -> Tuple[int, int]:
+        old = int(self.lib.sgpt_ctx_set_query_tile_shape(self.handle, int(bm), int(bn)))
+        if old < 0:
+            raise ValueError(f"set_query_tile_shape({bm}, {bn}): both positive, or both 0")
+        return old >> 16, old & 0xFFFF
 
     def reserve(self, encode_bytes: int = 0, score_bytes: int = 0) -> None:
         self._chk(self.lib.sgpt_ctx_reserve(self.handle, encode_bytes, score_bytes), "sgpt_ctx_reserve")
```

Result: no change. 37460, median of 2 (-0.0%).
